# mit-acl/clipper

Measured on AMD Instinct MI355X. Metric: affinity+solve ms and GEMV HBM GB/s, n=10k assoc, 95% outliers, 1/8 GPU, lower is better.
Workload: dtype f64 (M stored f32)

## Files before the change

clipper_amd/csrc/clipper_hip.hip:

```cpp
#include <hip/hip_runtime.h>
#include <rccl/rccl.h>

#include <dlfcn.h>

#include <algorithm>
#include <atomic>
#include <chrono>
#include <cmath>
#include <cstdarg>
#include <cstdio>
#include <cstdlib>
#include <cstring>
#include <functional>
#include <limits>
#include <queue>
#include <string>
#include <type_traits>
#include <utility>
#include <map>
#include <mutex>
#include <new>
#include <exception>
#include <vector>

#include "../../include/clipper_hip.h"
#include "kernels.hip.h"
#include "dsd_host.h"
#include "host_batch.hpp"
#include "host_plan.hpp"

using namespace clipper_hip;

#include "host_state.hpp"
#include "host_solver.hpp"
#include "host_matrix.hpp"
#include "host_rowview.hpp"
#include "host_resident.hpp"
#include "host_rv_resident.hpp"
#include "host_subproblem.hpp"
#include "host_registration.hpp"

namespace {

template <int K, int D>
int knn_run(const double* dP0, int64_t n0, const double* dP1, int64_t n1, int S, int64_t chunk,
            double* pd, int32_t* pi, double* od, int32_t* oi, hipStream_t st) {
  dim3 g(static_cast<unsigned>(ceil_div(n0, 256)), static_cast<unsigned>(S));
  hipLaunchKernelGGL((k_knn_partial<K, D>), g, dim3(256), 0, st, dP0, n0, dP1, n1, chunk, pd, pi);
  hipLaunchKernelGGL((k_knn_merge<K>), dim3(static_cast<unsigned>(ceil_div(n0, 256))), dim3(256), 0,
                     st, pd, pi, n0, S, od, oi);
  return 0;
}

}

extern "C" {

const char* clipper_hip_last_error(void) try {
  return g_err.c_str();
} CLIPPER_HIP_GUARD_STR

int clipper_hip_device_count(void) try {
  int n = 0;
  if (hipGetDeviceCount(&n) != hipSuccess) {
    (void)hipGetLastError();
    return 0;
  }
  return n;
} CLIPPER_HIP_GUARD_INT

clipper_hip_t* clipper_hip_create(int device, int storage) try {
  return make_ctx(&device, 1, storage, 1, 0, false);
} CLIPPER_HIP_GUARD_PTR

clipper_hip_t* clipper_hip_create_group(const int* devices, int nshards, int storage) try {
  if (!devices || nshards < 1) {
    fail(CLIPPER_HIP_E_INVALID, "invalid shard list");
    return nullptr;
  }
  return make_ctx(devices, nshards, storage, nshards, 0, false);
} CLIPPER_HIP_GUARD_PTR

clipper_hip_t* clipper_hip_create_rank(int device, int storage, int rank, int world) try {
  if (world < 1 || rank < 0 || rank >= world) {
    fail(CLIPPER_HIP_E_INVALID, "rank %d / world %d invalid", rank, world);
    return nullptr;
  }
  const char* force = std::getenv("CLIPPER_HIP_FORCE_RCCL");
  const bool multiproc = world > 1 || (force && force[0] == '1');
  return make_ctx(&device, 1, storage, world, rank, multiproc);
} CLIPPER_HIP_GUARD_PTR

int clipper_hip_comm_unique_id(void* id128) try {
  if (!id128) return fail(CLIPPER_HIP_E_INVALID, "null id buffer");
  int rc = load_rccl();
  if (rc) return rc;
  static_assert(sizeof(ncclUniqueId) == 128, "ncclUniqueId is 128 bytes");
  ncclUniqueId id;
  ncclResult_t r = g_rccl.GetUniqueId(&id);
  if (r != ncclSuccess) return fail(CLIPPER_HIP_E_COMM, "ncclGetUniqueId failed (%d)", (int)r);
  std::memcpy(id128, &id, sizeof(id));
  return 0;
} CLIPPER_HIP_GUARD_INT

int clipper_hip_comm_init(clipper_hip_t* h, const void* id128) try {
  if (!h || !id128) return fail(CLIPPER_HIP_E_INVALID, "invalid argument");
  if (!h->multiproc) return 0;
  int rc = load_rccl();
  if (rc) return rc;
  ncclUniqueId id;
  std::memcpy(&id, id128, sizeof(id));
  HIPCHK(hipSetDevice(h->sh[0].device));
  ncclResult_t r = g_rccl.CommInitRank(&h->comm, h->world, id, h->sh[0].slot);
  if (r != ncclSuccess)
    return fail(CLIPPER_HIP_E_COMM, "ncclCommInitRank: %s",
                g_rccl.GetErrorString ? g_rccl.GetErrorString(r) : "error");
  return 0;
} CLIPPER_HIP_GUARD_INT

int clipper_hip_comm_init_callback(clipper_hip_t* h, clipper_hip_allgather_fn fn, void* user) try {
  if (!h || !fn) return fail(CLIPPER_HIP_E_INVALID, "invalid argument");
  if (!h->multiproc) return 0;
  h->xchg_fn = fn;
  h->xchg_user = user;
  return 0;
} CLIPPER_HIP_GUARD_INT

void clipper_hip_destroy(clipper_hip_t* h) try {
  if (!h) return;
  for (auto& s : h->sh) {
    hipSetDevice(s.device);
    if (s.stream) hipStreamSynchronize(s.stream);
  }
  if (h->comm && g_rccl.CommDestroy) g_rccl.CommDestroy(h->comm);
  sub_free(h);
  for (auto& s : h->sh) {
    free_shard_buffers(s);
    if (s.ev_reduced) hipEventDestroy(s.ev_reduced);
    if (s.ev_copied) hipEventDestroy(s.ev_copied);
    if (s.stream) hipStreamDestroy(s.stream);
  }
  if (!h->sh.empty()) hipSetDevice(h->sh[0].device);
  for (hipEvent_t e : h->ev_pairs) hipEventDestroy(e);
  for (hipEvent_t e : h->ev_xchg) hipEventDestroy(e);
  if (h->ev_poll[0]) hipEventDestroy(h->ev_poll[0]);
  if (h->ev_poll[1]) hipEventDestroy(h->ev_poll[1]);
  if (h->host_state) hipHostFree(h->host_state);
  if (h->mirror) hipHostFree(h->mirror);
  if (h->kind) hipHostFree(h->kind);
  if (h->u_pinned) hipHostFree(h->u_pinned);
  if (h->stamps_dev) hipFree(h->stamps_dev);
  if (h->xchg_send) hipHostFree(h->xchg_send);
  if (h->xchg_recv) hipHostFree(h->xchg_recv);
  if (h->ev_aff[0]) hipEventDestroy(h->ev_aff[0]);
  if (h->ev_aff[1]) hipEventDestroy(h->ev_aff[1]);
  if (h->csc_hLq) hipHostFree(h->csc_hLq);
  if (h->csc_hctl) hipHostFree(h->csc_hctl);
  if (h->csc_htotal) hipHostFree(h->csc_htotal);
  resident_free(h);
  rvr_free(h);
  if (h->csc_hwork) hipHostFree(h->csc_hwork);
  if (h->rv_count) hipHostFree(h->rv_count);
  if (h->rv_desc_host) hipHostFree(h->rv_desc_host);
  delete h;
} CLIPPER_HIP_GUARD_VOID


int clipper_hip_stage_inputs(clipper_hip_t* h, const double* D1, int d, int64_t n1,
                             const double* D2, int64_t n2, const int32_t* A, int64_t m) try {
  return stage_inputs(h, D1, d, n1, D2, n2, A, m);
} CLIPPER_HIP_GUARD_INT

int clipper_hip_affinity_euclidean_staged(clipper_hip_t* h, double sigma, double epsilon,
                                          double mindist, double affinityeps) try {
  if (!h) return fail(CLIPPER_HIP_E_INVALID, "invalid argument");
  if (h->staged_d < 1) return fail(CLIPPER_HIP_E_STATE, "clipper_hip_stage_inputs not called");
  const EuclidParams prm{sigma, epsilon, mindist, affinityeps};
  const int64_t mm = h->m, W = h->W, pstride = h->staged_pstride;
  const int d = h->staged_d;
  h->fill_kind = 1;
  h->fill_e = prm;
  h->fill_n = PointNormalParams{};
  h->fill_E2 = guarded_threshold_sq(guarded_threshold(epsilon, h->staged_maxabs, d));
  return run_affinity(h, use_sym_fill(h) && (d == 2 || d == 3), [&](Shard& s) {
    dim3 grid(static_cast<unsigned>(ceil_div(W, 1024)),
              static_cast<unsigned>(ceil_div(mm, AFF_ROWS_PER_BLK))),
        block(256);
    const int64_t c0 = static_cast<int64_t>(s.slot) * W;
    const int32_t* A0 = s.Adev;
    const int32_t* A1 = s.Adev + mm;
#define LAUNCH_EUCLID(T, D)                                                                 \
  hipLaunchKernelGGL((k_affinity_euclid<T, D>), grid, block, 0, s.stream,                   \
                     static_cast<T*>(s.S), W, mm, c0, AFF_ROWS_PER_BLK, d, s.P1, s.P2, pstride, \
                     A0, A1, prm)
#define LAUNCH_EUCLID_COMPACT(T, D)                                                         \
  hipLaunchKernelGGL((k_affinity_euclid_compact<T, D>), grid, block, 0, s.stream,           \
                     static_cast<T*>(s.S), W, mm, c0, AFF_ROWS_PER_BLK, s.P1, s.P2, s.P1f,  \
                     s.P2f, pstride, A0, A1, prm, thr)
    const float thr = guarded_threshold(epsilon, h->staged_maxabs, d);
    if (use_sym_fill(h) && (d == 2 || d == 3)) {
      const int nT = static_cast<int>(ceil_div(mm, AT));
      dim3 g(static_cast<unsigned>(static_cast<int64_t>(nT) * (nT + 1) / 2));
      const PointNormalParams none{};
      const float E2 = guarded_threshold_sq(thr);
      if (h->storage == CLIPPER_HIP_STORE_F64) {
        if (d == 3)
          launch_sym<double>(k_affinity_sym<3, false, double>, g, s.stream, static_cast<double*>(nullptr), W, mm, nT, s,
                             pstride, A0, A1, prm, none, E2, h->csc_out);
        else
          launch_sym<double>(k_affinity_sym<2, false, double>, g, s.stream, static_cast<double*>(nullptr), W, mm, nT, s,
                             pstride, A0, A1, prm, none, E2, h->csc_out);
      } else if (d == 3)
        launch_sym<float>(k_affinity_sym<3, false>, g, s.stream, static_cast<float*>(s.S), W, mm, nT, s,
                          pstride, A0, A1, prm, none, E2, h->csc_out);
      else
        launch_sym<float>(k_affinity_sym<2, false>, g, s.stream, static_cast<float*>(s.S), W, mm, nT, s,
                          pstride, A0, A1, prm, none, E2, h->csc_out);
      h->csc_emitted = (h->csc_out.Pre != nullptr);
      return;
    }
    const bool compact = !h->plain_affinity && (d == 2 || d == 3);
    if (h->storage == CLIPPER_HIP_STORE_F64) {
      if (compact && d == 3) LAUNCH_EUCLID_COMPACT(double, 3);
      else if (compact && d == 2) LAUNCH_EUCLID_COMPACT(double, 2);
      else if (d == 3) LAUNCH_EUCLID(double, 3);
      else if (d == 2) LAUNCH_EUCLID(double, 2);
      else LAUNCH_EUCLID(double, 0);
    } else {
      if (compact && d == 3) LAUNCH_EUCLID_COMPACT(float, 3);
      else if (compact && d == 2) LAUNCH_EUCLID_COMPACT(float, 2);
      else if (d == 3) LAUNCH_EUCLID(float, 3);
      else if (d == 2) LAUNCH_EUCLID(float, 2);
      else LAUNCH_EUCLID(float, 0);
    }
#undef LAUNCH_EUCLID_COMPACT
#undef LAUNCH_EUCLID
  });
} CLIPPER_HIP_GUARD_INT

int clipper_hip_affinity_pointnormal_staged(clipper_hip_t* h, double sigp, double epsp,
                                            double sign, double epsn, double affinityeps) try {
  if (!h) return fail(CLIPPER_HIP_E_INVALID, "invalid argument");
  if (h->staged_d != 6)
    return fail(CLIPPER_HIP_E_STATE, "PointNormalDistance needs staged inputs with d == 6");
  const PointNormalParams prm{sigp, epsp, sign, epsn, affinityeps};
  const int64_t mm = h->m, W = h->W, pstride = h->staged_pstride;
  h->fill_kind = 2;
  h->fill_e = EuclidParams{};
  h->fill_n = prm;
  h->fill_E2 = guarded_threshold_sq(guarded_threshold(epsp, h->staged_maxabs, 3));
  return run_affinity(h, use_sym_fill(h), [&](Shard& s) {
    dim3 grid(static_cast<unsigned>(ceil_div(W, 1024)),
              static_cast<unsigned>(ceil_div(mm, AFF_ROWS_PER_BLK))),
        block(256);
    const int64_t c0 = static_cast<int64_t>(s.slot) * W;
    const float thr = guarded_threshold(epsp, h->staged_maxabs, 3);
    if (use_sym_fill(h)) {
      const int nT = static_cast<int>(ceil_div(mm, AT));
      dim3 g(static_cast<unsigned>(static_cast<int64_t>(nT) * (nT + 1) / 2));
      const EuclidParams none{};
      if (h->storage == CLIPPER_HIP_STORE_F64)
        launch_sym<double>(k_affinity_sym<3, true, double>, g, s.stream, static_cast<double*>(nullptr), W, mm, nT, s,
                           pstride, s.Adev, s.Adev + mm, none, prm, guarded_threshold_sq(thr), h->csc_out);
      else
        launch_sym<float>(k_affinity_sym<3, true>, g, s.stream, static_cast<float*>(s.S), W, mm, nT, s,
                          pstride, s.Adev, s.Adev + mm, none, prm, guarded_threshold_sq(thr), h->csc_out);
      h->csc_emitted = (h->csc_out.Pre != nullptr);
      return;
    }
    if (h->plain_affinity) {
      if (h->storage == CLIPPER_HIP_STORE_F64)
        hipLaunchKernelGGL((k_affinity_pointnormal<double>), grid, block, 0, s.stream,
                           static_cast<double*>(s.S), W, mm, c0, AFF_ROWS_PER_BLK, s.P1, s.P2,
                           pstride, s.Adev, s.Adev + mm, prm);
      else
        hipLaunchKernelGGL((k_affinity_pointnormal<float>), grid, block, 0, s.stream,
                           static_cast<float*>(s.S), W, mm, c0, AFF_ROWS_PER_BLK, s.P1, s.P2,
                           pstride, s.Adev, s.Adev + mm, prm);
    } else {
      if (h->storage == CLIPPER_HIP_STORE_F64)
        hipLaunchKernelGGL((k_affinity_pointnormal_compact<double>), grid, block, 0, s.stream,
                           static_cast<double*>(s.S), W, mm, c0, AFF_ROWS_PER_BLK, s.P1, s.P2,
                           s.P1f, s.P2f, pstride, s.Adev, s.Adev + mm, prm, thr);
      else
        hipLaunchKernelGGL((k_affinity_pointnormal_compact<float>), grid, block, 0, s.stream,
                           static_cast<float*>(s.S), W, mm, c0, AFF_ROWS_PER_BLK, s.P1, s.P2,
                           s.P1f, s.P2f, pstride, s.Adev, s.Adev + mm, prm, thr);
    }
  });
} CLIPPER_HIP_GUARD_INT

int clipper_hip_affinity_euclidean(clipper_hip_t* h, const double* D1, int d, int64_t n1,
                                   const double* D2, int64_t n2, const int32_t* A, int64_t m,
                                   double sigma, double epsilon, double mindist,
                                   double affinityeps) try {
  const auto t0 = std::chrono::high_resolution_clock::now();
  int rc = stage_inputs(h, D1, d, n1, D2, n2, A, m);
  if (rc) return rc;
  rc = clipper_hip_affinity_euclidean_staged(h, sigma, epsilon, mindist, affinityeps);
  if (rc) return rc;
  h->tm.affinity_total_ms =
      std::chrono::duration<double, std::milli>(std::chrono::high_resolution_clock::now() - t0)
          .count();
  return 0;
} CLIPPER_HIP_GUARD_INT

int clipper_hip_affinity_pointnormal(clipper_hip_t* h, const double* D1, int d, int64_t n1,
                                     const double* D2, int64_t n2, const int32_t* A, int64_t m,
                                     double sigp, double epsp, double sign, double epsn,
                                     double affinityeps) try {
  if (d != 6) return fail(CLIPPER_HIP_E_INVALID, "PointNormalDistance needs d == 6");
  const auto t0 = std::chrono::high_resolution_clock::now();
  int rc = stage_inputs(h, D1, d, n1, D2, n2, A, m);
  if (rc) return rc;
  rc = clipper_hip_affinity_pointnormal_staged(h, sigp, epsp, sign, epsn, affinityeps);
  if (rc) return rc;
  h->tm.affinity_total_ms =
      std::chrono::duration<double, std::milli>(std::chrono::high_resolution_clock::now() - t0)
          .count();
  return 0;
} CLIPPER_HIP_GUARD_INT

int64_t clipper_hip_num_associations(const clipper_hip_t* h) try {
  return h ? h->m : 0;
} CLIPPER_HIP_GUARD_INT

int clipper_hip_get_associations(const clipper_hip_t* h, int32_t* A_out) try {
  if (!h || !A_out) return fail(CLIPPER_HIP_E_INVALID, "invalid argument");
  if (h->A.size() != static_cast<size_t>(2 * h->m))
    return fail(CLIPPER_HIP_E_STATE, "no association list is held");
  std::memcpy(A_out, h->A.data(), h->A.size() * sizeof(int32_t));
  return 0;
} CLIPPER_HIP_GUARD_INT


int clipper_hip_set_matrix(clipper_hip_t* h, const double* M, const double* C, int64_t m) try {
  if (!h || !M || !C || m < 1) return fail(CLIPPER_HIP_E_INVALID, "invalid argument");
  if (h->A.size() != static_cast<size_t>(2 * m)) h->A.clear();
  h->nodes.clear();
  h->has_matrix = false;
  h->csc_valid = false;
  h->fill_kind = 0;
  rowview_drop(h);
  int rc = ensure_problem(h, m);
  if (rc) return rc;
  h->has_matrix = false;
  h->csc_valid = false;
  if ((rc = ensure_dense(h, false))) return rc;
  const size_t bytes = static_cast<size_t>(m) * m * sizeof(double);
  const int64_t W = h->W;
  struct Temps {
    std::vector<std::pair<int, void*>> v;
    ~Temps() {
      for (auto& p : v) {
        hipSetDevice(p.first);
        hipFree(p.second);
      }
    }
    int alloc(int dev, void** p, size_t n) {
      HIPCHK(hipMalloc(p, n));
      v.emplace_back(dev, *p);
      return 0;
    }
  } tmp;
  std::vector<double*> dM(h->sh.size(), nullptr), dC(h->sh.size(), nullptr);
  std::vector<int*> dflag(h->sh.size(), nullptr);
  int mismatch = 0;
  const unsigned gy = static_cast<unsigned>(std::min<int64_t>(m, 65535));
  for (size_t k = 0; k < h->sh.size(); ++k) {
    Shard& s = h->sh[k];
    HIPCHK(hipSetDevice(s.device));
    if ((rc = tmp.alloc(s.device, reinterpret_cast<void**>(&dM[k]), bytes))) return rc;
    if ((rc = tmp.alloc(s.device, reinterpret_cast<void**>(&dC[k]), bytes))) return rc;
    if ((rc = tmp.alloc(s.device, reinterpret_cast<void**>(&dflag[k]), sizeof(int)))) return rc;
    HIPCHK(hipMemsetAsync(dflag[k], 0, sizeof(int), s.stream));
    HIPCHK(hipMemcpyAsync(dM[k], M, bytes, hipMemcpyHostToDevice, s.stream));
    HIPCHK(hipMemcpyAsync(dC[k], C, bytes, hipMemcpyHostToDevice, s.stream));
    if (s.Cs) {
      hipFree(s.Cs);
      s.Cs = nullptr;
    }
    dim3 grid(static_cast<unsigned>(ceil_div(W, 256)), gy), block(256);
    const int64_t c0 = static_cast<int64_t>(s.slot) * W;
    if (h->storage == CLIPPER_HIP_STORE_F64)
      hipLaunchKernelGGL((k_from_dense_upper<double>), grid, block, 0, s.stream,
                         static_cast<double*>(s.S), W, m, c0, dM[k], dC[k],
                         static_cast<double*>(nullptr), dflag[k]);
    else
      hipLaunchKernelGGL((k_from_dense_upper<float>), grid, block, 0, s.stream,
                         static_cast<float*>(s.S), W, m, c0, dM[k], dC[k],
                         static_cast<float*>(nullptr), dflag[k]);
    int f = 0;
    HIPCHK(hipMemcpyAsync(&f, dflag[k], sizeof(int), hipMemcpyDeviceToHost, s.stream));
    HIPCHK(hipStreamSynchronize(s.stream));
    HIPCHK(hipGetLastError());
    mismatch |= f;
  }
  if (h->world > 1 && !mismatch) {
    for (int64_t hi = 1; hi < m && !mismatch; ++hi)
      for (int64_t lo = 0; lo < hi; ++lo) {
        const double mv = M[lo + hi * m], cv = C[lo + hi * m];
        if (cv != ((mv != 0.0) ? 1.0 : 0.0)) {
          mismatch = 1;
          break;
        }
      }
  }
  h->explicitC = (mismatch != 0);
  plan_tiles(h);
  if (h->explicitC) {
    for (size_t k = 0; k < h->sh.size(); ++k) {
      Shard& s = h->sh[k];
      HIPCHK(hipSetDevice(s.device));
      HIPCHK(hipMalloc(&s.Cs, s.bytes_S));
      dim3 grid(static_cast<unsigned>(ceil_div(W, 256)), gy), block(256);
      const int64_t c0 = static_cast<int64_t>(s.slot) * W;
      if (h->storage == CLIPPER_HIP_STORE_F64)
        hipLaunchKernelGGL((k_from_dense_upper<double>), grid, block, 0, s.stream,
                           static_cast<double*>(s.S), W, m, c0, dM[k], dC[k],
                           static_cast<double*>(s.Cs), static_cast<int*>(nullptr));
      else
        hipLaunchKernelGGL((k_from_dense_upper<float>), grid, block, 0, s.stream,
                           static_cast<float*>(s.S), W, m, c0, dM[k], dC[k],
                           static_cast<float*>(s.Cs), static_cast<int*>(nullptr));
    }
  }
  if ((rc = sync_all(h))) return rc;
  if ((rc = csc_rebuild(h))) return rc;
  h->has_matrix = true;
  return 0;
} CLIPPER_HIP_GUARD_INT

int clipper_hip_set_sparse(clipper_hip_t* h, int64_t m, const int64_t* Mcolptr,
                           const int32_t* Mrow, const double* Mval, const int64_t* Ccolptr,
                           const int32_t* Crow, const double* Cval) try {
  if (!h || !Mcolptr || !Ccolptr || m < 1) return fail(CLIPPER_HIP_E_INVALID, "invalid argument");
  auto check_csc = [&](const char* what, const int64_t* cp, const int32_t* ri, const double* va) -> int {
    if (cp[0] != 0) return fail(CLIPPER_HIP_E_INVALID, "%s: colptr[0] must be 0", what);
    for (int64_t c = 0; c < m; ++c)
      if (cp[c + 1] < cp[c]) return fail(CLIPPER_HIP_E_INVALID, "%s: colptr decreases at column %lld", what, static_cast<long long>(c));
    const int64_t nnz = cp[m];
    if (nnz > 0 && (!ri || !va)) return fail(CLIPPER_HIP_E_INVALID, "%s: null CSC arrays", what);
    for (int64_t p = 0; p < nnz; ++p)
      if (ri[p] < 0 || ri[p] >= m)
        return fail(CLIPPER_HIP_E_INVALID, "%s: row index %d out of range at entry %lld", what, ri[p], static_cast<long long>(p));
    return 0;
  };
  int rc;
  if ((rc = check_csc("M", Mcolptr, Mrow, Mval))) return rc;
  if ((rc = check_csc("C", Ccolptr, Crow, Cval))) return rc;
  struct Csc {
    std::vector<int64_t> cp;
    std::vector<int32_t> ri;
    std::vector<double> va;
  } Mn, Cn;
  int64_t dropped_below = 0;
  auto upper_only = [&](const char* what, const int64_t*& cp, const int32_t*& ri, const double*& va, Csc& out) -> int {
    bool strict = true;
    for (int64_t j = 0; j < m && strict; ++j)
      for (int64_t p = cp[j]; p < cp[j + 1]; ++p)
        if (ri[p] >= j) {
          strict = false;
          break;
        }
    if (strict) return 0;
    out.cp.assign(static_cast<size_t>(m) + 1, 0);
    for (int64_t j = 0; j < m; ++j) {
      for (int64_t p = cp[j]; p < cp[j + 1]; ++p) {
        const int64_t i = ri[p];
        if (i > j) {
          ++dropped_below;
          continue;
        }
        if (i == j) {
          if (va[p] != 0.0)
            return fail(CLIPPER_HIP_E_INVALID, "%s: a stored diagonal entry (%lld,%lld) — the matrices must not have diagonal values set",
                        what, static_cast<long long>(i), static_cast<long long>(j));
          continue;
        }
        out.ri.push_back(static_cast<int32_t>(i));
        out.va.push_back(va[p]);
      }
      out.cp[static_cast<size_t>(j) + 1] = static_cast<int64_t>(out.ri.size());
    }
    cp = out.cp.data();
    ri = out.ri.data();
    va = out.va.data();
    return 0;
  };
  if ((rc = upper_only("M", Mcolptr, Mrow, Mval, Mn))) return rc;
  if ((rc = upper_only("C", Ccolptr, Crow, Cval, Cn))) return rc;
  if (dropped_below > 0)
    (void)fail(0, "warning: %lld stored entries below the diagonal were ignored (the matrices are read through their upper "
                  "triangle, as the reference's selfadjointView<Upper> does: clipper.cpp:194-271)", static_cast<long long>(dropped_below));
  const int64_t nnzM = Mcolptr[m], nnzC = Ccolptr[m];
  if (h->A.size() != static_cast<size_t>(2 * m)) h->A.clear();
  h->nodes.clear();
  h->has_matrix = false;
  h->csc_valid = false;
  h->total_slice_bytes = 0.0;
  h->fill_kind = 0;
  rowview_drop(h);
  if ((rc = ensure_problem(h, m))) return rc;
  h->has_matrix = false;
  h->csc_valid = false;
  bool pattern = (nnzM == nnzC) && std::equal(Mcolptr, Mcolptr + m + 1, Ccolptr) &&
                 (nnzM == 0 || std::equal(Mrow, Mrow + nnzM, Crow));
  for (int64_t p = 0; pattern && p < nnzM; ++p) pattern = (Cval[p] == 1.0) && (Mval[p] != 0.0);
  h->explicitC = !pattern;
  plan_tiles(h);
  const int64_t W = h->W;
  for (auto& s : h->sh) {
    HIPCHK(hipSetDevice(s.device));
    if (s.Cs) {
      hipFree(s.Cs);
      s.Cs = nullptr;
    }
  }
  struct Temps {
    std::vector<std::pair<int, void*>> v;
    ~Temps() {
      for (auto& p : v) {
        hipSetDevice(p.first);
        hipFree(p.second);
      }
    }
    int alloc(int dev, void** p, size_t n) {
      HIPCHK(hipMalloc(p, std::max<size_t>(n, 16)));
      v.emplace_back(dev, *p);
      return 0;
    }
  } tmp;

  if (csc_applies(h)) {
    drop_dense(h);
    std::vector<int64_t> cp(static_cast<size_t>(m) + 1, 0);
    for (int64_t j = 0; j < m; ++j)
      for (int64_t p = Mcolptr[j]; p < Mcolptr[j + 1]; ++p) {
        const int64_t i = Mrow[p];
        if (i == j) continue;
        ++cp[static_cast<size_t>(i) + 1];
        ++cp[static_cast<size_t>(j) + 1];
      }
    for (int64_t c = 0; c < m; ++c) cp[static_cast<size_t>(c) + 1] += cp[static_cast<size_t>(c)];
    const int64_t nnz2 = cp[static_cast<size_t>(m)];
    std::vector<int32_t> ri(static_cast<size_t>(nnz2));
    std::vector<double> va(static_cast<size_t>(nnz2));
    {
      std::vector<int64_t> cur(cp.begin(), cp.end() - 1);
      for (int64_t j = 0; j < m; ++j)
        for (int64_t p = Mcolptr[j]; p < Mcolptr[j + 1]; ++p) {
          const int64_t i = Mrow[p];
          if (i == j) continue;
          int64_t& a = cur[static_cast<size_t>(j)];
          ri[static_cast<size_t>(a)] = static_cast<int32_t>(i);
          va[static_cast<size_t>(a)] = Mval[p];
          ++a;
          int64_t& b = cur[static_cast<size_t>(i)];
          ri[static_cast<size_t>(b)] = static_cast<int32_t>(j);
          va[static_cast<size_t>(b)] = Mval[p];
          ++b;
        }
    }
    std::vector<std::pair<int32_t, double>> buf;
    for (int64_t c = 0; c < m; ++c) {
      const int64_t a = cp[static_cast<size_t>(c)], b = cp[static_cast<size_t>(c) + 1];
      bool sorted = true;
      for (int64_t p = a + 1; p < b && sorted; ++p) sorted = ri[static_cast<size_t>(p - 1)] < ri[static_cast<size_t>(p)];
      if (sorted) continue;
      buf.clear();
      for (int64_t p = a; p < b; ++p) buf.emplace_back(ri[static_cast<size_t>(p)], va[static_cast<size_t>(p)]);
      std::sort(buf.begin(), buf.end(), [](const auto& x, const auto& y) { return x.first < y.first; });
      for (size_t q = 1; q < buf.size(); ++q)
        if (buf[q - 1].first == buf[q].first)
          return fail(CLIPPER_HIP_E_INVALID, "entry (%d,%lld) is stored more than once", buf[q].first,
                      static_cast<long long>(c));
      for (int64_t p = a; p < b; ++p) {
        ri[static_cast<size_t>(p)] = buf[static_cast<size_t>(p - a)].first;
        va[static_cast<size_t>(p)] = buf[static_cast<size_t>(p - a)].second;
      }
    }
    for (auto& s : h->sh) {
      HIPCHK(hipSetDevice(s.device));
      int64_t* dcp = nullptr;
      int32_t* dri = nullptr;
      double* dva = nullptr;
      if ((rc = tmp.alloc(s.device, reinterpret_cast<void**>(&dcp), cp.size() * sizeof(int64_t)))) return rc;
      if ((rc = tmp.alloc(s.device, reinterpret_cast<void**>(&dri), ri.size() * sizeof(int32_t)))) return rc;
      if ((rc = tmp.alloc(s.device, reinterpret_cast<void**>(&dva), va.size() * sizeof(double)))) return rc;
      HIPCHK(hipMemcpyAsync(dcp, cp.data(), cp.size() * sizeof(int64_t), hipMemcpyHostToDevice, s.stream));
      if (nnz2 > 0) {
        HIPCHK(hipMemcpyAsync(dri, ri.data(), ri.size() * sizeof(int32_t), hipMemcpyHostToDevice, s.stream));
        HIPCHK(hipMemcpyAsync(dva, va.data(), va.size() * sizeof(double), hipMemcpyHostToDevice, s.stream));
      }
      const int64_t c0 = static_cast<int64_t>(s.slot) * W;
      dispatch_vt(h, [&](auto t) {
        using VT = decltype(t);
        bool again = true;
        for (int attempt = 0; again && !rc; ++attempt) {
          if (attempt >= 3) {
            rc = fail(CLIPPER_HIP_E_HIP, "compressed storage: the build keeps overflowing");
            break;
          }
          GroupOut<VT> unused;
          if ((rc = groups_prepare<VT>(h, s, unused))) break;
          CscSource<VT> src{};
          src.colptr = dcp + std::min<int64_t>(c0, m);
          src.rowidx = dri;
          src.values = dva;
          src.ncols = std::max<int64_t>(0, std::min<int64_t>(W, m - c0));
          if ((rc = slices_enqueue<VT>(h, s, src, nullptr))) break;
          if (hipStreamSynchronize(s.stream) != hipSuccess) {
            rc = fail(CLIPPER_HIP_E_HIP, "set_sparse: %s", hipGetErrorString(hipGetLastError()));
            break;
          }
          rc = slices_check<VT>(h, s, false, again);
        }
      });
      if (rc) return rc;
    }
    if ((rc = sync_all(h))) return rc;
    h->csc_valid = true;
    if ((rc = gather_slice_bytes(h))) return rc;
    h->has_matrix = true;
    return 0;
  }

  if ((rc = ensure_dense(h, false))) return rc;
  auto scatter = [&](Shard& s, void* dst, const int64_t* cp, const int32_t* ri, const double* va,
                     int64_t nnz) -> int {
    int64_t* dcp = nullptr;
    int32_t* dri = nullptr;
    double* dva = nullptr;
    int r;
    if ((r = tmp.alloc(s.device, reinterpret_cast<void**>(&dcp), static_cast<size_t>(m + 1) * sizeof(int64_t)))) return r;
    if ((r = tmp.alloc(s.device, reinterpret_cast<void**>(&dri), static_cast<size_t>(nnz) * sizeof(int32_t)))) return r;
    if ((r = tmp.alloc(s.device, reinterpret_cast<void**>(&dva), static_cast<size_t>(nnz) * sizeof(double)))) return r;
    HIPCHK(hipMemcpyAsync(dcp, cp, static_cast<size_t>(m + 1) * sizeof(int64_t),
                          hipMemcpyHostToDevice, s.stream));
    if (nnz > 0) {
      HIPCHK(hipMemcpyAsync(dri, ri, static_cast<size_t>(nnz) * sizeof(int32_t),
                            hipMemcpyHostToDevice, s.stream));
      HIPCHK(hipMemcpyAsync(dva, va, static_cast<size_t>(nnz) * sizeof(double),
                            hipMemcpyHostToDevice, s.stream));
    }
    HIPCHK(hipMemsetAsync(dst, 0, s.bytes_S, s.stream));
    const int64_t c0 = static_cast<int64_t>(s.slot) * W;
    dim3 grid(static_cast<unsigned>(std::min<int64_t>(m, 1 << 20))), block(256);
    if (h->storage == CLIPPER_HIP_STORE_F64)
      hipLaunchKernelGGL((k_from_csc<double>), grid, block, 0, s.stream,
                         static_cast<double*>(dst), W, m, c0, W, dcp, dri, dva);
    else
      hipLaunchKernelGGL((k_from_csc<float>), grid, block, 0, s.stream, static_cast<float*>(dst),
                         W, m, c0, W, dcp, dri, dva);
    HIPCHK(hipGetLastError());
    HIPCHK(hipStreamSynchronize(s.stream));
    return 0;
  };
  for (auto& s : h->sh) {
    HIPCHK(hipSetDevice(s.device));
    rc = scatter(s, s.S, Mcolptr, Mrow, Mval, nnzM);
    if (rc) return rc;
    if (h->explicitC) {
      HIPCHK(hipMalloc(&s.Cs, s.bytes_S));
      rc = scatter(s, s.Cs, Ccolptr, Crow, Cval, nnzC);
      if (rc) return rc;
    }
  }
  rc = csc_rebuild(h);
  if (rc) return rc;
  h->has_matrix = true;
  return 0;
} CLIPPER_HIP_GUARD_INT

int clipper_hip_get_matrix(clipper_hip_t* h, double* M_out, double* C_out) try {
  if (!h) return fail(CLIPPER_HIP_E_INVALID, "invalid argument");
  if (!h->has_matrix) return fail(CLIPPER_HIP_E_STATE, "no matrix has been built or set");
  if (h->multiproc)
    return fail(CLIPPER_HIP_E_STATE, "get_matrix is not available on a multi-process shard");
  const int64_t m = h->m, W = h->W;
  const bool f64 = (h->storage == CLIPPER_HIP_STORE_F64);
  if (int rc = ensure_dense(h, true)) return rc;
  std::vector<unsigned char> buf;
  auto fetch = [&](Shard& s, const void* src, double* out, bool as_pattern) -> int {
    buf.resize(s.bytes_S);
    HIPCHK(hipSetDevice(s.device));
    HIPCHK(hipMemcpy(buf.data(), src, s.bytes_S, hipMemcpyDeviceToHost));
    const int64_t c0 = static_cast<int64_t>(s.slot) * W;
    for (int64_t c = 0; c < W; ++c) {
      const int64_t g = c0 + c;
      if (g >= m) break;
      for (int64_t j = 0; j < m; ++j) {
        const double v = f64 ? reinterpret_cast<const double*>(buf.data())[j * W + c]
                             : static_cast<double>(
                                   reinterpret_cast<const float*>(buf.data())[j * W + c]);
        double o = as_pattern ? ((v != 0.0) ? 1.0 : 0.0) : v;
        if (j == g) o += 1.0;
        out[j + g * m] = o;
      }
    }
    return 0;
  };
  for (auto& s : h->sh) {
    int rc;
    if (M_out && (rc = fetch(s, s.S, M_out, false))) return rc;
    if (C_out) {
      rc = h->explicitC ? fetch(s, s.Cs, C_out, false) : fetch(s, s.S, C_out, true);
      if (rc) return rc;
    }
  }
  if (h->csc_valid) drop_dense(h);
  return 0;
} CLIPPER_HIP_GUARD_INT


int clipper_hip_stage_u0(clipper_hip_t* h, const double* u0) try {
  if (!h || !u0) return fail(CLIPPER_HIP_E_INVALID, "u0 is required");
  if (!h->has_matrix) return fail(CLIPPER_HIP_E_STATE, "no matrix has been built or set");
  const size_t vbytes = static_cast<size_t>(h->m) * sizeof(double);
  for (auto& s : h->sh) {
    HIPCHK(hipSetDevice(s.device));
    HIPCHK(hipMemcpyAsync(s.u0, u0, vbytes, hipMemcpyHostToDevice, s.stream));
  }
  int rc = sync_all(h);
  if (rc) return rc;
  h->u0_staged = true;
  return 0;
} CLIPPER_HIP_GUARD_INT

int clipper_hip_solve(clipper_hip_t* h, const double* u0, const clipper_params_t* P,
                      double* u_out, clipper_solve_info_t* info) try {
  if (!h || !u0 || !P) return fail(CLIPPER_HIP_E_INVALID, "u0 and params are required");
  const auto t0 = std::chrono::high_resolution_clock::now();
  int rc = clipper_hip_stage_u0(h, u0);
  if (rc) return rc;
  rc = clipper_hip_solve_staged(h, P, u_out, info);
  if (rc) return rc;
  const double secs =
      std::chrono::duration<double>(std::chrono::high_resolution_clock::now() - t0).count();
  h->tm.solve_total_ms = secs * 1e3;
  if (info) info->seconds = secs;
  return 0;
} CLIPPER_HIP_GUARD_INT

int clipper_hip_solve_staged(clipper_hip_t* h, const clipper_params_t* P, double* u_out,
                             clipper_solve_info_t* info) try {
  if (!h || !P) return fail(CLIPPER_HIP_E_INVALID, "params are required");
  if (!h->has_matrix) return fail(CLIPPER_HIP_E_STATE, "no matrix has been built or set");
  if (!h->u0_staged) return fail(CLIPPER_HIP_E_STATE, "clipper_hip_stage_u0 not called");
  if (P->rounding == CLIPPER_ROUNDING_DSD && h->multiproc)
    return fail(CLIPPER_HIP_E_SCOPE,
                "Rounding::DSD needs the induced sub-matrix on one host: not available on a "
                "multi-process shard");
  if (P->rounding != CLIPPER_ROUNDING_NONZERO && P->rounding != CLIPPER_ROUNDING_DSD_HEU &&
      P->rounding != CLIPPER_ROUNDING_DSD)
    return fail(CLIPPER_HIP_E_INVALID, "unknown rounding mode %d", P->rounding);
  if (P->maxlsiters < 1) return fail(CLIPPER_HIP_E_INVALID, "maxlsiters must be >= 1");

  const auto t0 = std::chrono::high_resolution_clock::now();
  const int64_t m = h->m;
  const size_t vbytes = static_cast<size_t>(m) * sizeof(double);
  static const bool host_timing = std::getenv("CLIPPER_HIP_HOST_TIMING") != nullptr;
  std::vector<std::pair<const char*, double>> marks_t;
  auto mark_t = [&](const char* what) {
    if (host_timing)
      marks_t.emplace_back(what, std::chrono::duration<double, std::micro>(std::chrono::high_resolution_clock::now() - t0).count());
  };

  h->rv_stats = clipper_hip_view_stats_t{};
  h->ev_used = 0;
  std::fill(h->ev_xchg_used.begin(), h->ev_xchg_used.end(), 0);
  if (h->profiling)
  {
    const size_t n = static_cast<size_t>(std::min<int64_t>(h->launch_counter + 1, KIND_CAP));
    std::memset(h->kind, 0, n);
    HIPCHK(hipSetDevice(h->sh[0].device));
    HIPCHK(hipMemsetAsync(h->sh[0].marks, 0, n, h->sh[0].stream));
  }
  h->launch_counter = 0;

  SolverParams prm;
  prm.tol_u = P->tol_u;
  prm.tol_F = P->tol_F;
  prm.beta = P->beta;
  prm.eps = P->eps;
  prm.maxiniters = P->maxiniters;
  prm.maxoliters = P->maxoliters;
  prm.maxlsiters = P->maxlsiters;

  SolverState init;
  std::memset(&init, 0, sizeof(init));
  init.alpha = 1.0;
  for (int l = 0; l < VS; ++l) init.nrm[l] = 1.0;
  init.nlive = init.nout = static_cast<int32_t>(std::min<int64_t>(m, 0x7fffffff));
  init.rv_last = -100;
  init.weff = 0;
  init.zero_run = 2;
  rowview_drop(h);
  rvr_begin_solve(h);
  sub_begin_solve(h);
  h->rvp = rowview_policy(h);
  init.phase = P->rescale_u0 ? PH_RESCALE : PH_NORMALIZE;
  init.stage = P->rescale_u0 ? ST_PASS : ST_RESULTS;
  if (h->u_pinned_cap < vbytes) {
    if (h->u_pinned) hipHostFree(h->u_pinned);
    h->u_pinned = nullptr;
    h->u_pinned_dev = nullptr;
    h->u_pinned_cap = 0;
    HIPCHK(hipSetDevice(h->sh[0].device));
    HIPCHK(hipHostMalloc(reinterpret_cast<void**>(&h->u_pinned), vbytes,
                         hipHostMallocMapped | hipHostMallocCoherent));
    HIPCHK(hipHostGetDevicePointer(reinterpret_cast<void**>(&h->u_pinned_dev), h->u_pinned, 0));
    h->u_pinned_cap = vbytes;
  }
  Shard& s0 = h->sh[0];
  SolveShared fin;
  std::memset(&fin, 0, sizeof(fin));
  int rc = 0;
  bool resident = false;
  if ((rc = resident_solve(h, prm, P->rescale_u0 != 0, fin, resident))) return rc;
  h->last_solver = resident ? 1 : 0;
  if (!resident) {
  h->par = 0;
  std::memset(h->mirror, 0, sizeof(HostMirror));
  std::atomic_thread_fence(std::memory_order_seq_cst);
  for (auto& s : h->sh) {
    HIPCHK(hipSetDevice(s.device));
    const SolveArgs a = solve_args(h, s, prm, 0);
    hipLaunchKernelGGL(k_init, dim3(static_cast<unsigned>(ceil_div(m, 256))), dim3(256), 0,
                       s.stream, a, init, s.st, s.X[0]);
  }
  mark_t("init queued");
  if (!h->multiproc) {
    volatile HostMirror* hm = h->mirror;
    int64_t queued = 0;
    uint64_t spins = 0;
    h->rv_fresh = false;
    constexpr int run_ahead = RUN_AHEAD;
    h->enqueue_one = [h, &prm]() { return enqueue_iteration(h, prm); };
    auto enqueue_next = [&]() { return enqueue_iteration(h->sub.active ? h->sub.use : h, prm); };
    auto sub_account = [&]() {
      h->sub.sub_passes += std::max<int64_t>(0, hm->n_passes - h->sub.passes_at_entry);
    };
    struct ClearEnqueue {
      Ctx* c;
      ~ClearEnqueue() { c->enqueue_one = nullptr; }
    } clear_enqueue{h};
    while (!hm->done) {
      if (hm->hold) {
        mark_t("hold seen");
        if (host_timing)
          std::fprintf(stderr, "[solve] hold: iters %lld passes %lld trials %lld view passes %lld live %d of which outside the view %d\n",
                       static_cast<long long>(hm->iters), static_cast<long long>(hm->n_passes), static_cast<long long>(hm->n_trials),
                       static_cast<long long>(hm->n_view_passes), static_cast<int>(hm->hold_nlive), static_cast<int>(hm->nout));
        if (h->sh.size() > 1 && (rc = sync_all(h))) return rc;
        std::atomic_thread_fence(std::memory_order_acquire);
        const int hold_reason = hm->hold;
        hm->hold = 0;
        queued = hm->iters;
        h->launch_counter = hm->iters;
        while (h->ev_used > 0 && h->ev_launch_index[static_cast<size_t>(h->ev_used - 1)] >= hm->iters)
          --h->ev_used;
        if (hold_reason == 2) {
          if ((rc = sub_enter(h, prm))) return rc;
          ++queued;
          mark_t("sub-problem entered");
          continue;
        }
        if (hold_reason == 3) {
          sub_account();
          if ((rc = sub_leave(h))) return rc;
          mark_t("sub-problem left");
          continue;
        }
        bool built = false;
        if ((rc = rowview_build(h, built))) return rc;
        mark_t("view built");
        const bool early = h->early_decide_done;
        h->early_decide_done = false;
        if (early) ++queued;
        else h->rv_fresh = built;
        if (built && h->vres.ready) {
          if (!early) {
            h->decide_only = true;
            rc = enqueue_iteration(h, prm);
            h->decide_only = false;
            if (rc) return rc;
            ++queued;
          }
          bool launched = false;
          if ((rc = rvr_enqueue(h, prm, launched))) return rc;
          mark_t("resident queued");
        }
        if ((rc = rowview_finish_plan(h))) return rc;
        if (built && !h->vres.ready && !early) {
          if (int r2 = sub_prepare(h)) {
            if (r2 != CLIPPER_HIP_E_NOMEM) return r2;
            (void)hipGetLastError();
            h->sub.ready = false;
          }
          mark_t("sub-problem prepared");
        }
        continue;
      }
      if (hm->iters > queued) queued = hm->iters;
      if (queued - hm->iters < run_ahead) {
        if ((rc = enqueue_next())) return rc;
        ++queued;
        spins = 0;
      } else if ((++spins & 0xfffff) == 0) {
        hipError_t q = hipStreamQuery(s0.stream);
        if (q != hipSuccess && q != hipErrorNotReady)
          return fail(CLIPPER_HIP_E_HIP, "solver stream failed: %s", hipGetErrorString(q));
        if (q == hipSuccess && !hm->done && queued - hm->iters >= run_ahead)
          return fail(CLIPPER_HIP_E_HIP, "solver made no progress (iters %lld of %lld queued)",
                      static_cast<long long>(hm->iters), static_cast<long long>(queued));
      }
    }
    mark_t("done seen");
    std::atomic_thread_fence(std::memory_order_acquire);
    if (h->sub.active) {
      sub_account();
      h->sub.active = false;
    }
    fin.F = hm->F;
    fin.d = hm->d;
    fin.n_passes = hm->n_passes;
    fin.n_trials = hm->n_trials;
    fin.ifinal = hm->ifinal;
    fin.ubp = hm->ubp;
    fin.ubv = hm->ubv;
    h->rv_stats.view_passes = hm->n_view_passes;
  } else {
    int batch = SOLVE_BATCH;
    if (const char* e = std::getenv("CLIPPER_HIP_SOLVE_BATCH")) batch = std::max(1, std::atoi(e));
    HIPCHK(hipSetDevice(s0.device));
    h->rv_fresh = false;
    rc = run_batched_with_holds(
        batch, [&]() { return enqueue_iteration(h, prm); },
        [&](int slot) -> int {
          HIPCHK(hipSetDevice(s0.device));
          HIPCHK(hipMemcpyAsync(&h->host_state[slot], s0.shared, sizeof(SolveShared),
                                hipMemcpyDeviceToHost, s0.stream));
          HIPCHK(hipEventRecord(h->ev_poll[slot], s0.stream));
          return 0;
        },
        [&](int slot, int& st) -> int {
          HIPCHK(hipEventSynchronize(h->ev_poll[slot]));
          st = h->host_state[slot].done != 0 ? 1 : (h->host_state[slot].hold != 0 ? 2 : 0);
          return 0;
        },
        [&]() -> int {
          if (int r2 = sync_all(h)) return r2;
          h->mirror->hold = 0;
          h->launch_counter = h->mirror->iters;
          while (h->ev_used > 0 && h->ev_launch_index[static_cast<size_t>(h->ev_used - 1)] >= h->mirror->iters)
            --h->ev_used;
          bool built = false;
          if (int r2 = rowview_build(h, built)) return r2;
          h->rv_fresh = built;
          if (built)
            if (int r2 = rvr_replica_handover(h, prm)) return r2;
          return 0;
        },
        nullptr);
    if (rc) return rc;
    if ((rc = sync_all(h))) return rc;
    HIPCHK(hipSetDevice(s0.device));
    HIPCHK(hipMemcpy(&fin, s0.shared, sizeof(fin), hipMemcpyDeviceToHost));
    h->rv_stats.view_passes = h->mirror->n_view_passes;
  }

  rvr_end_solve(h);
  }

  HIPCHK(hipSetDevice(s0.device));
  if (h->multiproc) {
    const double* u_dev =
        s0.pt + ((static_cast<int64_t>(fin.ubp & 1) * h->V + fin.ubv) * 2 + 0) * h->mp;
    HIPCHK(hipMemcpyAsync(h->u_pinned, u_dev, vbytes, hipMemcpyDeviceToHost, s0.stream));
    if (h->profiling)
      HIPCHK(hipMemcpyAsync(h->kind, s0.marks,
                            static_cast<size_t>(std::min<int64_t>(h->launch_counter, KIND_CAP)),
                            hipMemcpyDeviceToHost, s0.stream));
    if ((rc = sync_all(h))) return rc;
  } else {
    HIPCHK(hipGetLastError());
  }
  std::vector<double>& u = h->u_host;
  u.assign(h->u_pinned, h->u_pinned + m);

  std::vector<int32_t> nodes;
  if (P->rounding == CLIPPER_ROUNDING_NONZERO) {
    for (int64_t i = 0; i < m; ++i)
      if (u[static_cast<size_t>(i)] > 0.0) nodes.push_back(static_cast<int32_t>(i));
  } else if (P->rounding == CLIPPER_ROUNDING_DSD) {
    std::vector<int32_t> S;
    for (int64_t i = 0; i < m; ++i)
      if (u[static_cast<size_t>(i)] > 0.0) S.push_back(static_cast<int32_t>(i));
    if ((rc = densest_subgraph_of(h, S, nodes))) return rc;
  } else {
    const int omega = static_cast<int>(std::round(fin.F));
    nodes = indices_of_k_largest(u, omega);
  }
  h->nodes = nodes;
  if (u_out) std::memcpy(u_out, u.data(), vbytes);
  mark_t("rounded");
  if (host_timing) {
    std::fprintf(stderr, "[solve]");
    for (const auto& mk : marks_t) std::fprintf(stderr, " %s %.1f |", mk.first, mk.second);
    std::fprintf(stderr, "\n");
  }

  const double secs =
      std::chrono::duration<double>(std::chrono::high_resolution_clock::now() - t0).count();
  h->tm.solve_total_ms = secs * 1e3;
  if (info) {
    info->score = fin.F;
    info->seconds = secs;
    info->d = fin.d;
    info->ifinal = fin.ifinal;
    info->num_nodes = static_cast<int32_t>(nodes.size());
    info->n_passes = fin.n_passes;
    info->n_trials = fin.n_trials;
  }
  h->rv_stats.passes = fin.n_passes;
  h->rv_stats.sub_leaves = h->sub.leaves;
  h->rv_stats.sub_passes = h->sub.sub_passes;
  h->rv_stats.sub_build_ms = h->sub.build_ms;
  if (h->rv_stats.sub_entries > 0 && h->sub.use) {
    h->rv_stats.sub_rows = h->sub.nS;
    h->rv_stats.sub_bytes = h->sub.use->csc_valid ? static_cast<int64_t>(h->sub.use->sh[0].s_bytes)
                                                   : static_cast<int64_t>(algorithmic_gemv_bytes(h->sub.use));
    h->rv_stats.sub_dense = h->sub.use->csc_valid ? 0 : 1;
  }

  h->tm.gemv_avg_us = h->tm.gemv_min_us = 0.0;
  h->tm.gemv_launches = 0;
  h->tm.gemv_bytes = algorithmic_gemv_bytes(h);
  h->tm.gemv_useful_bytes = h->csc_valid ? static_cast<double>(h->sh[0].s_entries) * (h->esize() + 1.0) : h->tm.gemv_bytes;
  if (h->profiling && h->ev_used > 0) {
    const uint8_t* kind = h->kind;
    const int64_t iters_run = std::min<int64_t>(h->launch_counter, KIND_CAP);
    double sum = 0.0, mn = 1e30, vsum = 0.0, ssum = 0.0;
    int64_t nreal = 0, nview = 0, nsub = 0;
    for (int k = 0; k < h->ev_used; ++k) {
      const int64_t li = h->ev_launch_index[static_cast<size_t>(k)];
      if (li >= iters_run || !kind[static_cast<size_t>(li)]) continue;
      float ms = 0.f;
      HIPCHK(hipEventElapsedTime(&ms, h->ev_pairs[2 * k], h->ev_pairs[2 * k + 1]));
      if (kind[static_cast<size_t>(li)] == 2) {
        vsum += ms;
        ++nview;
        continue;
      }
      if (kind[static_cast<size_t>(li)] == 4) {
        ssum += ms;
        ++nsub;
        continue;
      }
      if (kind[static_cast<size_t>(li)] == 3 || kind[static_cast<size_t>(li)] == 5) continue;
      sum += ms;
      mn = std::min<double>(mn, ms);
      ++nreal;
    }
    h->tm.exchange_avg_us = 0.0;
    h->tm.exchange_samples = 0;
    h->tm.exchange_bytes = static_cast<double>(nslot(h->V)) * static_cast<double>(h->W) * sizeof(double);
    {
      double xs = 0.0;
      int64_t nx = 0;
      for (int k = 0; k < h->ev_used; ++k) {
        const int64_t li = h->ev_launch_index[static_cast<size_t>(k)];
        if (!h->ev_xchg_used[static_cast<size_t>(k)] || li >= iters_run || !kind[static_cast<size_t>(li)]) continue;
        float ms = 0.f;
        HIPCHK(hipEventElapsedTime(&ms, h->ev_xchg[2 * k], h->ev_xchg[2 * k + 1]));
        xs += ms;
        ++nx;
      }
      if (nx > 0) {
        h->tm.exchange_avg_us = xs / static_cast<double>(nx) * 1e3;
        h->tm.exchange_samples = nx;
      }
    }
    if (nview > 0) {
      h->rv_stats.view_pass_avg_us = vsum / static_cast<double>(nview) * 1e3;
      h->rv_stats.view_pass_samples = nview;
    }
    if (nsub > 0) {
      h->rv_stats.sub_pass_avg_us = ssum / static_cast<double>(nsub) * 1e3;
      h->rv_stats.sub_pass_samples = nsub;
    }
    if (nreal > 0) {
      h->tm.gemv_avg_us = sum / static_cast<double>(nreal) * 1e3;
      h->tm.gemv_min_us = mn * 1e3;
      h->tm.gemv_launches = nreal;
    }
  }
  return 0;
} CLIPPER_HIP_GUARD_INT

int clipper_hip_get_nodes(const clipper_hip_t* h, int32_t* out, int32_t capacity) try {
  if (!h || !out) return fail(CLIPPER_HIP_E_INVALID, "invalid argument");
  const int32_t k = static_cast<int32_t>(h->nodes.size());
  if (capacity < k) return fail(CLIPPER_HIP_E_INVALID, "capacity %d < %d nodes", capacity, k);
  if (k) std::memcpy(out, h->nodes.data(), static_cast<size_t>(k) * sizeof(int32_t));
  return k;
} CLIPPER_HIP_GUARD_INT

int clipper_hip_get_selected_associations(const clipper_hip_t* h, int32_t* A_out,
                                          int32_t capacity) try {
  if (!h || !A_out) return fail(CLIPPER_HIP_E_INVALID, "invalid argument");
  const int32_t k = static_cast<int32_t>(h->nodes.size());
  if (capacity < k) return fail(CLIPPER_HIP_E_INVALID, "capacity %d < %d nodes", capacity, k);
  if (k == 0) return 0;
  if (h->A.size() != static_cast<size_t>(2 * h->m))
    return fail(CLIPPER_HIP_E_STATE, "no association list is held");
  for (int32_t r = 0; r < k; ++r) {
    const size_t n = static_cast<size_t>(h->nodes[static_cast<size_t>(r)]);
    A_out[r] = h->A[n];
    A_out[k + r] = h->A[static_cast<size_t>(h->m) + n];
  }
  return k;
} CLIPPER_HIP_GUARD_INT

int clipper_hip_densest_subgraph(clipper_hip_t* h, const int32_t* S, int32_t k, int32_t* nodes_out,
                                 int32_t capacity) try {
  if (!h || !nodes_out) return fail(CLIPPER_HIP_E_INVALID, "invalid argument");
  if (!h->has_matrix) return fail(CLIPPER_HIP_E_STATE, "no matrix has been built or set");
  if (h->multiproc)
    return fail(CLIPPER_HIP_E_SCOPE, "not available on a multi-process shard");
  std::vector<int32_t> sub;
  if (S == nullptr || k <= 0) {
    sub.resize(static_cast<size_t>(h->m));
    for (int64_t i = 0; i < h->m; ++i) sub[static_cast<size_t>(i)] = static_cast<int32_t>(i);
  } else {
    sub.assign(S, S + k);
    for (int32_t v : sub)
      if (v < 0 || v >= h->m) return fail(CLIPPER_HIP_E_INVALID, "node %d out of range", v);
  }
  std::vector<int32_t> nodes;
  int rc = densest_subgraph_of(h, sub, nodes);
  if (rc) return rc;
  const int32_t n = static_cast<int32_t>(nodes.size());
  if (capacity < n) return fail(CLIPPER_HIP_E_INVALID, "capacity %d < %d nodes", capacity, n);
  if (n) std::memcpy(nodes_out, nodes.data(), static_cast<size_t>(n) * sizeof(int32_t));
  return n;
} CLIPPER_HIP_GUARD_INT


int clipper_hip_knn(int device, const double* P0, int64_t n0, const double* P1, int64_t n1, int d,
                    int knn, int32_t* idx_out, double* sqd_out) try {
  if (!P0 || !P1 || !idx_out || n0 < 1 || n1 < 1) return fail(CLIPPER_HIP_E_INVALID, "invalid argument");
  if (d != 2 && d != 3) return fail(CLIPPER_HIP_E_INVALID, "points must have 2 or 3 coordinates");
  if (knn < 1 || knn > 16) return fail(CLIPPER_HIP_E_INVALID, "knn must be in 1..16");
  int ndev = 0;
  if (hipGetDeviceCount(&ndev) != hipSuccess || ndev <= 0)
    return fail(CLIPPER_HIP_E_NODEVICE, "no HIP device visible (this library has no CPU fallback)");
  if (device < 0 || device >= ndev) return fail(CLIPPER_HIP_E_INVALID, "device %d out of range", device);
  HIPCHK(hipSetDevice(device));
  const int K = knn <= 1 ? 1 : (knn <= 2 ? 2 : (knn <= 4 ? 4 : (knn <= 8 ? 8 : 16)));
  const int64_t qblocks = ceil_div(n0, 256);
  const int64_t tiles = ceil_div(n1, KNN_TILE);
  const int S = static_cast<int>(std::max<int64_t>(1, std::min<int64_t>(tiles, ceil_div(512, qblocks))));
  const int64_t chunk = ceil_div(tiles, S) * KNN_TILE;
  double *dP0 = nullptr, *dP1 = nullptr, *pd = nullptr, *od = nullptr;
  int32_t *pi = nullptr, *oi = nullptr;
  auto cleanup = [&]() {
    hipFree(dP0); hipFree(dP1); hipFree(pd); hipFree(od); hipFree(pi); hipFree(oi);
  };
  const size_t b0 = static_cast<size_t>(n0) * d * sizeof(double), b1 = static_cast<size_t>(n1) * d * sizeof(double);
  const size_t np = static_cast<size_t>(S) * n0 * K, no = static_cast<size_t>(n0) * K;
  if (hipMalloc(&dP0, b0) != hipSuccess || hipMalloc(&dP1, b1) != hipSuccess ||
      hipMalloc(&pd, np * sizeof(double)) != hipSuccess || hipMalloc(&pi, np * sizeof(int32_t)) != hipSuccess ||
      hipMalloc(&od, no * sizeof(double)) != hipSuccess || hipMalloc(&oi, no * sizeof(int32_t)) != hipSuccess) {
    cleanup();
    return fail(CLIPPER_HIP_E_NOMEM, "device allocation failed");
  }
  hipStream_t st = nullptr;
  bool ok = hipMemcpyAsync(dP0, P0, b0, hipMemcpyHostToDevice, st) == hipSuccess &&
            hipMemcpyAsync(dP1, P1, b1, hipMemcpyHostToDevice, st) == hipSuccess;
  if (ok) {
#define KNN_CASE(KK)                                                                        \
  case KK:                                                                                  \
    if (d == 3) knn_run<KK, 3>(dP0, n0, dP1, n1, S, chunk, pd, pi, od, oi, st);             \
    else knn_run<KK, 2>(dP0, n0, dP1, n1, S, chunk, pd, pi, od, oi, st);                    \
    break
    switch (K) {
      KNN_CASE(1);
      KNN_CASE(2);
      KNN_CASE(4);
      KNN_CASE(8);
      default:
        if (d == 3) knn_run<16, 3>(dP0, n0, dP1, n1, S, chunk, pd, pi, od, oi, st);
        else knn_run<16, 2>(dP0, n0, dP1, n1, S, chunk, pd, pi, od, oi, st);
        break;
    }
#undef KNN_CASE
    std::vector<double> hd(no);
    std::vector<int32_t> hi(no);
    ok = hipMemcpy(hd.data(), od, no * sizeof(double), hipMemcpyDeviceToHost) == hipSuccess &&
         hipMemcpy(hi.data(), oi, no * sizeof(int32_t), hipMemcpyDeviceToHost) == hipSuccess &&
         hipGetLastError() == hipSuccess;
    if (ok) {
      for (int64_t i = 0; i < n0; ++i)
        for (int k = 0; k < knn; ++k) {
          idx_out[i * knn + k] = hi[static_cast<size_t>(i) * K + k];
          if (sqd_out) sqd_out[i * knn + k] = hd[static_cast<size_t>(i) * K + k];
        }
    }
  }
  cleanup();
  if (!ok) return fail(CLIPPER_HIP_E_HIP, "nearest-neighbour search failed: %s", hipGetErrorString(hipGetLastError()));
  return 0;
} CLIPPER_HIP_GUARD_INT

int64_t clipper_hip_distance_based_correspondences(int device, const double* P0, int64_t n0,
                                                   const double* P1, int64_t n1, int d, int knn,
                                                   double radius, int enforce_1to1, int32_t* A_out,
                                                   int64_t capacity) try {
  if (!A_out && capacity > 0) return fail(CLIPPER_HIP_E_INVALID, "invalid argument");
  std::vector<int32_t> idx(static_cast<size_t>(std::max<int64_t>(n0, 0)) * std::max(knn, 0));
  std::vector<double> sqd(idx.size());
  int rc = clipper_hip_knn(device, P0, n0, P1, n1, d, knn, idx.data(), sqd.data());
  if (rc) return rc;
  const double r2 = radius * radius;
  std::vector<std::pair<int32_t, int32_t>> rows;
  std::map<int32_t, std::vector<std::pair<int32_t, double>>> claim;
  for (int64_t i = 0; i < n0; ++i)
    for (int k = 0; k < knn; ++k) {
      const int32_t c1 = idx[static_cast<size_t>(i) * knn + k];
      const double sd = sqd[static_cast<size_t>(i) * knn + k];
      if (c1 < 0) continue;
      if (sd <= r2) {
        rows.emplace_back(static_cast<int32_t>(i), c1);
        if (enforce_1to1) claim[c1].emplace_back(static_cast<int32_t>(i), sd);
      }
    }
  if (enforce_1to1) {
    rows.clear();
    for (const auto& it : claim) {
      size_t best = 0;
      for (size_t q = 1; q < it.second.size(); ++q)
        if (it.second[q].second < it.second[best].second) best = q;
      rows.emplace_back(it.second[best].first, it.first);
    }
  }
  const int64_t n = static_cast<int64_t>(rows.size());
  if (n > capacity) return fail(CLIPPER_HIP_E_INVALID, "capacity %lld < %lld associations",
                                static_cast<long long>(capacity), static_cast<long long>(n));
  for (int64_t r = 0; r < n; ++r) {
    A_out[r] = rows[static_cast<size_t>(r)].first;
    A_out[n + r] = rows[static_cast<size_t>(r)].second;
  }
  return n;
} CLIPPER_HIP_GUARD_INT

int clipper_hip_set_window(clipper_hip_t* h, int window) try {
  if (!h) return fail(CLIPPER_HIP_E_INVALID, "invalid argument");
  if (window != 0 && window != 1 && window != 4 && window != 6 && window != 8)
    return fail(CLIPPER_HIP_E_INVALID, "window must be 0 (automatic), 1, 4, 6 or 8");
  h->V_forced = window;
  return 0;
} CLIPPER_HIP_GUARD_INT

int clipper_hip_window(const clipper_hip_t* h) try {
  return h ? h->V : 0;
} CLIPPER_HIP_GUARD_INT

int clipper_hip_set_resident(clipper_hip_t* h, int mode) try {
  if (!h) return fail(CLIPPER_HIP_E_INVALID, "invalid argument");
  if (mode != 0 && mode != 1 && mode != 2)
    return fail(CLIPPER_HIP_E_INVALID, "mode must be 0 (automatic), 1 (never) or 2 (the sub-problem always as slices)");
  h->resident_mode = mode;
  return 0;
} CLIPPER_HIP_GUARD_INT

int clipper_hip_last_solver(const clipper_hip_t* h) try {
  return h ? h->last_solver : -1;
} CLIPPER_HIP_GUARD_INT

int clipper_hip_set_row_view(clipper_hip_t* h, int mode) try {
  if (!h) return fail(CLIPPER_HIP_E_INVALID, "invalid argument");
  if (mode != 0 && mode != 1 && mode != 2)
    return fail(CLIPPER_HIP_E_INVALID, "mode must be 0 (automatic), 1 (never) or 2 (views, but streamed: never the resident solver on one)");
  h->rv_mode = mode;
  if (mode == 1) rowview_drop(h);
  if (mode != 0) h->vres.ready = false;
  return 0;
} CLIPPER_HIP_GUARD_INT

int clipper_hip_set_subproblem(clipper_hip_t* h, int mode) try {
  if (!h) return fail(CLIPPER_HIP_E_INVALID, "invalid argument");
  if (mode != 0 && mode != 1 && mode != 2)
    return fail(CLIPPER_HIP_E_INVALID, "mode must be 0 (automatic), 1 (never) or 2 (the sub-problem always as slices)");
  h->sub_mode = mode;
  if (mode == 1) h->sub.ready = false;
  return 0;
} CLIPPER_HIP_GUARD_INT

int clipper_hip_get_view_stats(const clipper_hip_t* h, clipper_hip_view_stats_t* out) try {
  if (!h || !out) return fail(CLIPPER_HIP_E_INVALID, "invalid argument");
  *out = h->rv_stats;
  return 0;
} CLIPPER_HIP_GUARD_INT

int clipper_hip_storage_in_use(const clipper_hip_t* h) try {
  if (!h) return -1;
  if (!h->csc_valid) return h->storage;
  return h->storage == CLIPPER_HIP_STORE_F64 ? CLIPPER_HIP_STORE_F64_CSC : CLIPPER_HIP_STORE_F32_CSC;
} CLIPPER_HIP_GUARD_INT

int clipper_hip_matvec(clipper_hip_t* h, const double* x, double* yM, double* yC) try {
  if (!h || !x) return fail(CLIPPER_HIP_E_INVALID, "invalid argument");
  if (!h->has_matrix) return fail(CLIPPER_HIP_E_STATE, "no matrix has been built or set");
  const int64_t m = h->m, W = h->W;
  for (auto& s : h->sh) {
    HIPCHK(hipSetDevice(s.device));
    HIPCHK(hipMemcpyAsync(s.u0, x, static_cast<size_t>(m) * sizeof(double),
                          hipMemcpyHostToDevice, s.stream));
    hipLaunchKernelGGL(k_spread, dim3(static_cast<unsigned>(ceil_div(m, 256))), dim3(256), 0,
                       s.stream, s.u0, m, s.X[0]);
  }
  h->u0_staged = false;
  int rc = h->csc_valid ? 0 : ensure_dense(h, true);
  if (rc) return rc;
  if ((rc = enqueue_gemv_plain(h))) return rc;
  if ((rc = enqueue_reduce_exchange(h))) return rc;
  if ((rc = sync_all(h))) return rc;
  std::vector<double> ab(static_cast<size_t>(h->world) * 2 * W);
  Shard& s0 = h->sh[0];
  HIPCHK(hipSetDevice(s0.device));
  HIPCHK(hipMemcpy(ab.data(), s0.ab, ab.size() * sizeof(double), hipMemcpyDeviceToHost));
  for (int64_t i = 0; i < m; ++i) {
    const int64_t p = i / W, off = i - p * W;
    if (yM) yM[i] = ab[static_cast<size_t>(p * 2 * W + off)];
    if (yC) yC[i] = ab[static_cast<size_t>(p * 2 * W + W + off)];
  }
  return 0;
} CLIPPER_HIP_GUARD_INT

int clipper_hip_view_matvec(clipper_hip_t* h, const int32_t* rows, int64_t nrows, const double* x,
                            double* yM, double* yC) try {
  if (!h || !rows || !x || nrows < 1) return fail(CLIPPER_HIP_E_INVALID, "invalid argument");
  if (!h->has_matrix || !h->csc_valid || !csc_single(h) || !rect_fill_possible(h))
    return fail(CLIPPER_HIP_E_STATE, "a row view needs slices of a matrix scored from staged points on one device");
  const int64_t m = h->m, W = h->W;
  for (int64_t r = 0; r < nrows; ++r)
    if (rows[r] < 0 || rows[r] >= m || (r > 0 && rows[r] <= rows[r - 1]))
      return fail(CLIPPER_HIP_E_INVALID, "rows must be ascending association indices");
  Shard& s = h->sh[0];
  RowView& v = s.rv;
  HIPCHK(hipSetDevice(s.device));
  HIPCHK(hipStreamSynchronize(s.stream));
  v.valid = false;
  int rc;
  {
    size_t r0 = v.cap_rows, r1 = v.cap_rows;
    if ((rc = rv_grow(v.rowmap[0], r0, static_cast<size_t>(h->mp)))) return rc;
    if ((rc = rv_grow(v.rowmap[1], r1, static_cast<size_t>(h->mp)))) return rc;
    v.cap_rows = static_cast<size_t>(h->mp);
  }
  HIPCHK(hipMemcpyAsync(v.rowmap[0], rows, static_cast<size_t>(nrows) * sizeof(int32_t), hipMemcpyHostToDevice, s.stream));
  for (int attempt = 0;; ++attempt) {
    SliceOut O{};
    if ((rc = emit_prepare(h, s, v.st, nrows, O))) return rc;
    if ((rc = launch_rect(h, s, v.rowmap[0], nrows, O))) return rc;
    if ((rc = emit_enqueue(h, s, v.st))) return rc;
    HIPCHK(hipStreamSynchronize(s.stream));
    HIPCHK(hipGetLastError());
    bool again = false;
    if ((rc = emit_check(h, s, v.st, false, again))) return rc;
    if (!again) break;
    if (attempt >= 2) return fail(CLIPPER_HIP_E_HIP, "row view: the build keeps overflowing");
  }
  HIPCHK(hipMemcpyAsync(s.u0, x, static_cast<size_t>(m) * sizeof(double), hipMemcpyHostToDevice, s.stream));
  hipLaunchKernelGGL(k_spread, dim3(static_cast<unsigned>(ceil_div(m, 256))), dim3(256), 0, s.stream, s.u0, m, s.X[0]);
  h->u0_staged = false;
  SliceView R{};
  R.data = v.st.sdata;
  R.Pre = v.st.sPre;
  R.work = v.st.swork;
  R.nchunks = v.st.s_nchunks;
  R.ncg = v.st.s_ncg;
  R.nwork = v.st.s_nwork;
  R.rowmap = v.rowmap[0];
  R.nrows = nrows;
  R.pad = 0;
  dim3 grid(static_cast<unsigned>(R.nwork)), block(SL_NW * 64);
  if (h->storage == CLIPPER_HIP_STORE_F64)
    hipLaunchKernelGGL((k_gemv_slices_plain<double, 1>), grid, block, 0, s.stream, R, W, m, s.X[0], s.part);
  else
    hipLaunchKernelGGL((k_gemv_slices_plain<float, 1>), grid, block, 0, s.stream, R, W, m, s.X[0], s.part);
  hipLaunchKernelGGL(k_reduce, dim3(static_cast<unsigned>(ceil_div(2 * W, 256))), dim3(256), 0, s.stream, s.part,
                     v.st.s_nslots, 2, W, s.ab);
  std::vector<double> ab(static_cast<size_t>(2 * W));
  HIPCHK(hipMemcpyAsync(ab.data(), s.ab, ab.size() * sizeof(double), hipMemcpyDeviceToHost, s.stream));
  HIPCHK(hipStreamSynchronize(s.stream));
  HIPCHK(hipGetLastError());
  for (int64_t i = 0; i < m; ++i) {
    if (yM) yM[i] = ab[static_cast<size_t>(i)];
    if (yC) yC[i] = ab[static_cast<size_t>(W + i)];
  }
  return 0;
} CLIPPER_HIP_GUARD_INT


int clipper_hip_set_profiling(clipper_hip_t* h, int on) try {
  if (!h) return fail(CLIPPER_HIP_E_INVALID, "invalid argument");
  h->profiling = (on != 0);
  h->profiling_level = on;
  if (h->profiling && h->ev_pairs.empty()) {
    HIPCHK(hipSetDevice(h->sh[0].device));
    h->ev_pairs.resize(2 * MAX_EVENT_PAIRS);
    h->ev_launch_index.assign(MAX_EVENT_PAIRS, 0);
    for (auto& e : h->ev_pairs) HIPCHK(hipEventCreate(&e));
    h->ev_xchg.resize(2 * MAX_EVENT_PAIRS);
    h->ev_xchg_used.assign(MAX_EVENT_PAIRS, 0);
    for (auto& e : h->ev_xchg) HIPCHK(hipEventCreate(&e));
  }
  return 0;
} CLIPPER_HIP_GUARD_INT

int clipper_hip_get_timings(const clipper_hip_t* h, clipper_hip_timings_t* out) try {
  if (!h || !out) return fail(CLIPPER_HIP_E_INVALID, "invalid argument");
  *out = h->tm;
  return 0;
} CLIPPER_HIP_GUARD_INT

int clipper_hip_bench_matvec(clipper_hip_t* h, int reps, double* avg_us) try {
  if (!h || reps < 1 || !avg_us) return fail(CLIPPER_HIP_E_INVALID, "invalid argument");
  if (!h->has_matrix) return fail(CLIPPER_HIP_E_STATE, "no matrix has been built or set");
  if (!h->csc_valid)
    if (int rc = ensure_dense(h, true)) return rc;
  Shard& s = h->sh[0];
  HIPCHK(hipSetDevice(s.device));
  hipEvent_t e0, e1;
  HIPCHK(hipEventCreate(&e0));
  HIPCHK(hipEventCreate(&e1));
  for (int w = 0; w < 3; ++w) launch_plain(h, s, s.X[0]);
  HIPCHK(hipEventRecord(e0, s.stream));
  for (int r = 0; r < reps; ++r) launch_plain(h, s, s.X[0]);
  HIPCHK(hipEventRecord(e1, s.stream));
  HIPCHK(hipStreamSynchronize(s.stream));
  float ms = 0.f;
  HIPCHK(hipEventElapsedTime(&ms, e0, e1));
  hipEventDestroy(e0);
  hipEventDestroy(e1);
  *avg_us = static_cast<double>(ms) * 1e3 / reps;
  h->tm.gemv_bytes = algorithmic_gemv_bytes(h, !h->csc_valid);
  return 0;
} CLIPPER_HIP_GUARD_INT

int clipper_hip_debug_stamps(clipper_hip_t* h, int64_t* out, int capacity) try {
  if (!h || !out || capacity < 0) return fail(CLIPPER_HIP_E_INVALID, "invalid argument");
  if (!h->stamps_dev) return fail(CLIPPER_HIP_E_STATE, "CLIPPER_HIP_STAMPS was not set when the context was created");
  const int n = std::min(capacity, h->stamps_rows * 4);
  HIPCHK(hipSetDevice(h->sh[0].device));
  HIPCHK(hipStreamSynchronize(h->sh[0].stream));
  HIPCHK(hipMemcpy(out, h->stamps_dev, static_cast<size_t>(n) * sizeof(long long), hipMemcpyDeviceToHost));
  return n;
} CLIPPER_HIP_GUARD_INT

int clipper_hip_debug_occupy(int device, int workgroups, int lds_bytes, double milliseconds) try {
  if (workgroups < 1 || lds_bytes < 0 || lds_bytes > static_cast<int>(RS_LDS_MAX) || !(milliseconds >= 0.0) || milliseconds > 2000.0)
    return fail(CLIPPER_HIP_E_INVALID, "invalid argument");
  HIPCHK(hipSetDevice(device));
  if (!raise_dynamic_lds(reinterpret_cast<const void*>(k_debug_occupy), device, static_cast<int>(RS_LDS_MAX)))
    return fail(CLIPPER_HIP_E_HIP, "the device refuses %u bytes of dynamic LDS", RS_LDS_MAX);
  hipStream_t st = nullptr;
  HIPCHK(hipStreamCreateWithFlags(&st, hipStreamNonBlocking));
  hipLaunchKernelGGL(k_debug_occupy, dim3(static_cast<unsigned>(workgroups)), dim3(64), static_cast<size_t>(lds_bytes), st,
                     static_cast<long long>(milliseconds * 1e5));
  const hipError_t e = hipStreamSynchronize(st);
  hipStreamDestroy(st);
  HIPCHK(e);
  return 0;
} CLIPPER_HIP_GUARD_INT

int clipper_hip_device_info(const clipper_hip_t* h, char* name64, int* cus, int64_t* hbm_bytes) try {
  if (!h) return fail(CLIPPER_HIP_E_INVALID, "invalid argument");
  hipDeviceProp_t prop;
  HIPCHK(hipGetDeviceProperties(&prop, h->sh[0].device));
  if (name64) {
    std::snprintf(name64, 64, "%s (%s)", prop.name, prop.gcnArchName);
  }
  if (cus) *cus = prop.multiProcessorCount;
  if (hbm_bytes) *hbm_bytes = static_cast<int64_t>(prop.totalGlobalMem);
  return 0;
} CLIPPER_HIP_GUARD_INT

}
```

clipper_amd/csrc/host_matrix.hpp:

```cpp
#pragma once

namespace {

bool csc_applies(const Ctx* h) { return csc_possible(h) && !h->explicitC; }
constexpr int SL_H = 1;

SliceView slice_view(const Ctx* h, const Shard& s) {
  SliceView M;
  M.data = s.sdata;
  M.Pre = s.sPre;
  M.work = s.swork;
  M.nchunks = s.s_nchunks;
  M.ncg = s.s_ncg;
  M.nwork = s.s_nwork;
  M.rowmap = nullptr;
  M.nrows = h->m;
  M.pad = 0;
  return M;
}

SliceView row_view(const Ctx* h, const Shard& s) {
  SliceView R{};
  if (!s.rv.valid || !h->csc_valid) return R;
  R.data = s.rv.st.sdata;
  R.Pre = s.rv.st.sPre;
  R.work = s.rv.st.swork;
  R.nchunks = s.rv.st.s_nchunks;
  R.ncg = s.rv.st.s_ncg;
  R.nwork = s.rv.st.s_nwork;
  R.rowmap = s.rv.rowmap[s.rv.cur];
  R.nrows = s.rv.nrows;
  return R;
}

SliceView row_view_full(const Ctx* h, const Shard& s) {
  SliceView R{};
  if (!s.rv.valid || !s.rv.full_valid || !h->csc_valid) return R;
  R.data = s.rv.full.sdata;
  R.Pre = s.rv.full.sPre;
  R.work = nullptr;
  R.nchunks = s.rv.full.s_nchunks;
  R.ncg = s.rv.full.s_ncg;
  R.nwork = 0;
  R.rowmap = s.rv.rowmap[s.rv.cur];
  R.nrows = s.rv.nrows;
  return R;
}

template <typename F>
void dispatch_vt(const Ctx* h, F&& f) {
  if (h->storage == CLIPPER_HIP_STORE_F64) f(double{});
  else f(float{});
}

int ensure_dense(Ctx* h, bool from_csc) {
  for (auto& s : h->sh) {
    if (s.S) continue;
    HIPCHK(hipSetDevice(s.device));
    if (hipMalloc(&s.S, s.bytes_S) != hipSuccess) {
      s.S = nullptr;
      (void)hipGetLastError();
      return fail(CLIPPER_HIP_E_NOMEM, "dense store of %zu bytes (this call needs one) does not fit",
                  s.bytes_S);
    }
    if (from_csc && h->csc_valid) {
      const int64_t nsl = static_cast<int64_t>(s.s_ncg) * s.s_nchunks;
      dim3 grid(static_cast<unsigned>(ceil_div(nsl, 4))), block(256);
      dispatch_vt(h, [&](auto t) {
        using T = decltype(t);
        hipLaunchKernelGGL((k_slice_expand<T, SL_H, T>), grid, block, 0, s.stream, slice_view(h, s),
                           static_cast<T*>(s.S), h->W, h->m);
      });
      HIPCHK(hipStreamSynchronize(s.stream));
    }
  }
  return 0;
}

void drop_dense(Ctx* h) {
  for (auto& s : h->sh) {
    if (!s.S) continue;
    hipSetDevice(s.device);
    hipFree(s.S);
    s.S = nullptr;
  }
}

template <typename T>
int grow_dev(T*& p, size_t& cap, size_t need, size_t elem = sizeof(T)) {
  if (need <= cap && p) return 0;
  if (p) hipFree(p);
  p = nullptr;
  cap = 0;
  HIPCHK(hipMalloc(reinterpret_cast<void**>(&p), std::max<size_t>(need, 1) * elem));
  cap = need;
  return 0;
}

int slices_arrays(Ctx* h, Shard& sh, SliceStore& s, int64_t nrows, int64_t wcols = -1) {
  HIPCHK(hipSetDevice(sh.device));
  if (!sh.cctl) HIPCHK(hipMalloc(&sh.cctl, CSC_ARENAS * sizeof(CscBuildCtl)));
  s.s_ncg = static_cast<int>((wcols > 0 ? wcols : h->W) / SL_W);
  s.s_nchunks = static_cast<int>(ceil_div(nrows, SL_SUB * SL_H));
  const size_t nsl = static_cast<size_t>(s.s_ncg) * s.s_nchunks;
  if (nsl > s.scap_slices) {
    for (void** p : {reinterpret_cast<void**>(&s.sSizes), reinterpret_cast<void**>(&s.sLq),
                     reinterpret_cast<void**>(&s.sPre), reinterpret_cast<void**>(&s.sBlk)}) {
      if (*p) hipFree(*p);
      *p = nullptr;
    }
    s.scap_slices = 0;
    HIPCHK(hipMalloc(&s.sSizes, nsl * sizeof(uint32_t)));
    HIPCHK(hipMalloc(&s.sLq, round_up(nsl, 32) * sizeof(uint32_t) + CSC_ARENAS * sizeof(CscBuildCtl)));
    HIPCHK(hipMalloc(&s.sPre, nsl * sizeof(uint64_t)));
    HIPCHK(hipMalloc(&s.sBlk, (ceil_div(nsl, SCAN_BLK) + 4) * sizeof(uint64_t)));
    s.scap_slices = nsl;
  }
  if (nsl > h->csc_hcap_slices) {
    if (h->csc_hLq) hipHostFree(h->csc_hLq);
    h->csc_hLq = nullptr;
    h->csc_hcap_slices = 0;
    HIPCHK(hipHostMalloc(&h->csc_hLq, round_up(nsl, 32) * sizeof(uint32_t) + CSC_ARENAS * sizeof(CscBuildCtl),
                         hipHostMallocDefault));
    h->csc_hcap_slices = nsl;
  }
  if (!h->csc_hctl)
    HIPCHK(hipHostMalloc(&h->csc_hctl, 2 * CSC_ARENAS * sizeof(CscBuildCtl), hipHostMallocDefault));
  if (!h->csc_htotal) HIPCHK(hipHostMalloc(&h->csc_htotal, 2 * sizeof(uint64_t), hipHostMallocDefault));
  return 0;
}
int slices_arrays(Ctx* h, Shard& s) { return slices_arrays(h, s, s, h->m); }

int emit_prepare(Ctx* h, Shard& sh, SliceStore& s, int64_t nrows, SliceOut& out, int64_t wcols = -1) {
  out = SliceOut{};
  if (!csc_applies(h)) return 0;
  if (int rc = slices_arrays(h, sh, s, nrows, wcols)) return rc;
  const size_t units = s.scap_bytes >= SL_TAILPAD ? (s.scap_bytes - SL_TAILPAD) / 16 : 0;
  CscBuildCtl* init = h->csc_hctl + CSC_ARENAS;
  for (int k = 0; k < CSC_ARENAS; ++k) {
    init[k].cursor = 0;
    init[k].capacity = units / CSC_ARENAS;
    init[k].origin = static_cast<unsigned long long>(k) * (units / CSC_ARENAS);
    init[k].overflow = 0;
  }
  CscBuildCtl* ectl = reinterpret_cast<CscBuildCtl*>(
      s.sLq + round_up(static_cast<int64_t>(s.s_ncg) * s.s_nchunks, 32));
  void* idev = nullptr;
  if (hipHostGetDevicePointer(&idev, init, 0) == hipSuccess && idev) {
    hipLaunchKernelGGL(k_copy_words, dim3(1), dim3(256), 0, sh.stream, reinterpret_cast<const uint4*>(idev),
                       reinterpret_cast<uint4*>(ectl), static_cast<int64_t>(CSC_ARENAS * sizeof(CscBuildCtl) / 16));
  } else {
    (void)hipGetLastError();
    HIPCHK(hipMemcpyAsync(ectl, init, CSC_ARENAS * sizeof(CscBuildCtl), hipMemcpyHostToDevice, sh.stream));
  }
  out.Pre = s.sPre;
  out.Lq = s.sLq;
  out.data = s.sdata;
  out.ctl = ectl;
  out.nchunks = s.s_nchunks;
  out.ncg = s.s_ncg;
  out.stamps = h->stamps_dev ? h->stamps_dev + 8192 : nullptr;
  return 0;
}
int emit_prepare(Ctx* h, Shard& s, SliceOut& out) {
  h->csc_valid = false;
  h->csc_emitted = false;
  return emit_prepare(h, s, s, h->m, out);
}

int emit_enqueue(Ctx* h, Shard& sh, SliceStore& s) {
  HIPCHK(hipSetDevice(sh.device));
  const size_t nsl8 = static_cast<size_t>(round_up(static_cast<int64_t>(s.s_ncg) * s.s_nchunks, 32));
  const size_t bytes = nsl8 * sizeof(uint32_t) + CSC_ARENAS * sizeof(CscBuildCtl);
  void* hdev = nullptr;
  if (bytes <= (1u << 20) && hipHostGetDevicePointer(&hdev, h->csc_hLq, 0) == hipSuccess && hdev) {
    const int64_t n16 = static_cast<int64_t>(bytes / 16);
    hipLaunchKernelGGL(k_copy_words, dim3(static_cast<unsigned>(std::min<int64_t>(ceil_div(n16, 256), 64))),
                       dim3(256), 0, sh.stream, reinterpret_cast<const uint4*>(s.sLq),
                       reinterpret_cast<uint4*>(hdev), n16);
  } else {
    (void)hipGetLastError();
    HIPCHK(hipMemcpyAsync(h->csc_hLq, s.sLq, bytes, hipMemcpyDeviceToHost, sh.stream));
  }
  return 0;
}
int emit_enqueue(Ctx* h, Shard& s) { return emit_enqueue(h, s, s); }

int slices_plan(Ctx* h, Shard& sh, SliceStore& s, bool whole);
int slices_plan(Ctx* h, Shard& s) { return slices_plan(h, s, s, true); }
int resident_plan(Ctx* h, Shard& s);

int emit_check(Ctx* h, Shard& sh, SliceStore& s, bool whole, bool& again, bool plan = true) {
  again = false;
  HIPCHK(hipSetDevice(sh.device));
  bool over = false;
  size_t worst = 0;
  uint64_t sum = 0;
  const CscBuildCtl* rb = reinterpret_cast<const CscBuildCtl*>(
      h->csc_hLq + round_up(static_cast<int64_t>(s.s_ncg) * s.s_nchunks, 32));
  for (int k = 0; k < CSC_ARENAS; ++k) {
    over = over || rb[k].overflow != 0;
    worst = std::max(worst, static_cast<size_t>(rb[k].cursor));
    sum += rb[k].cursor;
  }
  if (over) {
    const size_t need = worst * CSC_ARENAS;
    if (s.sdata) hipFree(s.sdata);
    s.sdata = nullptr;
    s.scap_bytes = 0;
    const size_t units = (need + need / 8 + 256 * CSC_ARENAS) / CSC_ARENAS * CSC_ARENAS;
    const size_t cap = units * 16 + SL_TAILPAD;
    HIPCHK(hipMalloc(&s.sdata, cap));
    HIPCHK(hipMemsetAsync(s.sdata + units * 16, 0, SL_TAILPAD, sh.stream));
    s.scap_bytes = cap;
    again = true;
    return 0;
  }
  s.s_bytes = sum * 16;
  if (!plan) {
    s.s_nwork = 0;
    return 0;
  }
  return slices_plan(h, sh, s, whole);
}
int emit_check(Ctx* h, Shard& s, bool& again) { return emit_check(h, s, s, true, again); }

template <typename VT>
int groups_prepare(Ctx* h, Shard& s, GroupOut<VT>& out) {
  out = GroupOut<VT>{};
  h->csc_valid = false;
  h->csc_emitted = false;
  if (!csc_applies(h)) return 0;
  HIPCHK(hipSetDevice(s.device));
  h->csc_nblocks = static_cast<int>(ceil_div(h->m, GR_RB));
  h->csc_nstrips = static_cast<int>(ceil_div(h->W, GR_CW));
  const size_t G = static_cast<size_t>(h->csc_nstrips) * static_cast<size_t>(h->csc_nblocks);
  if (G > s.gcap_groups) {
    if (s.gOff) hipFree(s.gOff);
    if (s.gPre) hipFree(s.gPre);
    s.gOff = nullptr;
    s.gPre = nullptr;
    s.gcap_groups = 0;
    HIPCHK(hipMalloc(&s.gOff, G * GR_OFFS * sizeof(uint16_t)));
    HIPCHK(hipMalloc(&s.gPre, G * sizeof(uint64_t)));
    s.gcap_groups = G;
  }
  if (int rc = slices_arrays(h, s)) return rc;
  CscBuildCtl* init = h->csc_hctl + CSC_ARENAS;
  for (int k = 0; k < CSC_ARENAS; ++k) {
    init[k].cursor = 0;
    init[k].capacity = s.gcap_units / CSC_ARENAS;
    init[k].origin = static_cast<unsigned long long>(k) * (s.gcap_units / CSC_ARENAS);
    init[k].overflow = 0;
  }
  HIPCHK(hipMemcpyAsync(s.cctl, init, CSC_ARENAS * sizeof(CscBuildCtl), hipMemcpyHostToDevice,
                        s.stream));
  out.Goff = s.gOff;
  out.Gpre = s.gPre;
  out.vals = static_cast<VT*>(s.gvals);
  out.rows = s.grows;
  out.ctl = s.cctl;
  out.nblocks = h->csc_nblocks;
  return 0;
}

template <typename VT, typename Source>
int slices_enqueue(Ctx* h, Shard& s, const Source& src, const CscBuildCtl* ctl) {
  HIPCHK(hipSetDevice(s.device));
  const int64_t nsl = static_cast<int64_t>(s.s_ncg) * s.s_nchunks;
  const int64_t nblk = ceil_div(nsl, SCAN_BLK);
  dim3 g4(static_cast<unsigned>(ceil_div(nsl, 4))), b256(256);
  hipLaunchKernelGGL((k_slice_count<VT, SL_H, Source>), g4, b256, 0, s.stream, src, s.s_ncg,
                     s.s_nchunks, s.sSizes, s.sLq, ctl, s.sBlk + nblk + 1);
  if (nsl <= 32768) {
    hipLaunchKernelGGL(k_slice_scan_small, dim3(1), dim3(1024), 0, s.stream, s.sSizes, nsl, s.sPre,
                       s.sBlk + nblk);
  } else {
    hipLaunchKernelGGL(k_slice_scan_local, dim3(static_cast<unsigned>(nblk)), b256, 0, s.stream,
                       s.sSizes, nsl, s.sPre, s.sBlk);
    hipLaunchKernelGGL(k_slice_scan_blocks, dim3(1), b256, 0, s.stream, s.sBlk, nblk);
    hipLaunchKernelGGL(k_slice_scan_add, dim3(static_cast<unsigned>(nblk)), b256, 0, s.stream, s.sPre,
                       nsl, s.sBlk);
  }
  const uint64_t cap_units = s.scap_bytes >= SL_TAILPAD ? (s.scap_bytes - SL_TAILPAD) / 16 : 0;
  int heavy_only = 0;
  if constexpr (std::is_same<Source, GroupSource<VT>>::value && SL_H == 1) {
    hipLaunchKernelGGL((k_slice_pack_staged<VT>), g4, b256, 0, s.stream, src, s.s_ncg, s.s_nchunks,
                       s.sPre, s.sdata, s.sBlk + nblk, cap_units);
    heavy_only = 1;
  }
  hipLaunchKernelGGL((k_slice_pack<VT, SL_H, Source>),
                     dim3(static_cast<unsigned>(std::min<int64_t>(nsl, 1 << 20))),
                     dim3(SL_PACKW * 64), 0, s.stream, src, s.s_ncg, s.s_nchunks, s.sPre, s.sdata,
                     s.sBlk + nblk, cap_units, s.sLq, heavy_only);
  if (ctl)
    HIPCHK(hipMemcpyAsync(h->csc_hctl, s.cctl, CSC_ARENAS * sizeof(CscBuildCtl),
                          hipMemcpyDeviceToHost, s.stream));
  HIPCHK(hipMemcpyAsync(h->csc_htotal, s.sBlk + nblk, sizeof(uint64_t), hipMemcpyDeviceToHost,
                        s.stream));
  HIPCHK(hipMemcpyAsync(h->csc_hLq, s.sLq, static_cast<size_t>(nsl) * sizeof(uint32_t),
                        hipMemcpyDeviceToHost, s.stream));
  return 0;
}

template <typename VT>
GroupSource<VT> group_source(const Ctx* h, const Shard& s) {
  GroupSource<VT> g{};
  g.Goff = s.gOff;
  g.Gpre = s.gPre;
  g.vals = static_cast<const VT*>(s.gvals);
  g.rows = s.grows;
  g.nblocks = h->csc_nblocks;
  g.ncols = static_cast<int64_t>(h->csc_nstrips) * GR_CW;
  return g;
}

int slices_plan(Ctx* h, Shard& sh, SliceStore& s, bool whole) {
  static const double target_env = std::getenv("CLIPPER_HIP_CSC_WGS") ? std::max(1.0, std::atof(std::getenv("CLIPPER_HIP_CSC_WGS"))) : 0.0;
  static_assert(sizeof(clipper_plan::Work) == sizeof(SliceWork), "the planner's work item is the kernel's");
  static thread_local clipper_plan::PassPlan plan;
  clipper_plan::plan_pass(h->csc_hLq, s.s_ncg, s.s_nchunks, clipper_plan::PassConsts{SL_NW, SL_SO, SL_OCC, whole ? 12 : 8},
                          h->cus, target_env, 2.0, plan);
  s.s_entries = plan.entries;
  const int nslots = plan.nslots;
  const size_t nw = plan.work.size();
  if (nw > h->csc_hcap_work) {
    if (h->csc_hwork) hipHostFree(h->csc_hwork);
    h->csc_hwork = nullptr;
    h->csc_hcap_work = 0;
    HIPCHK(hipHostMalloc(&h->csc_hwork, (nw + 1024) * sizeof(SliceWork), hipHostMallocDefault));
    h->csc_hcap_work = nw + 1024;
  }
  std::memcpy(h->csc_hwork, plan.work.data(), nw * sizeof(SliceWork));
  HIPCHK(hipSetDevice(sh.device));
  int rc = grow_dev(s.swork, s.scap_work, nw);
  if (rc) return rc;
  {
    void* wdev = nullptr;
    const size_t bytes = nw * sizeof(SliceWork);
    if (bytes <= (1u << 20) && hipHostGetDevicePointer(&wdev, h->csc_hwork, 0) == hipSuccess && wdev) {
      hipLaunchKernelGGL(k_copy_words, dim3(static_cast<unsigned>(std::min<size_t>(ceil_div(bytes / 16, 256), 64))),
                         dim3(256), 0, sh.stream, reinterpret_cast<const uint4*>(wdev),
                         reinterpret_cast<uint4*>(s.swork), static_cast<int64_t>(bytes / 16));
    } else {
      (void)hipGetLastError();
      HIPCHK(hipMemcpyAsync(s.swork, h->csc_hwork, bytes, hipMemcpyHostToDevice, sh.stream));
    }
    if (h->sh.size() > 1) HIPCHK(hipStreamSynchronize(sh.stream));
  }
  const size_t NSLOT = static_cast<size_t>(nslot(h->V));
  if (static_cast<size_t>(nslots) > sh.part_tiles) {
    HIPCHK(hipStreamSynchronize(sh.stream));
    HIPCHK(hipFree(sh.part));
    sh.part = nullptr;
    sh.part_tiles = static_cast<size_t>(nslots) + 8;
    HIPCHK(hipMalloc(&sh.part, sh.part_tiles * NSLOT * static_cast<size_t>(h->W) * sizeof(double)));
  }
  s.s_nwork = static_cast<int>(nw);
  s.s_nslots = nslots;
  return whole ? resident_plan(h, sh) : 0;
}

template <typename VT>
int slices_check(Ctx* h, Shard& s, bool with_groups, bool& again) {
  again = false;
  if (!csc_applies(h)) return 0;
  HIPCHK(hipSetDevice(s.device));
  if (with_groups) {
    bool over = false;
    size_t worst = 0;
    for (int k = 0; k < CSC_ARENAS; ++k) {
      over = over || h->csc_hctl[k].overflow != 0;
      worst = std::max(worst, static_cast<size_t>(h->csc_hctl[k].cursor));
    }
    if (over) {
      const size_t need = worst * CSC_ARENAS;
      if (s.gvals) hipFree(s.gvals);
      if (s.grows) hipFree(s.grows);
      s.gvals = nullptr;
      s.grows = nullptr;
      s.gcap_units = 0;
      const size_t units = (need + need / 8 + 64 * CSC_ARENAS) / CSC_ARENAS * CSC_ARENAS;
      HIPCHK(hipMalloc(&s.gvals, units * 4 * sizeof(VT)));
      HIPCHK(hipMalloc(&s.grows, units * 4));
      s.gcap_units = units;
      again = true;
    }
  }
  const uint64_t bytes = h->csc_htotal[0] * 16;
  if (bytes + SL_TAILPAD > s.scap_bytes) {
    if (s.sdata) hipFree(s.sdata);
    s.sdata = nullptr;
    s.scap_bytes = 0;
    const size_t cap = static_cast<size_t>(bytes) + static_cast<size_t>(bytes) / 16 + SL_TAILPAD + 4096;
    HIPCHK(hipMalloc(&s.sdata, cap));
    HIPCHK(hipMemsetAsync(s.sdata + bytes, 0, cap - bytes, s.stream));
    s.scap_bytes = cap;
    again = true;
  }
  if (again) return 0;
  s.s_bytes = bytes;
  return slices_plan(h, s);
}

int gather_slice_bytes(Ctx* h);

int csc_rebuild(Ctx* h) {
  h->csc_valid = false;
  h->total_slice_bytes = 0.0;
  if (!csc_applies(h)) return 0;
  int rc = 0;
  dispatch_vt(h, [&](auto t) {
    using VT = decltype(t);
    for (auto& s : h->sh) {
      bool again = true;
      for (int attempt = 0; again; ++attempt) {
        if (attempt >= 3) {
          rc = fail(CLIPPER_HIP_E_HIP, "compressed storage: the build keeps overflowing");
          return;
        }
        GroupOut<VT> O;
        if ((rc = groups_prepare<VT>(h, s, O))) return;
        dim3 grid(h->csc_nstrips, static_cast<unsigned>(ceil_div(h->csc_nblocks, 2))), block(256);
        hipLaunchKernelGGL((k_groups_from_dense<VT>), grid, block, 0, s.stream,
                           static_cast<const VT*>(s.S), h->W, h->m, O);
        if ((rc = slices_enqueue<VT>(h, s, group_source<VT>(h, s), s.cctl))) return;
        if (hipStreamSynchronize(s.stream) != hipSuccess) {
          rc = fail(CLIPPER_HIP_E_HIP, "compressed storage: build failed: %s",
                    hipGetErrorString(hipGetLastError()));
          return;
        }
        if ((rc = slices_check<VT>(h, s, true, again))) return;
      }
    }
  });
  if (rc) return rc;
  h->csc_valid = true;
  drop_dense(h);
  if ((rc = sync_all(h))) return rc;
  return gather_slice_bytes(h);
}

bool rect_fill_possible(const Ctx* h);
int gather_slice_bytes(Ctx* h);
int launch_rect(Ctx* h, Shard& s, const int32_t* rowmap, int64_t nrows, const SliceOut& O, int64_t col0 = -1, int64_t wcols = -1);

int run_affinity_rect(Ctx* h, double& kernel_ms) {
  drop_dense(h);
  Shard& s0 = h->sh[0];
  HIPCHK(hipSetDevice(s0.device));
  if (!h->ev_aff[0]) {
    HIPCHK(hipEventCreate(&h->ev_aff[0]));
    HIPCHK(hipEventCreate(&h->ev_aff[1]));
  }
  std::vector<char> pending(h->sh.size(), 1);
  kernel_ms = 0.0;
  for (int attempt = 0;; ++attempt) {
    if (attempt >= 3) return fail(CLIPPER_HIP_E_HIP, "compressed storage: the build keeps overflowing");
    HIPCHK(hipSetDevice(s0.device));
    HIPCHK(hipEventRecord(h->ev_aff[0], s0.stream));
    std::vector<SliceOut> outs(h->sh.size());
    for (size_t k = 0; k < h->sh.size(); ++k) {
      if (!pending[k]) continue;
      Shard& s = h->sh[k];
      HIPCHK(hipSetDevice(s.device));
      int rc = emit_prepare(h, s, s, h->m, outs[k]);
      if (rc) return rc;
      if (h->sh.size() > 1) HIPCHK(hipStreamSynchronize(s.stream));
      if ((rc = launch_rect(h, s, nullptr, h->m, outs[k]))) return rc;
    }
    HIPCHK(hipSetDevice(s0.device));
    HIPCHK(hipEventRecord(h->ev_aff[1], s0.stream));
    bool any = false;
    for (size_t k = 0; k < h->sh.size(); ++k) {
      if (!pending[k]) continue;
      Shard& s = h->sh[k];
      int rc = emit_enqueue(h, s, s);
      if (rc) return rc;
      HIPCHK(hipStreamSynchronize(s.stream));
      HIPCHK(hipGetLastError());
      bool again = false;
      if ((rc = emit_check(h, s, s, csc_single(h), again))) return rc;
      pending[k] = again ? 1 : 0;
      any = any || again;
    }
    float ms = 0.f;
    HIPCHK(hipSetDevice(s0.device));
    HIPCHK(hipEventElapsedTime(&ms, h->ev_aff[0], h->ev_aff[1]));
    kernel_ms = ms;
    if (!any) break;
  }
  return sync_all(h);
}

template <typename Launch>
int run_affinity(Ctx* h, bool emits, Launch launch) {
  h->has_matrix = false;
  h->csc_valid = false;
  h->total_slice_bytes = 0.0;
  for (auto& s : h->sh) s.rv.valid = false;
  h->nodes.clear();
  for (auto& s : h->sh) {
    if (s.Cs) {
      hipSetDevice(s.device);
      hipFree(s.Cs);
      s.Cs = nullptr;
    }
  }
  h->explicitC = false;
  plan_tiles(h);
  int rc = 0;
  const bool emit = csc_applies(h) && csc_single(h) && emits;
  if (!emit && csc_applies(h) && rect_fill_possible(h) && !h->plain_affinity && !h->strip_affinity) {
    double kms = 0.0;
    if ((rc = run_affinity_rect(h, kms))) return rc;
    h->csc_valid = true;
    h->csc_emitted = true;
    if ((rc = gather_slice_bytes(h))) return rc;
    h->tm.affinity_kernel_ms = kms;
    h->tm.affinity_bytes = static_cast<double>(h->sh[0].s_bytes);
    h->has_matrix = true;
    return 0;
  }
  if (emit) drop_dense(h);
  else if ((rc = ensure_dense(h, false))) return rc;
  Shard& s0 = h->sh[0];
  HIPCHK(hipSetDevice(s0.device));
  if (!h->ev_aff[0]) {
    HIPCHK(hipEventCreate(&h->ev_aff[0]));
    HIPCHK(hipEventCreate(&h->ev_aff[1]));
  }
  hipEvent_t e0 = h->ev_aff[0], e1 = h->ev_aff[1];
  double build_ms = 0.0;
  for (int attempt = 0;; ++attempt) {
    CscOut O{};
    if (emit) {
      rc = emit_prepare(h, s0, O);
      if (rc) return rc;
    } else {
      h->csc_valid = false;
      h->csc_emitted = false;
    }
    h->csc_out = O;
    HIPCHK(hipSetDevice(s0.device));
    HIPCHK(hipEventRecord(e0, s0.stream));
    for (auto& s : h->sh) {
      HIPCHK(hipSetDevice(s.device));
      launch(s);
    }
    if (emit) {
      rc = emit_enqueue(h, s0);
      if (rc) return rc;
    }
    HIPCHK(hipSetDevice(s0.device));
    HIPCHK(hipEventRecord(e1, s0.stream));
    const auto th0 = std::chrono::high_resolution_clock::now();
    rc = sync_all(h);
    if (rc) return rc;
    const auto th1 = std::chrono::high_resolution_clock::now();
    if (!emit) {
      const auto t0 = std::chrono::high_resolution_clock::now();
      rc = csc_rebuild(h);
      if (rc) return rc;
      build_ms = std::chrono::duration<double, std::milli>(
                     std::chrono::high_resolution_clock::now() - t0).count();
      break;
    }
    bool again = false;
    rc = emit_check(h, s0, again);
    if (rc) return rc;
    if (std::getenv("CLIPPER_HIP_HOST_TIMING")) {
      const auto th2 = std::chrono::high_resolution_clock::now();
      float kms = 0.f;
      (void)hipEventElapsedTime(&kms, e0, e1);
      std::fprintf(stderr, "[affinity] enqueue->synced %.1f us (events %.1f us), check+plan %.1f us\n",
                   std::chrono::duration<double, std::micro>(th1 - th0).count(), kms * 1e3,
                   std::chrono::duration<double, std::micro>(th2 - th1).count());
    }
    if (!again) {
      h->csc_valid = true;
      break;
    }
    if (attempt >= 2) return fail(CLIPPER_HIP_E_HIP, "compressed storage: the build keeps overflowing");
  }
  float ms = 0.f;
  HIPCHK(hipSetDevice(s0.device));
  HIPCHK(hipEventElapsedTime(&ms, e0, e1));
  h->tm.affinity_kernel_ms = ms + (h->csc_valid ? build_ms : 0.0);
  h->tm.affinity_bytes = h->csc_valid ? static_cast<double>(h->sh[0].s_bytes)
                                      : static_cast<double>(h->sh[0].bytes_S);
  h->has_matrix = true;
  return 0;
}

constexpr int AFF_ROWS_PER_BLK = 32;

double algorithmic_gemv_bytes(const Ctx* h, bool dense = false) {
  if (h->csc_valid && !dense)
    return static_cast<double>(h->sh[0].s_bytes) +
           static_cast<double>(h->sh[0].s_ncg) * h->sh[0].s_nchunks * 8.0;
  const int64_t c0 = static_cast<int64_t>(h->sh[0].slot) * h->W;
  const int64_t valid = std::max<int64_t>(0, std::min<int64_t>(h->W, h->m - c0));
  return static_cast<double>(h->esize()) * static_cast<double>(h->m) *
         static_cast<double>(valid) * (h->explicitC ? 2.0 : 1.0);
}

int densest_subgraph_of(Ctx* h, const std::vector<int32_t>& S, std::vector<int32_t>& nodes) {
  nodes.clear();
  const int k = static_cast<int>(S.size());
  if (k < 2) return 0;
  std::vector<double> Wsub, tmp;
  std::vector<int32_t> pos;
  try {
    Wsub.assign(static_cast<size_t>(k) * k, 0.0);
    tmp.resize(static_cast<size_t>(k) * k);
    pos.assign(static_cast<size_t>(h->m), -1);
  } catch (const std::bad_alloc&) {
    return fail(CLIPPER_HIP_E_NOMEM, "densest subgraph of %d nodes: %.1f GB of host memory per copy of the sub-matrix", k,
                static_cast<double>(k) * k * 8e-9);
  }
  bool listed_once = true;
  for (int a = 0; a < k; ++a) {
    int32_t& p = pos[static_cast<size_t>(S[static_cast<size_t>(a)])];
    listed_once = listed_once && p < 0;
    p = a;
  }
  const bool from_slices = h->csc_valid && listed_once;
  const auto t0 = std::chrono::high_resolution_clock::now();
  if (!from_slices)
    if (int rc = ensure_dense(h, true)) return rc;
  for (auto& s : h->sh) {
    HIPCHK(hipSetDevice(s.device));
    int32_t* didx = nullptr;
    double* dout = nullptr;
    const size_t nidx = from_slices ? pos.size() : static_cast<size_t>(k);
    HIPCHK(hipMalloc(&didx, nidx * sizeof(int32_t)));
    HIPCHK(hipMalloc(&dout, tmp.size() * sizeof(double)));
    HIPCHK(hipMemcpyAsync(didx, from_slices ? pos.data() : S.data(), nidx * sizeof(int32_t),
                          hipMemcpyHostToDevice, s.stream));
    HIPCHK(hipMemsetAsync(dout, 0, tmp.size() * sizeof(double), s.stream));
    const int64_t c0 = static_cast<int64_t>(s.slot) * h->W;
    if (from_slices) {
      const int64_t nsl = static_cast<int64_t>(s.s_ncg) * s.s_nchunks;
      dim3 grid(static_cast<unsigned>(ceil_div(nsl, 4))), block(256);
      dispatch_vt(h, [&](auto t) {
        using T = decltype(t);
        hipLaunchKernelGGL((k_slice_gather_sub<T, SL_H>), grid, block, 0, s.stream, slice_view(h, s), didx,
                           c0, h->m, k, dout);
      });
    } else {
      dim3 grid(static_cast<unsigned>(ceil_div(static_cast<int64_t>(k) * k, 256))), block(256);
      if (h->storage == CLIPPER_HIP_STORE_F64)
        hipLaunchKernelGGL((k_gather_sub<double>), grid, block, 0, s.stream,
                           static_cast<const double*>(s.S), h->W, c0, h->W, didx, k, dout);
      else
        hipLaunchKernelGGL((k_gather_sub<float>), grid, block, 0, s.stream,
                           static_cast<const float*>(s.S), h->W, c0, h->W, didx, k, dout);
    }
    HIPCHK(hipGetLastError());
    HIPCHK(hipMemcpyAsync(tmp.data(), dout, tmp.size() * sizeof(double), hipMemcpyDeviceToHost,
                          s.stream));
    HIPCHK(hipStreamSynchronize(s.stream));
    hipFree(didx);
    hipFree(dout);
    for (size_t e = 0; e < tmp.size(); ++e) Wsub[e] += tmp[e];
  }
  if (h->csc_valid) drop_dense(h);
  const auto t1 = std::chrono::high_resolution_clock::now();
  int flows = 0;
  tmp = std::vector<double>();
  try {
    for (int32_t a : dsd::densest_subgraph(Wsub, k, h->m, &flows)) nodes.push_back(S[static_cast<size_t>(a)]);
  } catch (const std::bad_alloc&) {
    return fail(CLIPPER_HIP_E_NOMEM, "densest subgraph of %d nodes: the flow network does not fit the host's memory", k);
  }
  if (std::getenv("CLIPPER_HIP_HOST_TIMING"))
    std::fprintf(stderr, "[dsd] k = %d: gather (%s) %.2f ms, host %.2f ms, %d maximum flows%s, %zu nodes\n", k,
                 from_slices ? "slices" : "dense store", std::chrono::duration<double, std::milli>(t1 - t0).count(),
                 std::chrono::duration<double, std::milli>(std::chrono::high_resolution_clock::now() - t1).count(),
                 flows < 0 ? -flows : flows, flows < 0 ? " (plain bisection)" : "", nodes.size());
  return 0;
}

}
```

clipper_amd/csrc/host_rowview.hpp:

```cpp
#pragma once

namespace {

template <typename K>
void launch_rect_kernel(K kernel, int lds_bytes, dim3 grid, hipStream_t stream, const RectGeom& G,
                        const Shard& s, int64_t pstride, const int32_t* A0, const int32_t* A1,
                        const EuclidParams& e, const PointNormalParams& n, float E2, const SliceOut& O) {
  raise_dynamic_lds(reinterpret_cast<const void*>(kernel), s.device, lds_bytes);
  hipLaunchKernelGGL(kernel, grid, dim3(AT_WAVES * 64), lds_bytes, stream, G, s.P1, s.P2, s.P1f, s.P2f,
                     pstride, A0, A1, e, n, E2, O);
}

bool rect_fill_possible(const Ctx* h) {
  return (h->fill_kind == 1 && (h->staged_d == 2 || h->staged_d == 3)) ||
         (h->fill_kind == 2 && h->staged_d == 6);
}

int launch_rect(Ctx* h, Shard& s, const int32_t* rowmap, int64_t nrows, const SliceOut& O, int64_t col0, int64_t wcols) {
  if (!rect_fill_possible(h)) return fail(CLIPPER_HIP_E_STATE, "no built-in invariant is staged");
  const int64_t W = wcols > 0 ? wcols : h->W;
  RectGeom G;
  G.m = h->m;
  G.nrows = nrows;
  G.rowmap = rowmap;
  G.col0 = col0 >= 0 ? col0 : static_cast<int64_t>(s.slot) * h->W;
  G.ncols = std::max<int64_t>(0, std::min<int64_t>(W, h->m - G.col0));
  const int64_t nTr = ceil_div(nrows, AT);
  const int32_t* A0 = s.Adev;
  const int32_t* A1 = s.Adev + h->m;
  const int64_t ps = h->staged_pstride;
  const bool thin = nTr * ceil_div(W, 128) <= 2 * static_cast<int64_t>(h->cus);
  dispatch_vt(h, [&](auto t) {
    using VT = decltype(t);
    auto run = [&](auto twc) {
      constexpr int TW = decltype(twc)::value;
      G.nTc = static_cast<int>(ceil_div(W, TW));
      const int64_t ntiles = nTr * G.nTc;
      constexpr int64_t PER_LAUNCH = int64_t(1) << 22;
      constexpr int L = rect_lds_bytes<VT, TW>();
      for (int64_t t0 = 0; t0 < ntiles; t0 += PER_LAUNCH) {
        G.tile0 = t0;
        const dim3 grid(static_cast<unsigned>(std::min<int64_t>(PER_LAUNCH, ntiles - t0)));
        if (h->fill_kind == 2)
          launch_rect_kernel(k_affinity_rect<3, true, VT, TW>, L, grid, s.stream, G, s, ps, A0, A1, h->fill_e, h->fill_n, h->fill_E2, O);
        else if (h->staged_d == 3)
          launch_rect_kernel(k_affinity_rect<3, false, VT, TW>, L, grid, s.stream, G, s, ps, A0, A1, h->fill_e, h->fill_n, h->fill_E2, O);
        else
          launch_rect_kernel(k_affinity_rect<2, false, VT, TW>, L, grid, s.stream, G, s, ps, A0, A1, h->fill_e, h->fill_n, h->fill_E2, O);
      }
    };
    if constexpr (rect_tw<VT>() == 64) {
      run(std::integral_constant<int, 64>{});
    } else {
      if (thin) run(std::integral_constant<int, 64>{});
      else run(std::integral_constant<int, 128>{});
    }
  });
  HIPCHK(hipGetLastError());
  return 0;
}

int launch_filter(Ctx* h, Shard& s, const int32_t* rowmap, const int32_t* viewpos, int64_t nrows, const SliceOut& O) {
  FilterGeom G;
  G.nrows = nrows;
  G.rowmap = rowmap;
  G.viewpos = viewpos;
  const int64_t nTr = ceil_div(nrows, AT);
  const SliceView M = slice_view(h, s);
  dispatch_vt(h, [&](auto t) {
    using VT = decltype(t);
    G.nTc = static_cast<int>(ceil_div(h->W, FILT_TW));
    const int64_t ntiles = nTr * G.nTc;
    constexpr int64_t PER_LAUNCH = int64_t(1) << 22;
    constexpr int L = filt_lds_bytes<VT>();
    raise_dynamic_lds(reinterpret_cast<const void*>(k_slice_filter_rows<VT>), s.device, L);
    for (int64_t t0 = 0; t0 < ntiles; t0 += PER_LAUNCH) {
      G.tile0 = t0;
      const dim3 grid(static_cast<unsigned>(std::min<int64_t>(PER_LAUNCH, ntiles - t0)));
      hipLaunchKernelGGL((k_slice_filter_rows<VT>), grid, dim3(AT_WAVES * 64), L, s.stream, M, G, O);
    }
  });
  HIPCHK(hipGetLastError());
  return 0;
}

int rowview_build_env() {
  static const int mode = [] {
    const char* e = std::getenv("CLIPPER_HIP_RV_BUILD");
    if (!e) return 0;
    const std::string v(e);
    return v == "filter" ? 1 : (v == "rectfill" ? 2 : 0);
  }();
  return mode;
}
bool rowview_fill_by_filter(const Ctx* h) { return rowview_build_env() == 1 || !rect_fill_possible(h); }
bool rowview_cost_of_filter(const Ctx* h) { return rowview_build_env() != 0 || !rect_fill_possible(h); }


int rvr_plan(Ctx* h, Shard& s, bool replica);
uint32_t* rvr_ctl_block(Ctx* h) {
  ViewResident& r = h->vres;
  return (r.ctl != nullptr && r.launches_this_solve < RVR_GIVEUP_SLOTS) ? r.ctl + 16 * r.launches_this_solve : nullptr;
}
bool rvr_candidate(const Ctx* h, int64_t nrows);
int rowview_put_descriptor(Ctx* h, Shard& s);

void rowview_drop(Ctx* h) {
  for (auto& s : h->sh) s.rv.valid = s.rv.full_valid = false;
  h->vres.ready = false;
}

void rowview_free(Shard& s) {
  auto fr = [](auto*& p) {
    if (p) hipFree(p);
    p = nullptr;
  };
  RowView& v = s.rv;
  fr(v.st.sSizes);
  fr(v.st.sLq);
  fr(v.st.sPre);
  fr(v.st.sBlk);
  fr(v.st.sdata);
  fr(v.st.swork);
  v.st = SliceStore{};
  fr(v.full.sSizes);
  fr(v.full.sLq);
  fr(v.full.sPre);
  fr(v.full.sBlk);
  fr(v.full.sdata);
  fr(v.full.swork);
  v.full = SliceStore{};
  v.full_valid = false;
  fr(v.rowmap[0]);
  fr(v.rowmap[1]);
  fr(v.in_view[0]);
  fr(v.in_view[1]);
  fr(v.blk);
  fr(v.viewpos);
  fr(v.desc);
  v.cap_rows = v.cap_flags = v.cap_blk = v.cap_pos = 0;
  v.valid = false;
  v.nrows = 0;
}

bool rowview_possible(const Ctx* h) {
  static const bool env_off = [] {
    const char* e = std::getenv("CLIPPER_HIP_ROW_VIEW");
    return e && std::atoi(e) == 0;
  }();
  return !env_off && h->rv_mode != 1 && h->csc_valid && !h->explicitC &&
         h->m >= RV_MIN_M &&
         (csc_single(h) || h->total_slice_bytes > 0.0);
}

int gather_slice_bytes(Ctx* h) {
  h->total_slice_bytes = 0.0;
  if (csc_single(h) || !h->csc_valid) return 0;
  if (h->multiproc && !h->comm && !h->xchg_fn) return 0;
  for (auto& s : h->sh) {
    HIPCHK(hipSetDevice(s.device));
    const double v = static_cast<double>(s.s_bytes);
    HIPCHK(hipMemcpy(s.ab + static_cast<int64_t>(s.slot) * h->W, &v, sizeof(double), hipMemcpyHostToDevice));
  }
  if (int rc = exchange(h, 1)) return rc;
  if (int rc = sync_all(h)) return rc;
  Shard& s0 = h->sh[0];
  HIPCHK(hipSetDevice(s0.device));
  double total = 0.0;
  for (int p = 0; p < h->world; ++p) {
    double v = 0.0;
    HIPCHK(hipMemcpy(&v, s0.ab + static_cast<int64_t>(p) * h->W, sizeof(double), hipMemcpyDeviceToHost));
    total += v;
  }
  h->total_slice_bytes = total;
  return 0;
}

ViewPolicy rowview_policy(const Ctx* h) {
  static const double scale_env = std::getenv("CLIPPER_HIP_RV_BUILD_SCALE") ? std::atof(std::getenv("CLIPPER_HIP_RV_BUILD_SCALE")) : 1.0;
  ViewPolicy p{};
  p.on = rowview_possible(h) ? 1 : 0;
  p.max_builds = RV_MAX_BUILDS;
  p.pass_fixed = 8e-6;
  const double bytes = csc_single(h) ? static_cast<double>(h->sh[0].s_bytes)
                                     : h->total_slice_bytes / static_cast<double>(std::max(1, h->world));
  p.pass_per_row = bytes / static_cast<double>(h->m) / 3.3e12;
  if (rowview_cost_of_filter(h)) {
    p.build_fixed = (100e-6 + bytes / 1.1e12) * scale_env;
    p.build_per_row = bytes / static_cast<double>(h->m) / 1.1e12 * scale_env;
  } else {
    p.build_fixed = 60e-6 * scale_env;
    p.build_per_row = static_cast<double>(h->W) * (h->esize() == 8 ? 9.0e-12 : 4.5e-12) * scale_env;
  }
  return p;
}

template <typename T>
int rv_grow(T*& p, size_t& cap, size_t need) {
  if (need <= cap && p) return 0;
  if (p) hipFree(p);
  p = nullptr;
  cap = 0;
  HIPCHK(hipMalloc(reinterpret_cast<void**>(&p), std::max<size_t>(need, 1) * sizeof(T)));
  cap = need;
  return 0;
}

template <int V>
int rowview_build_shard(Ctx* h, Shard& s, bool& built);

template <int V>
int rowview_build_v(Ctx* h, bool& built) {
  built = false;
  bool first = true;
  for (auto& s : h->sh) {
    bool b = false;
    if (int rc = rowview_build_shard<V>(h, s, b)) return rc;
    if (first) built = b;
    else if (b != built) return fail(CLIPPER_HIP_E_HIP, "row view: the shards disagree");
    first = false;
  }
  if (built) {
    h->rv_stats.builds += 1;
    h->rv_stats.rows = h->sh[0].rv.nrows;
    h->rv_stats.bytes = static_cast<int64_t>(h->sh[0].rv.st.s_bytes);
  }
  return 0;
}

template <int V>
int rowview_build_shard(Ctx* h, Shard& s, bool& built) {
  built = false;
  RowView& v = s.rv;
  const auto t0 = std::chrono::high_resolution_clock::now();
  HIPCHK(hipSetDevice(s.device));
  const int64_t m = h->m, mp = h->mp;
  const int nblk = static_cast<int>(ceil_div(m, RV_BLK));
  int rc;
  {
    size_t c0 = v.cap_flags, c1 = v.cap_flags;
    if ((rc = rv_grow(v.in_view[0], c0, static_cast<size_t>(mp)))) return rc;
    if ((rc = rv_grow(v.in_view[1], c1, static_cast<size_t>(mp)))) return rc;
    v.cap_flags = static_cast<size_t>(mp);
    size_t r0 = v.cap_rows, r1 = v.cap_rows;
    if ((rc = rv_grow(v.rowmap[0], r0, static_cast<size_t>(mp)))) return rc;
    if ((rc = rv_grow(v.rowmap[1], r1, static_cast<size_t>(mp)))) return rc;
    v.cap_rows = static_cast<size_t>(mp);
    if ((rc = rv_grow(v.blk, v.cap_blk, static_cast<size_t>(nblk) + 2))) return rc;
    if ((rc = rv_grow(v.viewpos, v.cap_pos, static_cast<size_t>(mp)))) return rc;
  }
  if (!h->rv_count) {
    HIPCHK(hipHostMalloc(reinterpret_cast<void**>(&h->rv_count), 64, hipHostMallocMapped | hipHostMallocCoherent));
    HIPCHK(hipHostGetDevicePointer(reinterpret_cast<void**>(&h->rv_count_dev), h->rv_count, 0));
  }
  const int next = v.cur ^ 1;
  *h->rv_count = -1;
  std::atomic_thread_fence(std::memory_order_seq_cst);
  if (mp <= RV_ONE_MAX) {
    hipLaunchKernelGGL((k_rv_list_one<V>), dim3(1), dim3(1024), 0, s.stream, s.st + h->par, s.pt, mp, m, v.in_view[next],
                       v.rowmap[next], static_cast<int64_t>(v.cap_rows), v.viewpos, h->rv_count_dev);
  } else {
    hipLaunchKernelGGL((k_rv_flags<V>), dim3(static_cast<unsigned>(nblk)), dim3(256), 0, s.stream,
                       s.st + h->par, s.pt, mp, m, v.in_view[next], v.blk);
    hipLaunchKernelGGL(k_rv_scan, dim3(1), dim3(1024), 0, s.stream, v.blk, nblk, h->rv_count_dev);
    hipLaunchKernelGGL(k_rv_scatter, dim3(static_cast<unsigned>(nblk)), dim3(256), 0, s.stream,
                       v.in_view[next], m, v.blk, v.rowmap[next], static_cast<int64_t>(v.cap_rows), v.viewpos, mp);
  }
  static const bool host_timing = std::getenv("CLIPPER_HIP_HOST_TIMING") != nullptr;
  auto lap = [&](const char* what) {
    if (host_timing)
      std::fprintf(stderr, "[view] %s %.1f us\n", what,
                   std::chrono::duration<double, std::micro>(std::chrono::high_resolution_clock::now() - t0).count());
  };
  const int64_t asked = h->mirror->hold_nlive;
  int64_t nrows = asked;
  static const bool test_miscount = std::getenv("CLIPPER_HIP_RV_TEST_MISCOUNT") != nullptr;
  if (test_miscount && asked > 1) nrows = asked - 1;
  bool counted = false;
  bool store_gone = false;
  bool early_done = false;
  const bool early_ok = h->enqueue_one != nullptr && h->sh.size() == 1 && !h->multiproc;
  h->early_decide_done = false;
  if (asked <= 0 || asked > m) {
    HIPCHK(hipStreamSynchronize(s.stream));
    nrows = *h->rv_count;
    counted = true;
    lap("row list");
  }
  const double rows_now = v.valid ? static_cast<double>(v.nrows) : static_cast<double>(m);
  const ViewPolicy pol = h->rvp;
  const double horizon = std::max<double>(12.0, static_cast<double>(h->mirror->iters + 1));
  for (int attempt = 0;; ++attempt) {
    if (counted) {
      if (nrows < 0) return fail(CLIPPER_HIP_E_HIP, "row view: the row count did not arrive");
      const bool as_asked = nrows > 0 && nrows == asked;
      if (!as_asked &&
          (nrows == 0 ||
           (!store_gone && (static_cast<double>(nrows) > RV_ROWS_RATIO * rows_now ||
                            RV_GAIN_MARGIN * (pol.build_fixed + pol.build_per_row * static_cast<double>(nrows)) >=
                                horizon * (rows_now - static_cast<double>(nrows)) * pol.pass_per_row)))) {
        if (!early_done)
          hipLaunchKernelGGL(k_rv_resume, dim3(1), dim3(64), 0, s.stream, s.st + h->par, s.shared, static_cast<int>(nrows),
                             static_cast<uint32_t*>(nullptr));
        h->early_decide_done = early_done;
        h->rv_stats.build_ms +=
            std::chrono::duration<double, std::milli>(std::chrono::high_resolution_clock::now() - t0).count();
        return 0;
      }
    }
    v.valid = false;
    v.full_valid = false;
    store_gone = true;
    SliceOut O{};
    if ((rc = emit_prepare(h, s, v.st, nrows, O))) return rc;
    if (rowview_fill_by_filter(h)) rc = launch_filter(h, s, v.rowmap[next], v.viewpos, nrows, O);
    else rc = launch_rect(h, s, v.rowmap[next], nrows, O);
    if (rc) return rc;
    if ((rc = emit_enqueue(h, s, v.st))) return rc;
    if (early_ok && attempt == 0 && !counted && rvr_candidate(h, nrows)) {
      const int cur0 = v.cur;
      const int64_t nrows0 = v.nrows;
      v.cur = next;
      v.nrows = nrows;
      v.valid = true;
      v.st.s_nwork = 0;
      if ((rc = rowview_put_descriptor(h, s))) return rc;
      hipLaunchKernelGGL(k_rv_resume, dim3(1), dim3(64), 0, s.stream, s.st + h->par, s.shared, 0, rvr_ctl_block(h));
      h->rv_fresh = true;
      h->decide_only = true;
      rc = h->enqueue_one ? h->enqueue_one() : CLIPPER_HIP_E_INTERNAL;
      h->decide_only = false;
      if (rc) return rc;
      early_done = true;
      v.valid = false;
      v.cur = cur0;
      v.nrows = nrows0;
    }
    HIPCHK(hipStreamSynchronize(s.stream));
    HIPCHK(hipGetLastError());
    lap("filled");
    if (!counted) {
      counted = true;
      if (*h->rv_count != nrows) {
        nrows = *h->rv_count;
        continue;
      }
    }
    bool again = false;
    const bool defer = rvr_candidate(h, nrows);
    if ((rc = emit_check(h, s, v.st, false, again, !defer))) return rc;
    lap("planned");
    if (!again) {
      v.plan_pending = defer;
      break;
    }
    if (attempt >= 3) return fail(CLIPPER_HIP_E_HIP, "row view: the build keeps overflowing");
  }
  v.cur = next;
  v.nrows = nrows;
  v.valid = true;
  built = true;
  if ((rc = rvr_plan(h, s, false))) return rc;
  lap("resident plan");
  if (v.plan_pending && !h->vres.ready) {
    if ((rc = slices_plan(h, s, v.st, false))) return rc;
    v.plan_pending = false;
  }
  if ((rc = rowview_put_descriptor(h, s))) return rc;
  if (!early_done) hipLaunchKernelGGL(k_rv_resume, dim3(1), dim3(64), 0, s.stream, s.st + h->par, s.shared, 0, rvr_ctl_block(h));
  h->early_decide_done = early_done;
  h->rv_stats.build_ms +=
      std::chrono::duration<double, std::milli>(std::chrono::high_resolution_clock::now() - t0).count();
  return 0;
}

int rowview_put_descriptor(Ctx* h, Shard& s) {
  RowView& v = s.rv;
  if (!v.desc) HIPCHK(hipMalloc(reinterpret_cast<void**>(&v.desc), sizeof(SliceView)));
  if (!h->rv_desc_host) {
    HIPCHK(hipHostMalloc(reinterpret_cast<void**>(&h->rv_desc_host), 2 * sizeof(SliceView), hipHostMallocMapped | hipHostMallocCoherent));
    HIPCHK(hipHostGetDevicePointer(reinterpret_cast<void**>(&h->rv_desc_host_dev), h->rv_desc_host, 0));
  }
  const int slot = (h->rv_desc_slot ^= 1);
  h->rv_desc_host[slot] = row_view(h, s);
  std::atomic_thread_fence(std::memory_order_seq_cst);
  hipLaunchKernelGGL(k_copy_words, dim3(1), dim3(64), 0, s.stream, reinterpret_cast<const uint4*>(h->rv_desc_host_dev + slot),
                     reinterpret_cast<uint4*>(v.desc), static_cast<int64_t>(sizeof(SliceView) / 16));
  if (h->sh.size() > 1) HIPCHK(hipStreamSynchronize(s.stream));
  return 0;
}

int rowview_finish_plan(Ctx* h) {
  for (auto& s : h->sh) {
    RowView& v = s.rv;
    if (!v.valid || !v.plan_pending) continue;
    HIPCHK(hipSetDevice(s.device));
    if (int rc = slices_plan(h, s, v.st, false)) return rc;
    v.plan_pending = false;
    if (int rc = rowview_put_descriptor(h, s)) return rc;
  }
  return 0;
}

int rowview_build(Ctx* h, bool& built) {
  int rc = 0;
  dispatch_window(h, [&](auto v) { rc = rowview_build_v<decltype(v)::value>(h, built); });
  return rc;
}

}
```

clipper_amd/csrc/host_solver.hpp:

```cpp
#pragma once

namespace {

using Ctx = clipper_hip_ctx;

void rowview_free(Shard& s);
void rowview_drop(Ctx* h);
void sub_free(Ctx* h);

int free_shard_buffers(Shard& s) {
  hipSetDevice(s.device);
  auto fr = [](auto*& p) {
    if (p) hipFree(p);
    p = nullptr;
  };
  fr(s.S);
  fr(s.Cs);
  fr(s.part);
  fr(s.u0);
  fr(s.pt);
  fr(s.cab);
  fr(s.X[0]);
  fr(s.X[1]);
  fr(s.ab);
  fr(s.scal);
  fr(s.st);
  fr(s.shared);
  fr(s.marks);
  fr(s.gOff);
  fr(s.gPre);
  fr(s.gvals);
  fr(s.grows);
  fr(s.cctl);
  s.gcap_units = s.gcap_groups = 0;
  fr(s.sSizes);
  fr(s.sLq);
  fr(s.sPre);
  fr(s.sBlk);
  fr(s.sdata);
  fr(s.swork);
  s.scap_slices = s.scap_bytes = s.scap_work = 0;
  rowview_free(s);
  s.part_tiles = 0;
  fr(s.P1);
  fr(s.P2);
  fr(s.P1f);
  fr(s.P2f);
  s.capPf = 0;
  fr(s.Adev);
  fr(s.dD1);
  fr(s.dD2);
  s.capP = s.capA = s.capD1 = s.capD2 = 0;
  s.bytes_S = 0;
  return 0;
}

bool csc_possible(const Ctx* h) { return h->compressed; }
bool csc_single(const Ctx* h) { return csc_possible(h) && h->world == 1 && !h->multiproc; }

int plan_unr(const Ctx* h) {
  return gemv_unr(h->V, static_cast<int>(h->esize()), h->explicitC);
}

int64_t max_tiles(const Ctx* h) {
  const int64_t slots = static_cast<int64_t>(h->cus) * GEMV_WG_PER_CU;
  int64_t nt = std::max<int64_t>(16, ceil_div(slots, std::max(1, h->nstrips)) + 1);
  return nt;
}

void plan_tiles(Ctx* h) {
  const int unr = plan_unr(h);
  const int64_t chunk = static_cast<int64_t>(GEMV_NW) * unr;
  h->nstrips = static_cast<int>(ceil_div(h->W, 256));
  const double slots = static_cast<double>(h->cus) * GEMV_WG_PER_CU;
  int64_t nt_max = std::min<int64_t>(max_tiles(h), std::max<int64_t>(1, ceil_div(h->m, chunk)));
  if (h->world > 1) nt_max = std::min<int64_t>(nt_max, 32);
  int64_t best = 1;
  double best_cost = 1e300;
  for (int64_t nt = 1; nt <= nt_max; ++nt) {
    const double w = static_cast<double>(h->nstrips) * static_cast<double>(nt) / slots;
    const double whole = std::floor(w), frac = w - whole;
    const double waves = whole + ((frac <= 0.03 && whole >= 1.0) ? frac : (frac > 0.0 ? 1.0 : 0.0));
    const double cost = waves / w + 0.003 * static_cast<double>(nt);
    if (cost < best_cost) {
      best_cost = cost;
      best = nt;
    }
  }
  int64_t rpt = round_up(ceil_div(h->m, best), chunk);
  h->rows_per_tile = static_cast<int>(rpt);
  h->ntiles = static_cast<int>(ceil_div(h->m, rpt));
}

int ensure_problem(Ctx* h, int64_t m) {
  if (m <= 0) return fail(CLIPPER_HIP_E_INVALID, "m must be positive");
  const int64_t P = h->world;
  const int64_t W = round_up(ceil_div(m, P), 64);
  h->m = m;
  h->W = W;
  h->mp = P * W;
  const int64_t six_from = h->compressed ? WINDOW_MIN_M_CSC : WINDOW_MIN_M;
  const int V = h->V_forced ? h->V_forced : (m >= six_from ? 6 : (m >= WINDOW4_MIN_M ? 4 : 1));
  const bool same = (h->alloc_m == m && h->alloc_W == W && h->V == V);
  h->V = V;
  plan_tiles(h);
  if (same) return 0;
  sub_free(h);
  for (auto& s : h->sh) {
    free_shard_buffers(s);
    HIPCHK(hipSetDevice(s.device));
    const size_t bytesS = static_cast<size_t>(m) * static_cast<size_t>(W) * h->esize();
    s.bytes_S = bytesS;
    if (!h->compressed) HIPCHK(hipMalloc(&s.S, bytesS));
    const size_t nvec = static_cast<size_t>(P * W) * sizeof(double);
    const size_t V = static_cast<size_t>(h->V);
    HIPCHK(hipMalloc(&s.u0, nvec));
    const size_t NSLOT = static_cast<size_t>(nslot(h->V));
    HIPCHK(hipMalloc(&s.pt, 2 * V * 2 * nvec));
    HIPCHK(hipMalloc(&s.cab, 2 * nvec));
    for (int k = 0; k < 2; ++k) {
      HIPCHK(hipMalloc(&s.X[k], (V + 1) * VS * nvec));
      HIPCHK(hipMemsetAsync(s.X[k], 0, (V + 1) * VS * nvec, s.stream));
    }
    const size_t Q = static_cast<size_t>(tail_q(h->V));
    const size_t nwg = static_cast<size_t>(ceil_div(m, TAIL_THREADS));
    HIPCHK(hipMalloc(&s.scal, (nwg + ceil_div(nwg, SCAL_FOLD) + 1) * Q * sizeof(double)));
    HIPCHK(hipMalloc(&s.ab, NSLOT * nvec));
    HIPCHK(hipMemsetAsync(s.ab, 0, NSLOT * nvec, s.stream));
    s.part_tiles = static_cast<size_t>(max_tiles(h));
    HIPCHK(hipMalloc(&s.part, s.part_tiles * NSLOT * W * sizeof(double)));
    HIPCHK(hipMalloc(&s.st, 2 * sizeof(SolverState)));
    HIPCHK(hipMemsetAsync(s.st, 0, 2 * sizeof(SolverState), s.stream));
    HIPCHK(hipMalloc(&s.shared, sizeof(SolveShared)));
    HIPCHK(hipMalloc(&s.marks, KIND_CAP));
    HIPCHK(hipMemsetAsync(s.marks, 0, KIND_CAP, s.stream));
    HIPCHK(hipMemsetAsync(s.shared, 0, sizeof(SolveShared), s.stream));
  }
  h->alloc_m = m;
  h->alloc_W = W;
  h->has_matrix = false;
  h->csc_valid = false;
  h->explicitC = false;
  plan_tiles(h);
  h->u0_staged = false;
  h->staged_d = 0;
  return 0;
}

template <typename T, bool HASC, int V>
void launch_pass_tv(Ctx* h, Shard& s, const SolveArgs& a) {
  constexpr int UNR = gemv_unr(V, sizeof(T), HASC);
  dim3 grid(h->nstrips, h->ntiles), block(GEMV_NW * 64);
  hipLaunchKernelGGL((k_gemv<T, HASC, V, GEMV_NW, UNR>), grid, block, 0, s.stream,
                     static_cast<const T*>(s.S), static_cast<const T*>(s.Cs), h->rows_per_tile, a);
}

template <typename T, bool HASC>
void launch_plain_t(Ctx* h, Shard& s, const double* X) {
  constexpr int UNR = gemv_unr(1, sizeof(T), HASC);
  dim3 grid(h->nstrips, h->ntiles), block(GEMV_NW * 64);
  hipLaunchKernelGGL((k_gemv_plain<T, HASC, GEMV_NW, UNR>), grid, block, 0, s.stream,
                     static_cast<const T*>(s.S), static_cast<const T*>(s.Cs), h->W, h->m,
                     h->rows_per_tile, X, s.part);
}

template <typename F>
void dispatch_storage(Ctx* h, F&& f) {
  if (h->storage == CLIPPER_HIP_STORE_F64) {
    if (h->explicitC) f(double{}, std::true_type{});
    else f(double{}, std::false_type{});
  } else {
    if (h->explicitC) f(float{}, std::true_type{});
    else f(float{}, std::false_type{});
  }
}

template <int V>
void launch_pass(Ctx* h, Shard& s, const SolveArgs& a) {
  dispatch_storage(h, [&](auto t, auto c) {
    launch_pass_tv<decltype(t), decltype(c)::value, V>(h, s, a);
  });
}

SliceView slice_view(const Ctx* h, const Shard& s);
SliceView row_view(const Ctx* h, const Shard& s);

void launch_plain(Ctx* h, Shard& s, const double* X) {
  if (h->csc_valid) {
    const SliceView M = slice_view(h, s);
    dim3 grid(static_cast<unsigned>(s.s_nwork)), block(SL_NW * 64);
    if (h->storage == CLIPPER_HIP_STORE_F64)
      hipLaunchKernelGGL((k_gemv_slices_plain<double, 1>), grid, block, 0, s.stream, M, h->W, h->m, X, s.part);
    else
      hipLaunchKernelGGL((k_gemv_slices_plain<float, 1>), grid, block, 0, s.stream, M, h->W, h->m, X, s.part);
    return;
  }
  dispatch_storage(h, [&](auto t, auto c) {
    launch_plain_t<decltype(t), decltype(c)::value>(h, s, X);
  });
}

SliceView slice_view(const Ctx* h, const Shard& s);

template <int V>
void launch_pass_csc(Ctx* h, Shard& s, const SolveArgs& a) {
  const SliceView M = slice_view(h, s), R = row_view(h, s);
  dim3 grid(static_cast<unsigned>(std::max(M.nwork, R.nwork))), block(SL_NW * 64);
  const SliceView* rdev = s.rv.desc;
  if (h->storage == CLIPPER_HIP_STORE_F64)
    hipLaunchKernelGGL((k_gemv_slices<double, 1, V>), grid, block, 0, s.stream, M, rdev, a);
  else
    hipLaunchKernelGGL((k_gemv_slices<float, 1, V>), grid, block, 0, s.stream, M, rdev, a);
}

template <typename F>
void dispatch_window(const Ctx* h, F&& f) {
  switch (h->V) {
    case 1: f(std::integral_constant<int, 1>{}); break;
    case 4: f(std::integral_constant<int, 4>{}); break;
#ifndef CLIPPER_NO_V8
    case 8: f(std::integral_constant<int, 8>{}); break;
#endif
    default: f(std::integral_constant<int, 6>{}); break;
  }
}

void launch_reduce(Ctx* h, Shard& s, int nslots) {
  dim3 grid(static_cast<unsigned>(ceil_div(static_cast<int64_t>(nslots) * h->W, 256))), block(256);
  hipLaunchKernelGGL(k_reduce, grid, block, 0, s.stream, s.part,
                     h->csc_valid ? s.s_nslots : h->ntiles, nslots, h->W,
                     s.ab + static_cast<int64_t>(s.slot) * nslots * h->W);
}

int exchange(Ctx* h, int nslots) {
  if (h->world == 1 && !h->multiproc) return 0;
  const int64_t blk_elems = static_cast<int64_t>(nslots) * h->W;
  const size_t blk = static_cast<size_t>(blk_elems) * sizeof(double);
  if (h->multiproc && h->xchg_fn) {
    Shard& s = h->sh[0];
    HIPCHK(hipSetDevice(s.device));
    const size_t need = static_cast<size_t>(h->world) * blk;
    if (need > h->xchg_cap) {
      if (h->xchg_send) hipHostFree(h->xchg_send);
      if (h->xchg_recv) hipHostFree(h->xchg_recv);
      h->xchg_send = h->xchg_recv = nullptr;
      h->xchg_cap = 0;
      HIPCHK(hipHostMalloc(reinterpret_cast<void**>(&h->xchg_send), blk, hipHostMallocDefault));
      HIPCHK(hipHostMalloc(reinterpret_cast<void**>(&h->xchg_recv), need, hipHostMallocDefault));
      h->xchg_cap = need;
    }
    HIPCHK(hipMemcpyAsync(h->xchg_send, s.ab + static_cast<int64_t>(s.slot) * blk_elems, blk,
                          hipMemcpyDeviceToHost, s.stream));
    HIPCHK(hipStreamSynchronize(s.stream));
    if (int rc = h->xchg_fn(h->xchg_user, h->xchg_send, h->xchg_recv, blk))
      return fail(CLIPPER_HIP_E_COMM, "the exchange callback returned %d", rc);
    HIPCHK(hipMemcpyAsync(s.ab, h->xchg_recv, need, hipMemcpyHostToDevice, s.stream));
    return 0;
  }
  if (h->multiproc) {
    if (!h->comm) return fail(CLIPPER_HIP_E_COMM, "clipper_hip_comm_init was not called");
    Shard& s = h->sh[0];
    ncclResult_t r = g_rccl.AllGather(s.ab + static_cast<int64_t>(s.slot) * blk_elems, s.ab,
                                      static_cast<size_t>(blk_elems), ncclDouble, h->comm,
                                      s.stream);
    if (r != ncclSuccess)
      return fail(CLIPPER_HIP_E_COMM, "ncclAllGather: %s",
                  g_rccl.GetErrorString ? g_rccl.GetErrorString(r) : "error");
    return 0;
  }
  for (auto& p : h->sh) {
    HIPCHK(hipSetDevice(p.device));
    HIPCHK(hipEventRecord(p.ev_reduced, p.stream));
  }
  for (auto& q : h->sh) {
    HIPCHK(hipSetDevice(q.device));
    for (auto& p : h->sh) {
      if (p.slot == q.slot) continue;
      HIPCHK(hipStreamWaitEvent(q.stream, p.ev_reduced, 0));
      const int64_t off = static_cast<int64_t>(p.slot) * blk_elems;
      if (p.device == q.device) {
        HIPCHK(hipMemcpyAsync(q.ab + off, p.ab + off, blk, hipMemcpyDeviceToDevice, q.stream));
      } else {
        HIPCHK(hipMemcpyPeerAsync(q.ab + off, q.device, p.ab + off, p.device, blk, q.stream));
      }
    }
    HIPCHK(hipEventRecord(q.ev_copied, q.stream));
  }
  for (auto& p : h->sh) {
    HIPCHK(hipSetDevice(p.device));
    for (auto& q : h->sh) {
      if (p.slot == q.slot) continue;
      HIPCHK(hipStreamWaitEvent(p.stream, q.ev_copied, 0));
    }
  }
  return 0;
}

SolveArgs solve_args(Ctx* h, Shard& s, const SolverParams& prm, int par) {
  SolveArgs a;
  a.st_cur = s.st + par;
  a.st_next = s.st + (par ^ 1);
  a.shared = s.shared;
  a.host = (&s == &h->sh[0]) ? h->mirror_dev : nullptr;
  a.prm = prm;
  a.m = h->m;
  a.W = h->W;
  a.mp = h->mp;
  a.u0 = s.u0;
  a.pt = s.pt;
  a.cab = s.cab;
  a.Xin = s.X[par];
  a.Xout = s.X[par ^ 1];
  a.ab = s.ab;
  a.part = s.part;
  a.ntiles = h->csc_valid ? s.s_nslots : h->ntiles;
  a.slot = s.slot;
  a.scal = s.scal;
  a.nwg = static_cast<int>(ceil_div(h->m, TAIL_THREADS));
  a.scal_in = s.scal;
  a.nwg_in = a.nwg;
  if (a.nwg > SCAL_FOLD_MIN) {
    a.scal_in = s.scal + static_cast<int64_t>(a.nwg) * tail_q(h->V);
    a.nwg_in = static_cast<int>(ceil_div(a.nwg, SCAL_FOLD));
  }
  a.marks = (h->profiling && &s == &h->sh[0]) ? s.marks : nullptr;
  a.kind = (a.marks && !h->multiproc) ? h->kind_dev : nullptr;
  a.host_u = (!h->multiproc && &s == &h->sh[0]) ? h->u_pinned_dev : nullptr;
  a.stamps = (&s == &h->sh[0]) ? h->stamps_dev : nullptr;
  a.stamps_wide = h->stamps_rows > 4096 ? 1 : 0;
  const bool view = h->csc_valid && s.rv.valid;
  a.in_view = view ? s.rv.in_view[s.rv.cur] : nullptr;
  a.rv_nslots = view ? s.rv.st.s_nslots : 0;
  a.rv_nwork = view ? s.rv.st.s_nwork : 0;
  a.rv_fresh = (view && h->rv_fresh) ? 1 : 0;
  a.rv_rows = view ? static_cast<int>(s.rv.nrows) : 0;
  a.rvp = h->rvp;
  a.decide_only = h->decide_only ? 1 : 0;
  a.adaptive_window = (h->csc_valid && h->world == 1 && !h->multiproc && h->sh.size() == 1 && h->adaptive_window) ? 1 : 0;
  a.sub_state = 0;
  a.sub_ncol = 0.0;
  a.colmap = nullptr;
  if (h->parent != nullptr) {
    Ctx* p = h->parent;
    a.host = p->mirror_dev;
    a.host_u = p->u_pinned_dev;
    a.marks = p->profiling ? p->sh[0].marks : nullptr;
    a.kind = a.marks ? p->kind_dev : nullptr;
    a.stamps = p->stamps_dev;
    a.stamps_wide = p->stamps_rows > 4096 ? 1 : 0;
    a.sub_state = 2;
    a.sub_ncol = p->sub.ncol;
    a.colmap = p->sub.colmap;
    static const int test_leave = std::getenv("CLIPPER_HIP_SUB_TEST_LEAVE") ? std::atoi(std::getenv("CLIPPER_HIP_SUB_TEST_LEAVE")) : 0;
    if (test_leave > 0 && p->sub.launches_since_entry >= test_leave) a.sub_ncol = 1e300;
  } else if (h->sub.ready && !h->sub.active && !h->decide_only) {
    a.sub_state = 1;
    a.sub_ncol = h->sub.ncol;
  }
  return a;
}

template <int V>
int enqueue_iteration_v(Ctx* h, const SolverParams& prm) {
  const int par = h->par;
  h->par ^= 1;
  const bool sharded = !(h->world == 1 && !h->multiproc);
  Shard& s0 = h->sh[0];
  constexpr int every = PROFILE_EVERY;
  Ctx* hp = h->parent != nullptr ? h->parent : h;
  const bool prof = hp->profiling && (hp->launch_counter % every == 4 || hp->launch_counter == 11) &&
                    hp->ev_used < MAX_EVENT_PAIRS;
  for (auto& s : h->sh) {
    HIPCHK(hipSetDevice(s.device));
    const SolveArgs a = solve_args(h, s, prm, par);
    if (prof && &s == &s0) HIPCHK(hipEventRecord(hp->ev_pairs[2 * hp->ev_used], s.stream));
    if (h->csc_valid) launch_pass_csc<V>(h, s, a);
    else launch_pass<V>(h, s, a);
    if (prof && &s == &s0) {
      HIPCHK(hipEventRecord(hp->ev_pairs[2 * hp->ev_used + 1], s.stream));
      hp->ev_launch_index[hp->ev_used] = hp->launch_counter;
      ++hp->ev_used;
    }
  }
  ++hp->launch_counter;
  if (h->parent != nullptr) ++hp->sub.launches_since_entry;
  const bool fresh_used = h->rv_fresh;
  const int xk = (prof && sharded) ? h->ev_used - 1 : -1;
  if (xk >= 0) HIPCHK(hipEventRecord(h->ev_xchg[2 * xk], s0.stream));
  if (sharded) {
    for (auto& s : h->sh) {
      HIPCHK(hipSetDevice(s.device));
      const SolveArgs a = solve_args(h, s, prm, par);
      const int64_t n = static_cast<int64_t>(nslot(V)) * h->W;
      hipLaunchKernelGGL(k_reduce_pass, dim3(static_cast<unsigned>(ceil_div(n, 256))), dim3(256), 0,
                         s.stream, a, nslot(V));
    }
    int rc = exchange(h, nslot(V));
    if (rc) return rc;
    if (xk >= 0) {
      HIPCHK(hipSetDevice(s0.device));
      HIPCHK(hipEventRecord(h->ev_xchg[2 * xk + 1], s0.stream));
      h->ev_xchg_used[static_cast<size_t>(xk)] = 1;
    }
  }
  for (auto& s : h->sh) {
    HIPCHK(hipSetDevice(s.device));
    const SolveArgs a = solve_args(h, s, prm, par);
    dim3 grid(static_cast<unsigned>(a.nwg), V);
    const bool tables = !h->csc_valid;
    if (sharded) {
      if (tables) hipLaunchKernelGGL((k_tail<V, false, true>), grid, dim3(TAIL_THREADS), 0, s.stream, a);
      else hipLaunchKernelGGL((k_tail<V, false, false>), grid, dim3(TAIL_THREADS), 0, s.stream, a);
    } else {
      if (tables) hipLaunchKernelGGL((k_tail<V, true, true>), grid, dim3(TAIL_THREADS * TAIL_SPLIT), 0, s.stream, a);
      else hipLaunchKernelGGL((k_tail<V, true, false>), grid, dim3(TAIL_THREADS * TAIL_SPLIT), 0, s.stream, a);
    }
    if (a.nwg_in != a.nwg)
      hipLaunchKernelGGL(k_scal_fold, dim3(static_cast<unsigned>(a.nwg_in)), dim3(128), 0, s.stream,
                         a.scal, a.nwg, tail_q(V),
                         const_cast<double*>(a.scal_in), a.shared);
  }
  if (fresh_used) h->rv_fresh = false;
  return 0;
}

int enqueue_iteration(Ctx* h, const SolverParams& prm) {
  int rc = 0;
  dispatch_window(h, [&](auto v) { rc = enqueue_iteration_v<decltype(v)::value>(h, prm); });
  return rc;
}

int enqueue_gemv_plain(Ctx* h) {
  for (auto& s : h->sh) {
    HIPCHK(hipSetDevice(s.device));
    launch_plain(h, s, s.X[0]);
  }
  return 0;
}

int enqueue_reduce_exchange(Ctx* h) {
  for (auto& s : h->sh) {
    HIPCHK(hipSetDevice(s.device));
    launch_reduce(h, s, 2);
  }
  return exchange(h, 2);
}

int sync_all(Ctx* h) {
  for (auto& s : h->sh) {
    HIPCHK(hipSetDevice(s.device));
    HIPCHK(hipStreamSynchronize(s.stream));
  }
  HIPCHK(hipGetLastError());
  return 0;
}

std::vector<int32_t> indices_of_k_largest(const std::vector<double>& x, int k) {
  using T = std::pair<double, int>;
  if (k < 1) return {};
  if (static_cast<size_t>(k) > x.size()) k = static_cast<int>(x.size());
  std::vector<int> pos;
  bool nonneg = true;
  for (size_t i = 0; i < x.size(); ++i) {
    if (x[i] > 0.0) pos.push_back(static_cast<int>(i));
    else if (!(x[i] == 0.0)) nonneg = false;
  }
  const bool sparse_walk = nonneg && pos.size() >= static_cast<size_t>(k);
  const size_t n = sparse_walk ? pos.size() : x.size();
  std::priority_queue<T, std::vector<T>, std::greater<T>> q;
  for (size_t t = 0; t < n; ++t) {
    const size_t i = sparse_walk ? static_cast<size_t>(pos[t]) : t;
    if (q.size() < static_cast<size_t>(k)) {
      q.push({x[i], static_cast<int>(i)});
    } else if (q.top().first < x[i]) {
      q.pop();
      q.push({x[i], static_cast<int>(i)});
    }
  }
  std::vector<int32_t> out(static_cast<size_t>(k));
  for (int i = 0; i < k; ++i) {
    out[static_cast<size_t>(k - i - 1)] = q.top().second;
    q.pop();
  }
  return out;
}

Ctx* make_ctx(const int* devices, int nlocal, int storage, int world, int first_slot,
              bool multiproc) {
  int ndev = 0;
  if (hipGetDeviceCount(&ndev) != hipSuccess || ndev <= 0) {
    fail(CLIPPER_HIP_E_NODEVICE, "no HIP device visible (this library has no CPU fallback)");
    return nullptr;
  }
  if (storage != CLIPPER_HIP_STORE_F32 && storage != CLIPPER_HIP_STORE_F64 &&
      storage != CLIPPER_HIP_STORE_F32_CSC && storage != CLIPPER_HIP_STORE_F64_CSC) {
    fail(CLIPPER_HIP_E_INVALID, "storage must be CLIPPER_HIP_STORE_F32, _F64, _F32_CSC or _F64_CSC");
    return nullptr;
  }
  Ctx* h = new Ctx();
  h->compressed = (storage == CLIPPER_HIP_STORE_F32_CSC || storage == CLIPPER_HIP_STORE_F64_CSC);
  h->storage = (storage == CLIPPER_HIP_STORE_F32_CSC) ? CLIPPER_HIP_STORE_F32
               : (storage == CLIPPER_HIP_STORE_F64_CSC) ? CLIPPER_HIP_STORE_F64 : storage;
  h->world = world;
  h->multiproc = multiproc;
  h->sh.resize(static_cast<size_t>(nlocal));
  for (int p = 0; p < nlocal; ++p) {
    Shard& s = h->sh[static_cast<size_t>(p)];
    s.device = devices[p];
    s.slot = first_slot + p;
    if (s.device < 0 || s.device >= ndev) {
      fail(CLIPPER_HIP_E_INVALID, "device %d out of range (%d visible)", s.device, ndev);
      clipper_hip_destroy(h);
      return nullptr;
    }
    if (hipSetDevice(s.device) != hipSuccess ||
        hipStreamCreateWithFlags(&s.stream, hipStreamNonBlocking) != hipSuccess ||
        hipEventCreateWithFlags(&s.ev_reduced, hipEventDisableTiming) != hipSuccess ||
        hipEventCreateWithFlags(&s.ev_copied, hipEventDisableTiming) != hipSuccess) {
      fail(CLIPPER_HIP_E_HIP, "cannot create stream/events on device %d", s.device);
      clipper_hip_destroy(h);
      return nullptr;
    }
  }
  for (auto& a : h->sh)
    for (auto& b : h->sh)
      if (a.device != b.device) {
        hipSetDevice(a.device);
        int can = 0;
        hipDeviceCanAccessPeer(&can, a.device, b.device);
        if (can) {
          hipError_t e = hipDeviceEnablePeerAccess(b.device, 0);
          if (e != hipSuccess && e != hipErrorPeerAccessAlreadyEnabled) (void)hipGetLastError();
          (void)hipGetLastError();
        }
      }
  hipSetDevice(h->sh[0].device);
  hipDeviceProp_t prop;
  if (hipGetDeviceProperties(&prop, h->sh[0].device) == hipSuccess)
    h->cus = prop.multiProcessorCount > 0 ? prop.multiProcessorCount : 256;
  if (hipHostMalloc(reinterpret_cast<void**>(&h->host_state), 2 * sizeof(SolveShared),
                    hipHostMallocDefault) != hipSuccess ||
      hipEventCreateWithFlags(&h->ev_poll[0], hipEventDisableTiming) != hipSuccess ||
      hipEventCreateWithFlags(&h->ev_poll[1], hipEventDisableTiming) != hipSuccess) {
    fail(CLIPPER_HIP_E_HIP, "cannot allocate pinned solver state");
    clipper_hip_destroy(h);
    return nullptr;
  }
  if (hipHostMalloc(reinterpret_cast<void**>(&h->mirror), sizeof(HostMirror),
                    hipHostMallocMapped | hipHostMallocCoherent) != hipSuccess ||
      hipHostGetDevicePointer(reinterpret_cast<void**>(&h->mirror_dev), h->mirror, 0) !=
          hipSuccess) {
    fail(CLIPPER_HIP_E_HIP, "cannot allocate the pinned progress record");
    clipper_hip_destroy(h);
    return nullptr;
  }
  std::memset(h->mirror, 0, sizeof(HostMirror));
  if (hipHostMalloc(reinterpret_cast<void**>(&h->kind), KIND_CAP,
                    hipHostMallocMapped | hipHostMallocCoherent) != hipSuccess ||
      hipHostGetDevicePointer(reinterpret_cast<void**>(&h->kind_dev), h->kind, 0) != hipSuccess) {
    fail(CLIPPER_HIP_E_HIP, "cannot allocate the pinned iteration marks");
    clipper_hip_destroy(h);
    return nullptr;
  }
  std::memset(h->kind, 0, KIND_CAP);
  if (const char* e = std::getenv("CLIPPER_HIP_STAMPS")) {
    h->stamps_rows = std::atoi(e) == 2 ? 16384 : 4096;
    const size_t bytes = static_cast<size_t>(h->stamps_rows) * 4 * sizeof(long long);
    if (hipMalloc(&h->stamps_dev, bytes) == hipSuccess) (void)hipMemset(h->stamps_dev, 0, bytes);
    else h->stamps_dev = nullptr;
  }
  if (const char* w = std::getenv("CLIPPER_HIP_WINDOW")) {
    const int v = std::atoi(w);
    if (v == 1 || v == 4 || v == 6 || v == 8) h->V_forced = v;
  }
  if (const char* e = std::getenv("CLIPPER_HIP_ADAPTIVE_WINDOW"))
    if (std::atoi(e) == 0) h->adaptive_window = false;
  if (const char* e = std::getenv("CLIPPER_HIP_RESIDENT"))
    if (std::atoi(e) == 0) h->resident_mode = 1;
  return h;
}

template <typename T>
int ensure_cap(T*& p, size_t& cap, size_t bytes) {
  if (bytes <= cap && p) return 0;
  if (p) hipFree(p);
  p = nullptr;
  cap = 0;
  HIPCHK(hipMalloc(&p, bytes));
  cap = bytes;
  return 0;
}

int upload_points(Ctx* h, Shard& s, const double* D1, const double* D2, int d, int64_t n1,
                  int64_t n2, int64_t pstride) {
  const size_t b1 = static_cast<size_t>(d) * n1 * sizeof(double);
  const size_t b2 = static_cast<size_t>(d) * n2 * sizeof(double);
  const size_t bp = static_cast<size_t>(d) * pstride * sizeof(double);
  const size_t ba = static_cast<size_t>(2 * h->m) * sizeof(int32_t);
  int rc;
  if ((rc = ensure_cap(s.dD1, s.capD1, b1))) return rc;
  if ((rc = ensure_cap(s.dD2, s.capD2, b2))) return rc;
  size_t capP2 = s.capP;
  if ((rc = ensure_cap(s.P1, s.capP, bp))) return rc;
  if ((rc = ensure_cap(s.P2, capP2, bp))) return rc;
  if ((rc = ensure_cap(s.Adev, s.capA, ba))) return rc;
  size_t capPf2 = s.capPf;
  if ((rc = ensure_cap(s.P1f, s.capPf, bp / 2))) return rc;
  if ((rc = ensure_cap(s.P2f, capPf2, bp / 2))) return rc;
  HIPCHK(hipMemcpyAsync(s.dD1, D1, b1, hipMemcpyHostToDevice, s.stream));
  HIPCHK(hipMemcpyAsync(s.dD2, D2, b2, hipMemcpyHostToDevice, s.stream));
  HIPCHK(hipMemcpyAsync(s.Adev, h->A.data(), ba, hipMemcpyHostToDevice, s.stream));
  dim3 grid(static_cast<unsigned>(ceil_div(pstride, 256))), block(256);
  hipLaunchKernelGGL(k_gather_points, grid, block, 0, s.stream, s.dD1, d, s.Adev, h->m, pstride,
                     s.P1, s.P1f);
  hipLaunchKernelGGL(k_gather_points, grid, block, 0, s.stream, s.dD2, d, s.Adev + h->m, h->m,
                     pstride, s.P2, s.P2f);
  HIPCHK(hipStreamSynchronize(s.stream));
  return 0;
}

int stage_inputs(Ctx* h, const double* D1, int d, int64_t n1, const double* D2, int64_t n2,
                 const int32_t* A, int64_t m_in) {
  if (!h || !D1 || !D2 || d < 1 || n1 < 1 || n2 < 1)
    return fail(CLIPPER_HIP_E_INVALID, "invalid argument");
  int64_t m = m_in;
  if (A == nullptr || m_in == 0) {
    m = n1 * n2;
    h->A.assign(static_cast<size_t>(2 * m), 0);
    for (int64_t i = 0; i < n1; ++i)
      for (int64_t j = 0; j < n2; ++j) {
        h->A[static_cast<size_t>(j + i * n2)] = static_cast<int32_t>(i);
        h->A[static_cast<size_t>(m + j + i * n2)] = static_cast<int32_t>(j);
      }
  } else {
    h->A.assign(A, A + 2 * m);
  }
  for (int64_t r = 0; r < m; ++r) {
    const int32_t a0 = h->A[static_cast<size_t>(r)], a1 = h->A[static_cast<size_t>(m + r)];
    if (a0 < 0 || a0 >= n1 || a1 < 0 || a1 >= n2)
      return fail(CLIPPER_HIP_E_INVALID, "association %lld = (%d,%d) out of range",
                  static_cast<long long>(r), a0, a1);
  }
  h->nodes.clear();
  h->fill_kind = 0;
  rowview_drop(h);
  int rc = ensure_problem(h, m);
  if (rc) return rc;
  const int64_t pstride = round_up(m, 64);
  if (static_cast<int64_t>(d) * pstride * static_cast<int64_t>(sizeof(double)) >= (int64_t(1) << 32))
    return fail(CLIPPER_HIP_E_SCOPE, "point tables of %d x %lld doubles exceed 4 GiB", d, static_cast<long long>(pstride));
  for (auto& s : h->sh) {
    HIPCHK(hipSetDevice(s.device));
    rc = upload_points(h, s, D1, D2, d, n1, n2, pstride);
    if (rc) return rc;
  }
  h->staged_d = d;
  h->staged_pstride = pstride;
  double mx = 0.0;
  for (int64_t i = 0; i < static_cast<int64_t>(d) * n1; ++i) mx = std::max(mx, std::fabs(D1[i]));
  for (int64_t i = 0; i < static_cast<int64_t>(d) * n2; ++i) mx = std::max(mx, std::fabs(D2[i]));
  h->staged_maxabs = mx;
  const char* mode = std::getenv("CLIPPER_HIP_AFFINITY");
  h->plain_affinity = (mode && std::strcmp(mode, "plain") == 0);
  h->strip_affinity = (mode && std::strcmp(mode, "strip") == 0);
  return 0;
}

float guarded_threshold(double eps, double maxabs, int d) {
  const double guard = std::ldexp(128.0 * (d + 1), -24) * maxabs;
  const double t = eps + guard;
  if (!(t < 3.0e38)) return std::numeric_limits<float>::infinity();
  return std::nextafter(static_cast<float>(t), std::numeric_limits<float>::infinity());
}

float guarded_threshold_sq(float E) {
  if (!(E < 1.0e19f)) return std::numeric_limits<float>::infinity();
  const double e2 = static_cast<double>(E) * static_cast<double>(E);
  return std::nextafter(static_cast<float>(e2), std::numeric_limits<float>::infinity());
}

bool use_sym_fill(const Ctx* h) {
  return !h->plain_affinity && !h->strip_affinity && h->world == 1 && !h->multiproc &&
         (h->storage == CLIPPER_HIP_STORE_F32 || (h->storage == CLIPPER_HIP_STORE_F64 && h->compressed));
}

bool raise_dynamic_lds(const void* fn, int device, int bytes) {
  static std::mutex mu;
  static std::vector<std::pair<const void*, int>> raised;
  std::lock_guard<std::mutex> lock(mu);
  const std::pair<const void*, int> key{fn, device};
  if (std::find(raised.begin(), raised.end(), key) != raised.end()) return true;
  if (hipFuncSetAttribute(fn, hipFuncAttributeMaxDynamicSharedMemorySize, bytes) != hipSuccess) {
    (void)hipGetLastError();
    return false;
  }
  raised.push_back(key);
  return true;
}

template <typename VT, typename K>
void launch_sym(K kernel, dim3 grid, hipStream_t stream, VT* S, int64_t W, int64_t mm, int nT,
                const Shard& s, int64_t pstride, const int32_t* A0, const int32_t* A1,
                const EuclidParams& e, const PointNormalParams& n, float E2, const CscOut& O) {
  constexpr int L = at_sym_lds_bytes<VT>();
  raise_dynamic_lds(reinterpret_cast<const void*>(kernel), s.device, L);
  hipLaunchKernelGGL(kernel, grid, dim3(AT_WAVES * 64), L, stream, S, W, mm, nT, s.P1, s.P2,
                     s.P1f, s.P2f, pstride, A0, A1, e, n, E2, O);
}


}
```

clipper_amd/csrc/host_state.hpp:

```cpp
#pragma once

namespace {

thread_local std::string g_err;

int fail(int code, const char* fmt, ...) {
  char buf[512];
  va_list ap;
  va_start(ap, fmt);
  vsnprintf(buf, sizeof(buf), fmt, ap);
  va_end(ap);
  g_err = buf;
  return code;
}

int guard_fail(int code, const char* what) noexcept {
  try {
    g_err = what;
  } catch (...) {
  }
  return code;
}
#define CLIPPER_HIP_GUARD_CATCH(on_nomem, on_other)                                                     \
  catch (const std::bad_alloc&) { on_nomem; }                                                            \
  catch (const std::exception& e) { (void)e; on_other; }                                                 \
  catch (...) { on_other; }
#define CLIPPER_HIP_GUARD_INT                                                                            \
  CLIPPER_HIP_GUARD_CATCH(return guard_fail(CLIPPER_HIP_E_NOMEM, "out of host memory inside the library"), \
                          return guard_fail(CLIPPER_HIP_E_INTERNAL, "unexpected exception inside the library"))
#define CLIPPER_HIP_GUARD_PTR                                                                            \
  CLIPPER_HIP_GUARD_CATCH({ guard_fail(CLIPPER_HIP_E_NOMEM, "out of host memory inside the library"); return nullptr; }, \
                          { guard_fail(CLIPPER_HIP_E_INTERNAL, "unexpected exception inside the library"); return nullptr; })
#define CLIPPER_HIP_GUARD_STR CLIPPER_HIP_GUARD_CATCH(return "", return "")
#define CLIPPER_HIP_GUARD_VOID CLIPPER_HIP_GUARD_CATCH(return, return)


#define HIPCHK(expr)                                                                  \
  do {                                                                                \
    hipError_t e_ = (expr);                                                           \
    if (e_ != hipSuccess)                                                             \
      return fail(e_ == hipErrorOutOfMemory ? CLIPPER_HIP_E_NOMEM : CLIPPER_HIP_E_HIP, \
                  "%s failed: %s (%s:%d)", #expr, hipGetErrorString(e_), __FILE__,    \
                  __LINE__);                                                          \
  } while (0)

inline int64_t round_up(int64_t a, int64_t b) { return (a + b - 1) / b * b; }
inline int64_t ceil_div(int64_t a, int64_t b) { return (a + b - 1) / b; }

constexpr int GEMV_NW = 8;
constexpr int GEMV_WG_PER_CU = 2;
constexpr int gemv_unr(int V, int esize, bool hasc) {
  int u = (V <= 6) ? 8 : 4;
  if (esize == 8) u /= 2;
  if (hasc) u /= 2;
  return u < 1 ? 1 : u;
}
constexpr int64_t WINDOW_MIN_M = 6000;
constexpr int64_t WINDOW_MIN_M_CSC = 8500;
constexpr int64_t WINDOW4_MIN_M = 2000;
constexpr int64_t RV_MIN_M = 3000;
constexpr int RV_MAX_BUILDS = 6;
constexpr int SOLVE_BATCH = 4;
constexpr int RUN_AHEAD = 4;
constexpr int MAX_EVENT_PAIRS = 256;
constexpr int PROFILE_EVERY = 20;

struct Rccl {
  void* lib = nullptr;
  ncclResult_t (*GetUniqueId)(ncclUniqueId*) = nullptr;
  ncclResult_t (*CommInitRank)(ncclComm_t*, int, ncclUniqueId, int) = nullptr;
  ncclResult_t (*AllGather)(const void*, void*, size_t, ncclDataType_t, ncclComm_t,
                            hipStream_t) = nullptr;
  ncclResult_t (*CommDestroy)(ncclComm_t) = nullptr;
  const char* (*GetErrorString)(ncclResult_t) = nullptr;
};
Rccl g_rccl;

int load_rccl() {
  if (g_rccl.lib) return 0;
  const char* names[] = {"librccl.so.1", "librccl.so", "/opt/rocm/lib/librccl.so.1"};
  void* lib = nullptr;
  for (const char* n : names) {
    lib = dlopen(n, RTLD_NOW | RTLD_GLOBAL);
    if (lib) break;
  }
  if (!lib) return fail(CLIPPER_HIP_E_COMM, "cannot load librccl: %s", dlerror());
  auto sym = [&](const char* s) { return dlsym(lib, s); };
  g_rccl.GetUniqueId = reinterpret_cast<decltype(g_rccl.GetUniqueId)>(sym("ncclGetUniqueId"));
  g_rccl.CommInitRank = reinterpret_cast<decltype(g_rccl.CommInitRank)>(sym("ncclCommInitRank"));
  g_rccl.AllGather = reinterpret_cast<decltype(g_rccl.AllGather)>(sym("ncclAllGather"));
  g_rccl.CommDestroy = reinterpret_cast<decltype(g_rccl.CommDestroy)>(sym("ncclCommDestroy"));
  g_rccl.GetErrorString =
      reinterpret_cast<decltype(g_rccl.GetErrorString)>(sym("ncclGetErrorString"));
  if (!g_rccl.GetUniqueId || !g_rccl.CommInitRank || !g_rccl.AllGather || !g_rccl.CommDestroy)
    return fail(CLIPPER_HIP_E_COMM, "librccl is missing required symbols");
  g_rccl.lib = lib;
  return 0;
}

struct SliceStore {
  uint32_t* sSizes = nullptr;
  uint32_t* sLq = nullptr;
  uint64_t* sPre = nullptr;
  uint64_t* sBlk = nullptr;
  uint8_t* sdata = nullptr;
  SliceWork* swork = nullptr;
  size_t scap_slices = 0, scap_bytes = 0, scap_work = 0;
  int s_ncg = 0, s_nchunks = 0;
  int s_nwork = 0;
  int s_nslots = 0;
  uint64_t s_bytes = 0;
  uint64_t s_entries = 0;
};

struct RowView {
  SliceStore st;
  int32_t* rowmap[2] = {nullptr, nullptr};
  uint8_t* in_view[2] = {nullptr, nullptr};
  int cur = 0;
  SliceView* desc = nullptr;
  uint32_t* blk = nullptr;
  int32_t* viewpos = nullptr;
  size_t cap_rows = 0, cap_flags = 0, cap_blk = 0, cap_pos = 0;
  int64_t nrows = 0;
  bool valid = false;
  bool plan_pending = false;
  SliceStore full;
  bool full_valid = false;
};

struct Shard : SliceStore {
  int device = 0;
  int slot = 0;
  hipStream_t stream = nullptr;
  void* S = nullptr;
  void* Cs = nullptr;
  double* part = nullptr;
  double* u0 = nullptr;
  double* pt = nullptr;
  double* cab = nullptr;
  double* X[2] = {nullptr, nullptr};
  double* ab = nullptr;
  double* scal = nullptr;
  SolverState* st = nullptr;
  uint8_t* marks = nullptr;
  SolveShared* shared = nullptr;
  double *P1 = nullptr, *P2 = nullptr;
  float *P1f = nullptr, *P2f = nullptr;
  size_t capPf = 0;
  int32_t* Adev = nullptr;
  double *dD1 = nullptr, *dD2 = nullptr;
  size_t capP = 0, capA = 0, capD1 = 0, capD2 = 0;
  hipEvent_t ev_reduced = nullptr, ev_copied = nullptr;
  size_t bytes_S = 0;
  size_t part_tiles = 0;
  uint16_t* gOff = nullptr;
  uint64_t* gPre = nullptr;
  void* gvals = nullptr;
  uint8_t* grows = nullptr;
  CscBuildCtl* cctl = nullptr;
  size_t gcap_units = 0, gcap_groups = 0;
  RowView rv;
};

struct Resident {
  bool ready = false;
  bool failed = false;
  int last_error = 0;
  int V = 0, E = 0, nunits = 0, maxslots = 0;
  uint32_t lds_slices = 0, lds_total = 0;
  uint8_t* host_plan = nullptr;
  uint8_t* host_plan_dev = nullptr;
  size_t host_plan_cap = 0;
  size_t off_np = 0, off_wc = 0, off_pc = 0;
  unsigned long long* xb = nullptr;
  size_t xb_cap = 0;
  unsigned long long* ctl = nullptr;
  unsigned long long epoch = 0;
  int V_forced = 0;
  bool xcd_off = false;
  int home = -1;
};

struct ViewResident {
  bool ready = false;
  int nunits = 0;
  uint32_t lds_slices = 0;
  uint8_t* host_plan = nullptr;
  uint8_t* host_plan_dev = nullptr;
  size_t host_plan_cap = 0;
  size_t off_np = 0, off_wc = 0, off_pc = 0;
  unsigned long long* xb = nullptr;
  size_t xb_bytes = 0;
  uint32_t* ctl = nullptr;
  unsigned long long epoch = 0;
  int target_units = 0;
  uint32_t* giveup_host = nullptr;
  hipEvent_t ev[2 * 16] = {};
  int ev_n = 0;
  uint64_t plan_entries = 0;
  uint32_t* giveup_host_dev = nullptr;
  int launches_this_solve = 0;
  int cooldown = 0, cooldown_next = 1;
  int max_units_device = -1;
  bool on_replica = false;
  uint8_t* backup = nullptr;
};
constexpr int RVR_GIVEUP_SLOTS = 16;

constexpr int SUB_MAX_ENTRIES = 4;
constexpr int64_t SUB_MIN_M = 12000;
struct SubProblem {
  struct clipper_hip_ctx* ctx = nullptr;
  struct clipper_hip_ctx* ctx_dense = nullptr;
  struct clipper_hip_ctx* use = nullptr;
  int32_t* cnt = nullptr;
  uint8_t* flags = nullptr;
  int32_t* colmap = nullptr;
  int32_t* pos = nullptr;
  uint32_t* blk = nullptr;
  int32_t* nout_acc = nullptr;
  size_t cap = 0, cap_blk = 0;
  SubRecord* rec = nullptr;
  SubRecord* rec_dev = nullptr;
  bool ready = false;
  bool active = false;
  int entries = 0;
  int launches_since_entry = 0;
  int64_t nS = 0;
  double ncol = 0.0;
  int64_t passes_at_entry = 0, sub_passes = 0, leaves = 0;
  double build_ms = 0.0;
};

}

struct clipper_hip_ctx {
  int storage = CLIPPER_HIP_STORE_F32;
  int world = 1;
  bool multiproc = false;
  std::vector<Shard> sh;
  ncclComm_t comm = nullptr;
  clipper_hip_allgather_fn xchg_fn = nullptr;
  void* xchg_user = nullptr;
  double* xchg_send = nullptr;
  double* xchg_recv = nullptr;
  size_t xchg_cap = 0;

  int64_t m = 0;
  int64_t W = 0;
  int64_t alloc_m = 0, alloc_W = 0;
  bool has_matrix = false;
  bool explicitC = false;
  bool compressed = false;
  bool csc_valid = false;
  bool csc_emitted = false;
  CscOut csc_out{};
  int csc_nblocks = 0, csc_nstrips = 0;
  uint32_t* csc_hLq = nullptr;
  CscBuildCtl* csc_hctl = nullptr;
  uint64_t* csc_htotal = nullptr;
  SliceWork* csc_hwork = nullptr;
  size_t csc_hcap_slices = 0, csc_hcap_work = 0;
  int staged_d = 0;
  double staged_maxabs = 0;
  bool plain_affinity = false;
  bool strip_affinity = false;
  int64_t staged_pstride = 0;
  bool u0_staged = false;
  int ntiles = 1, rows_per_tile = 0, nstrips = 0;
  int cus = 256;

  std::vector<int32_t> A;
  std::vector<int32_t> nodes;
  std::vector<double> u_host;

  SolveShared* host_state = nullptr;
  hipEvent_t ev_poll[2] = {nullptr, nullptr};
  hipEvent_t ev_aff[2] = {nullptr, nullptr};
  HostMirror* mirror = nullptr;
  HostMirror* mirror_dev = nullptr;
  uint8_t* kind = nullptr;
  uint8_t* kind_dev = nullptr;
  double* u_pinned = nullptr;
  double* u_pinned_dev = nullptr;
  size_t u_pinned_cap = 0;
  int V = 6;
  int V_forced = 0;
  int64_t mp = 0;
  int par = 0;
  Resident res;
  ViewResident vres;
  bool decide_only = false;
  std::function<int()> enqueue_one;
  bool early_decide_done = false;
  int resident_mode = 0;
  int last_solver = 0;

  int fill_kind = 0;
  EuclidParams fill_e{};
  PointNormalParams fill_n{};
  float fill_E2 = 0.f;
  double total_slice_bytes = 0.0;
  ViewPolicy rvp{};
  bool rv_fresh = false;
  int rv_mode = 0;
  SliceView* rv_desc_host = nullptr;
  int rv_desc_slot = 0;
  SliceView* rv_desc_host_dev = nullptr;
  int32_t* rv_count = nullptr;
  int32_t* rv_count_dev = nullptr;
  clipper_hip_view_stats_t rv_stats{};
  SubProblem sub;
  struct clipper_hip_ctx* parent = nullptr;
  bool adaptive_window = true;
  int sub_mode = 0;

  long long* stamps_dev = nullptr;
  int stamps_rows = 4096;
  bool profiling = false;
  int profiling_level = 0;
  std::vector<hipEvent_t> ev_pairs;
  std::vector<int64_t> ev_launch_index;
  std::vector<hipEvent_t> ev_xchg;
  std::vector<char> ev_xchg_used;
  int ev_used = 0;
  int64_t launch_counter = 0;
  clipper_hip_timings_t tm{};

  size_t esize() const { return storage == CLIPPER_HIP_STORE_F64 ? 8 : 4; }
};
```

clipper_amd/csrc/host_subproblem.hpp:

```cpp
#pragma once

namespace {

bool sub_enabled(const Ctx* h) {
  static const bool env_off = [] {
    const char* e = std::getenv("CLIPPER_HIP_SUBPROBLEM");
    return e && std::atoi(e) == 0;
  }();
  static const int64_t min_m = std::getenv("CLIPPER_HIP_SUBPROBLEM_MIN_M") ? std::atoll(std::getenv("CLIPPER_HIP_SUBPROBLEM_MIN_M")) : SUB_MIN_M;
  return !env_off && h->sub_mode != 1 && h->parent == nullptr && h->sh.size() == 1 && h->world == 1 && !h->multiproc &&
         h->csc_valid && !h->explicitC && h->m >= min_m && rect_fill_possible(h);
}

void sub_begin_solve(Ctx* h) {
  SubProblem& sp = h->sub;
  sp.ready = sp.active = false;
  sp.entries = 0;
  sp.sub_passes = sp.leaves = 0;
  sp.build_ms = 0.0;
}

void sub_free(Ctx* h) {
  SubProblem& sp = h->sub;
  for (Ctx** pc : {&sp.ctx, &sp.ctx_dense}) {
    if (*pc) {
      (*pc)->sh[0].stream = nullptr;
      clipper_hip_destroy(*pc);
      *pc = nullptr;
    }
  }
  sp.use = nullptr;
  if (!h->sh.empty()) hipSetDevice(h->sh[0].device);
  auto fr = [](auto*& p) {
    if (p) hipFree(p);
    p = nullptr;
  };
  fr(sp.cnt);
  fr(sp.flags);
  fr(sp.colmap);
  fr(sp.pos);
  fr(sp.blk);
  fr(sp.nout_acc);
  if (sp.rec) hipHostFree(sp.rec);
  sp.rec = sp.rec_dev = nullptr;
  sp.cap = sp.cap_blk = 0;
  sp.ready = sp.active = false;
}

int sub_stage(Ctx* h, Ctx* c, int64_t nS) {
  Shard& s = h->sh[0];
  Shard& cs = c->sh[0];
  c->V_forced = h->V;
  c->resident_mode = 1;
  c->rv_mode = 1;
  c->nodes.clear();
  c->fill_kind = 0;
  rowview_drop(c);
  int rc = ensure_problem(c, nS);
  if (rc) return rc;
  const int d = h->staged_d;
  const int64_t qs = round_up(nS, 64);
  const size_t bp = static_cast<size_t>(d) * qs * sizeof(double);
  size_t capP2 = cs.capP;
  if ((rc = ensure_cap(cs.P1, cs.capP, bp))) return rc;
  if ((rc = ensure_cap(cs.P2, capP2, bp))) return rc;
  size_t capPf2 = cs.capPf;
  if ((rc = ensure_cap(cs.P1f, cs.capPf, bp / 2))) return rc;
  if ((rc = ensure_cap(cs.P2f, capPf2, bp / 2))) return rc;
  if ((rc = ensure_cap(cs.Adev, cs.capA, static_cast<size_t>(2 * nS) * sizeof(int32_t)))) return rc;
  dim3 grid(static_cast<unsigned>(ceil_div(qs, 256))), block(256);
  hipLaunchKernelGGL(k_sub_gather_points, grid, block, 0, s.stream, s.P1, s.P1f, d, h->staged_pstride, s.Adev, h->m,
                     h->sub.colmap, nS, qs, cs.P1, cs.P1f, cs.Adev, 0);
  hipLaunchKernelGGL(k_sub_gather_points, grid, block, 0, s.stream, s.P2, s.P2f, d, h->staged_pstride, s.Adev, h->m,
                     h->sub.colmap, nS, qs, cs.P2, cs.P2f, cs.Adev, 1);
  c->staged_d = d;
  c->staged_pstride = qs;
  c->staged_maxabs = h->staged_maxabs;
  c->plain_affinity = h->plain_affinity;
  c->strip_affinity = h->strip_affinity;
  return 0;
}

template <int V>
int sub_prepare_v(Ctx* h) {
  SubProblem& sp = h->sub;
  sp.ready = false;
  Shard& s = h->sh[0];
  RowView& v = s.rv;
  if (!sub_enabled(h) || !v.valid || h->vres.ready || sp.entries >= SUB_MAX_ENTRIES) return 0;
  const auto t0 = std::chrono::high_resolution_clock::now();
  HIPCHK(hipSetDevice(s.device));
  const int64_t m = h->m, mp = h->mp;
  const int nblk = static_cast<int>(ceil_div(m, RV_BLK));
  int rc;
  if (static_cast<size_t>(mp) > sp.cap) {
    for (void** p : {reinterpret_cast<void**>(&sp.cnt), reinterpret_cast<void**>(&sp.flags), reinterpret_cast<void**>(&sp.colmap),
                     reinterpret_cast<void**>(&sp.pos)}) {
      if (*p) hipFree(*p);
      *p = nullptr;
    }
    sp.cap = 0;
    HIPCHK(hipMalloc(&sp.cnt, static_cast<size_t>(mp) * sizeof(int32_t)));
    HIPCHK(hipMalloc(&sp.flags, static_cast<size_t>(mp)));
    HIPCHK(hipMalloc(&sp.colmap, static_cast<size_t>(mp) * sizeof(int32_t)));
    HIPCHK(hipMalloc(&sp.pos, static_cast<size_t>(mp) * sizeof(int32_t)));
    sp.cap = static_cast<size_t>(mp);
  }
  if ((rc = rv_grow(sp.blk, sp.cap_blk, static_cast<size_t>(nblk) + 2))) return rc;
  if (!sp.nout_acc) HIPCHK(hipMalloc(&sp.nout_acc, 8 * sizeof(int32_t)));
  if (!sp.rec) {
    HIPCHK(hipHostMalloc(reinterpret_cast<void**>(&sp.rec), 64, hipHostMallocMapped | hipHostMallocCoherent));
    HIPCHK(hipHostGetDevicePointer(reinterpret_cast<void**>(&sp.rec_dev), sp.rec, 0));
  }
  sp.rec->nS = -1;
  sp.rec->ncol = -1;
  sp.rec->n0 = -1;
  std::atomic_thread_fence(std::memory_order_seq_cst);
  const SliceView RV = row_view(h, s);
  hipLaunchKernelGGL(k_sub_begin, dim3(1), dim3(64), 0, s.stream, sp.nout_acc);
  hipLaunchKernelGGL(k_sub_colcount, dim3(static_cast<unsigned>(ceil_div(RV.ncg, 4))), dim3(256), 0, s.stream, RV, sp.cnt, mp);
  hipLaunchKernelGGL((k_sub_flags<V>), dim3(static_cast<unsigned>(nblk)), dim3(256), 0, s.stream, s.st + h->par, sp.cnt,
                     v.in_view[v.cur], m, mp, sp.flags, sp.blk, sp.nout_acc);
  hipLaunchKernelGGL(k_rv_scan, dim3(1), dim3(1024), 0, s.stream, sp.blk, nblk, &sp.rec_dev->nS);
  hipLaunchKernelGGL(k_rv_scatter, dim3(static_cast<unsigned>(nblk)), dim3(256), 0, s.stream, sp.flags, m, sp.blk, sp.colmap,
                     static_cast<int64_t>(sp.cap), sp.pos, mp);
  hipLaunchKernelGGL(k_sub_publish, dim3(1), dim3(64), 0, s.stream, sp.nout_acc, sp.rec_dev);
  HIPCHK(hipStreamSynchronize(s.stream));
  HIPCHK(hipGetLastError());
  std::atomic_thread_fence(std::memory_order_acquire);
  const int64_t nS = sp.rec->nS;
  static const bool host_timing = std::getenv("CLIPPER_HIP_HOST_TIMING") != nullptr;
  if (host_timing)
    std::fprintf(stderr, "[sub] view of %lld rows: S = %lld associations, N0 = %d, the largest count outside %d\n",
                 static_cast<long long>(v.nrows), static_cast<long long>(nS), sp.rec->n0, sp.rec->ncol);
  if (nS < 64 || sp.rec->ncol < 0 || nS > 2 * v.nrows + 1024 || 3 * nS > m) return 0;
  auto build_child = [&](Ctx*& c, int storage) -> int {
    if (!c) {
      c = make_ctx(&s.device, 1, storage, 1, 0, false);
      if (!c) return CLIPPER_HIP_E_HIP;
      hipStreamDestroy(c->sh[0].stream);
      c->sh[0].stream = s.stream;
      c->parent = h;
    }
    if (int r2 = sub_stage(h, c, nS)) return r2;
    if (h->fill_kind == 1)
      return clipper_hip_affinity_euclidean_staged(c, h->fill_e.sigma, h->fill_e.epsilon, h->fill_e.mindist, h->fill_e.affinityeps);
    return clipper_hip_affinity_pointnormal_staged(c, h->fill_n.sigp, h->fill_n.epsp, h->fill_n.sign, h->fill_n.epsn,
                                                   h->fill_n.affinityeps);
  };
  const int storage = h->compressed ? (h->storage == CLIPPER_HIP_STORE_F64 ? CLIPPER_HIP_STORE_F64_CSC : CLIPPER_HIP_STORE_F32_CSC)
                                    : h->storage;
  static const bool dense_off = std::getenv("CLIPPER_HIP_SUB_DENSE") && std::atoi(std::getenv("CLIPPER_HIP_SUB_DENSE")) == 0;
  const double in_entries = static_cast<double>((static_cast<unsigned long long>(sp.rec->entries_hi) << 32) | sp.rec->entries_lo);
  const double density = in_entries / (static_cast<double>(nS) * static_cast<double>(std::max<int64_t>(1, v.nrows)));
  const bool dense = !dense_off && h->sub_mode != 2 && h->storage == CLIPPER_HIP_STORE_F32 && density >= 0.5 && nS >= 1024;
  Ctx* c = nullptr;
  if (dense) {
    rc = build_child(sp.ctx_dense, CLIPPER_HIP_STORE_F32);
    if (rc == 0 && sp.ctx_dense->has_matrix && !sp.ctx_dense->csc_valid) c = sp.ctx_dense;
    else if (rc != 0 && rc != CLIPPER_HIP_E_NOMEM) return rc;
    else (void)hipGetLastError();
  }
  if (c == nullptr) {
    if ((rc = build_child(sp.ctx, storage))) return rc;
    if (!sp.ctx->csc_valid) return 0;
    c = sp.ctx;
  }
  sp.use = c;
  HIPCHK(hipSetDevice(s.device));
  sp.nS = nS;
  sp.ncol = static_cast<double>(std::max(1, sp.rec->ncol)) + static_cast<double>(std::max<int64_t>(0, nS - v.nrows));
  sp.ready = true;
  sp.build_ms += std::chrono::duration<double, std::milli>(std::chrono::high_resolution_clock::now() - t0).count();
  if (host_timing)
    std::fprintf(stderr, "[sub] ready: %lld associations, density %.2f -> %s (%.1f MB), prepared in %.2f ms\n",
                 static_cast<long long>(nS), density, c->csc_valid ? "slices" : "a dense fp32 store",
                 (c->csc_valid ? static_cast<double>(c->sh[0].s_bytes) : algorithmic_gemv_bytes(c)) * 1e-6, sp.build_ms);
  return 0;
}

int sub_prepare(Ctx* h) {
  int rc = 0;
  dispatch_window(h, [&](auto v) { rc = sub_prepare_v<decltype(v)::value>(h); });
  return rc;
}

int enqueue_iteration(Ctx* h, const SolverParams& prm);

int sub_enter(Ctx* h, const SolverParams& prm) {
  SubProblem& sp = h->sub;
  if (!sp.ready || sp.active || !sp.use) return fail(CLIPPER_HIP_E_INTERNAL, "sub-problem: a hand-over nobody prepared");
  Shard& s = h->sh[0];
  Ctx* c = sp.use;
  Shard& cs = c->sh[0];
  HIPCHK(hipSetDevice(s.device));
  hipLaunchKernelGGL(k_sub_resume, dim3(1), dim3(64), 0, s.stream, s.st + h->par, s.shared);
  h->decide_only = true;
  int rc = enqueue_iteration(h, prm);
  h->decide_only = false;
  if (rc) return rc;
  std::memset(h->u_pinned, 0, static_cast<size_t>(h->m) * sizeof(double));
  std::atomic_thread_fence(std::memory_order_seq_cst);
  hipLaunchKernelGGL(k_sub_enter, dim3(static_cast<unsigned>(ceil_div(c->mp, 256))), dim3(256), 0, s.stream, s.st + h->par, s.pt,
                     s.cab, h->mp, h->V, sp.colmap, sp.nS, cs.st, cs.shared, cs.pt, cs.cab, c->mp,
                     c->csc_valid ? static_cast<double*>(nullptr) : cs.X[0], prm.beta);
  c->par = 0;
  c->decide_only = false;
  c->rv_fresh = false;
  sp.active = true;
  sp.entries += 1;
  sp.launches_since_entry = 0;
  sp.passes_at_entry = h->mirror->n_passes;
  h->rv_stats.sub_entries += 1;
  return 0;
}

int sub_leave(Ctx* h) {
  SubProblem& sp = h->sub;
  if (!sp.active || !sp.use) return fail(CLIPPER_HIP_E_INTERNAL, "sub-problem: nothing to leave");
  Shard& s = h->sh[0];
  Ctx* c = sp.use;
  Shard& cs = c->sh[0];
  HIPCHK(hipSetDevice(s.device));
  hipLaunchKernelGGL(k_sub_leave, dim3(static_cast<unsigned>(ceil_div(h->mp, 256))), dim3(256), 0, s.stream, cs.st + c->par, cs.pt,
                     cs.cab, c->mp, h->V, sp.pos, s.rv.in_view[s.rv.cur], h->m, s.pt, s.cab, h->mp, sp.nout_acc);
  hipLaunchKernelGGL(k_sub_leave_state, dim3(1), dim3(256), 0, s.stream, cs.st + c->par, s.st + h->par, s.shared, sp.nout_acc);
  sp.active = false;
  sp.leaves += 1;
  if (sp.entries >= SUB_MAX_ENTRIES) sp.ready = false;
  return 0;
}

}
```

Before: 1.328.

## Defer compressed affinity build completion and settle lazily on next API call

The compressed (CSC-emitting) affinity build is now enqueued and returned immediately, with completion checking, overflow retry and validity flags deferred to a settle step that every public entry point calls first. Host-side waits switch from stream synchronize to spin-polling an event. The solver's run-ahead enqueue is capped to one iteration while a resident launch is still in flight. This aims to overlap host work with the fill kernel and to cut synchronisation latency. In exchange it adds deferred-state complexity, lambdas captured by value for later replay, and a busy-wait that uses a CPU core.

```diff
diff --git a/clipper_amd/csrc/clipper_hip.hip b/clipper_amd/csrc/clipper_hip.hip
--- a/clipper_amd/csrc/clipper_hip.hip
+++ b/clipper_amd/csrc/clipper_hip.hip
@@ -104,6 +104,7 @@
 } CLIPPER_HIP_GUARD_INT
 
 int clipper_hip_comm_init(clipper_hip_t* h, const void* id128) try {
+  if (int rc = settle(h)) return rc;
   if (!h || !id128) return fail(CLIPPER_HIP_E_INVALID, "invalid argument");
   if (!h->multiproc) return 0;
   int rc = load_rccl();
@@ -119,6 +120,7 @@
 } CLIPPER_HIP_GUARD_INT
 
 int clipper_hip_comm_init_callback(clipper_hip_t* h, clipper_hip_allgather_fn fn, void* user) try {
+  if (int rc = settle(h)) return rc;
   if (!h || !fn) return fail(CLIPPER_HIP_E_INVALID, "invalid argument");
   if (!h->multiproc) return 0;
   h->xchg_fn = fn;
@@ -128,6 +130,8 @@
 
 void clipper_hip_destroy(clipper_hip_t* h) try {
   if (!h) return;
+  h->build_pending = false;
+  h->pending_fill = nullptr;
   for (auto& s : h->sh) {
     hipSetDevice(s.device);
     if (s.stream) hipStreamSynchronize(s.stream);
@@ -138,6 +142,7 @@
     free_shard_buffers(s);
     if (s.ev_reduced) hipEventDestroy(s.ev_reduced);
     if (s.ev_copied) hipEventDestroy(s.ev_copied);
+    if (s.ev_wait) hipEventDestroy(s.ev_wait);
     if (s.stream) hipStreamDestroy(s.stream);
   }
   if (!h->sh.empty()) hipSetDevice(h->sh[0].device);
@@ -145,6 +150,7 @@
   for (hipEvent_t e : h->ev_xchg) hipEventDestroy(e);
   if (h->ev_poll[0]) hipEventDestroy(h->ev_poll[0]);
   if (h->ev_poll[1]) hipEventDestroy(h->ev_poll[1]);
+  if (h->ev_res_end) hipEventDestroy(h->ev_res_end);
   if (h->host_state) hipHostFree(h->host_state);
   if (h->mirror) hipHostFree(h->mirror);
   if (h->kind) hipHostFree(h->kind);
@@ -173,6 +179,7 @@
 
 int clipper_hip_affinity_euclidean_staged(clipper_hip_t* h, double sigma, double epsilon,
                                           double mindist, double affinityeps) try {
+  if (int rc = settle(h)) return rc;
   if (!h) return fail(CLIPPER_HIP_E_INVALID, "invalid argument");
   if (h->staged_d < 1) return fail(CLIPPER_HIP_E_STATE, "clipper_hip_stage_inputs not called");
   const EuclidParams prm{sigma, epsilon, mindist, affinityeps};
@@ -182,7 +189,7 @@
   h->fill_e = prm;
   h->fill_n = PointNormalParams{};
   h->fill_E2 = guarded_threshold_sq(guarded_threshold(epsilon, h->staged_maxabs, d));
-  return run_affinity(h, use_sym_fill(h) && (d == 2 || d == 3), [&](Shard& s) {
+  return run_affinity(h, use_sym_fill(h) && (d == 2 || d == 3), [=](Shard& s) {
     dim3 grid(static_cast<unsigned>(ceil_div(W, 1024)),
               static_cast<unsigned>(ceil_div(mm, AFF_ROWS_PER_BLK))),
         block(256);
@@ -240,6 +247,7 @@
 
 int clipper_hip_affinity_pointnormal_staged(clipper_hip_t* h, double sigp, double epsp,
                                             double sign, double epsn, double affinityeps) try {
+  if (int rc = settle(h)) return rc;
   if (!h) return fail(CLIPPER_HIP_E_INVALID, "invalid argument");
   if (h->staged_d != 6)
     return fail(CLIPPER_HIP_E_STATE, "PointNormalDistance needs staged inputs with d == 6");
@@ -249,7 +257,7 @@
   h->fill_e = EuclidParams{};
   h->fill_n = prm;
   h->fill_E2 = guarded_threshold_sq(guarded_threshold(epsp, h->staged_maxabs, 3));
-  return run_affinity(h, use_sym_fill(h), [&](Shard& s) {
+  return run_affinity(h, use_sym_fill(h), [=](Shard& s) {
     dim3 grid(static_cast<unsigned>(ceil_div(W, 1024)),
               static_cast<unsigned>(ceil_div(mm, AFF_ROWS_PER_BLK))),
         block(256);
@@ -294,11 +302,13 @@
                                    const double* D2, int64_t n2, const int32_t* A, int64_t m,
                                    double sigma, double epsilon, double mindist,
                                    double affinityeps) try {
+  if (int rc = settle(h)) return rc;
   const auto t0 = std::chrono::high_resolution_clock::now();
   int rc = stage_inputs(h, D1, d, n1, D2, n2, A, m);
   if (rc) return rc;
   rc = clipper_hip_affinity_euclidean_staged(h, sigma, epsilon, mindist, affinityeps);
   if (rc) return rc;
+  if ((rc = settle(h))) return rc;
   h->tm.affinity_total_ms =
       std::chrono::duration<double, std::milli>(std::chrono::high_resolution_clock::now() - t0)
           .count();
@@ -309,12 +319,14 @@
                                      const double* D2, int64_t n2, const int32_t* A, int64_t m,
                                      double sigp, double epsp, double sign, double epsn,
                                      double affinityeps) try {
+  if (int rc = settle(h)) return rc;
   if (d != 6) return fail(CLIPPER_HIP_E_INVALID, "PointNormalDistance needs d == 6");
   const auto t0 = std::chrono::high_resolution_clock::now();
   int rc = stage_inputs(h, D1, d, n1, D2, n2, A, m);
   if (rc) return rc;
   rc = clipper_hip_affinity_pointnormal_staged(h, sigp, epsp, sign, epsn, affinityeps);
   if (rc) return rc;
+  if ((rc = settle(h))) return rc;
   h->tm.affinity_total_ms =
       std::chrono::duration<double, std::milli>(std::chrono::high_resolution_clock::now() - t0)
           .count();
@@ -335,6 +347,7 @@
 
 
 int clipper_hip_set_matrix(clipper_hip_t* h, const double* M, const double* C, int64_t m) try {
+  if (int rc = settle(h)) return rc;
   if (!h || !M || !C || m < 1) return fail(CLIPPER_HIP_E_INVALID, "invalid argument");
   if (h->A.size() != static_cast<size_t>(2 * m)) h->A.clear();
   h->nodes.clear();
@@ -434,6 +447,7 @@
 int clipper_hip_set_sparse(clipper_hip_t* h, int64_t m, const int64_t* Mcolptr,
                            const int32_t* Mrow, const double* Mval, const int64_t* Ccolptr,
                            const int32_t* Crow, const double* Cval) try {
+  if (int rc = settle(h)) return rc;
   if (!h || !Mcolptr || !Ccolptr || m < 1) return fail(CLIPPER_HIP_E_INVALID, "invalid argument");
   auto check_csc = [&](const char* what, const int64_t* cp, const int32_t* ri, const double* va) -> int {
     if (cp[0] != 0) return fail(CLIPPER_HIP_E_INVALID, "%s: colptr[0] must be 0", what);
@@ -674,6 +688,7 @@
 } CLIPPER_HIP_GUARD_INT
 
 int clipper_hip_get_matrix(clipper_hip_t* h, double* M_out, double* C_out) try {
+  if (int rc = settle(h)) return rc;
   if (!h) return fail(CLIPPER_HIP_E_INVALID, "invalid argument");
   if (!h->has_matrix) return fail(CLIPPER_HIP_E_STATE, "no matrix has been built or set");
   if (h->multiproc)
@@ -715,6 +730,7 @@
 
 
 int clipper_hip_stage_u0(clipper_hip_t* h, const double* u0) try {
+  if (int rc = settle(h)) return rc;
   if (!h || !u0) return fail(CLIPPER_HIP_E_INVALID, "u0 is required");
   if (!h->has_matrix) return fail(CLIPPER_HIP_E_STATE, "no matrix has been built or set");
   const size_t vbytes = static_cast<size_t>(h->m) * sizeof(double);
@@ -730,6 +746,7 @@
 
 int clipper_hip_solve(clipper_hip_t* h, const double* u0, const clipper_params_t* P,
                       double* u_out, clipper_solve_info_t* info) try {
+  if (int rc = settle(h)) return rc;
   if (!h || !u0 || !P) return fail(CLIPPER_HIP_E_INVALID, "u0 and params are required");
   const auto t0 = std::chrono::high_resolution_clock::now();
   int rc = clipper_hip_stage_u0(h, u0);
@@ -745,6 +762,7 @@
 
 int clipper_hip_solve_staged(clipper_hip_t* h, const clipper_params_t* P, double* u_out,
                              clipper_solve_info_t* info) try {
+  if (int rc = settle(h)) return rc;
   if (!h || !P) return fail(CLIPPER_HIP_E_INVALID, "params are required");
   if (!h->has_matrix) return fail(CLIPPER_HIP_E_STATE, "no matrix has been built or set");
   if (!h->u0_staged) return fail(CLIPPER_HIP_E_STATE, "clipper_hip_stage_u0 not called");
@@ -835,6 +853,8 @@
     volatile HostMirror* hm = h->mirror;
     int64_t queued = 0;
     uint64_t spins = 0;
+    bool behind_resident = false;
+    int64_t queued_behind = 0;
     h->rv_fresh = false;
     constexpr int run_ahead = RUN_AHEAD;
     h->enqueue_one = [h, &prm]() { return enqueue_iteration(h, prm); };
@@ -890,6 +910,12 @@
           }
           bool launched = false;
           if ((rc = rvr_enqueue(h, prm, launched))) return rc;
+          if (launched) {
+            if (!h->ev_res_end) HIPCHK(hipEventCreateWithFlags(&h->ev_res_end, hipEventDisableTiming));
+            HIPCHK(hipEventRecord(h->ev_res_end, s0.stream));
+            behind_resident = true;
+            queued_behind = 0;
+          }
           mark_t("resident queued");
         }
         if ((rc = rowview_finish_plan(h))) return rc;
@@ -904,9 +930,11 @@
         continue;
       }
       if (hm->iters > queued) queued = hm->iters;
-      if (queued - hm->iters < run_ahead) {
+      if (behind_resident && hipEventQuery(h->ev_res_end) != hipErrorNotReady) behind_resident = false;
+      if (behind_resident ? queued_behind < 1 : queued - hm->iters < run_ahead) {
         if ((rc = enqueue_next())) return rc;
         ++queued;
+        queued_behind += behind_resident ? 1 : 0;
         spins = 0;
       } else if ((++spins & 0xfffff) == 0) {
         hipError_t q = hipStreamQuery(s0.stream);
@@ -1101,6 +1129,7 @@
 } CLIPPER_HIP_GUARD_INT
 
 int clipper_hip_get_nodes(const clipper_hip_t* h, int32_t* out, int32_t capacity) try {
+  if (int rc = settle(h)) return rc;
   if (!h || !out) return fail(CLIPPER_HIP_E_INVALID, "invalid argument");
   const int32_t k = static_cast<int32_t>(h->nodes.size());
   if (capacity < k) return fail(CLIPPER_HIP_E_INVALID, "capacity %d < %d nodes", capacity, k);
@@ -1110,6 +1139,7 @@
 
 int clipper_hip_get_selected_associations(const clipper_hip_t* h, int32_t* A_out,
                                           int32_t capacity) try {
+  if (int rc = settle(h)) return rc;
   if (!h || !A_out) return fail(CLIPPER_HIP_E_INVALID, "invalid argument");
   const int32_t k = static_cast<int32_t>(h->nodes.size());
   if (capacity < k) return fail(CLIPPER_HIP_E_INVALID, "capacity %d < %d nodes", capacity, k);
@@ -1126,6 +1156,7 @@
 
 int clipper_hip_densest_subgraph(clipper_hip_t* h, const int32_t* S, int32_t k, int32_t* nodes_out,
                                  int32_t capacity) try {
+  if (int rc = settle(h)) return rc;
   if (!h || !nodes_out) return fail(CLIPPER_HIP_E_INVALID, "invalid argument");
   if (!h->has_matrix) return fail(CLIPPER_HIP_E_STATE, "no matrix has been built or set");
   if (h->multiproc)
@@ -1257,6 +1288,7 @@
 } CLIPPER_HIP_GUARD_INT
 
 int clipper_hip_set_window(clipper_hip_t* h, int window) try {
+  if (int rc = settle(h)) return rc;
   if (!h) return fail(CLIPPER_HIP_E_INVALID, "invalid argument");
   if (window != 0 && window != 1 && window != 4 && window != 6 && window != 8)
     return fail(CLIPPER_HIP_E_INVALID, "window must be 0 (automatic), 1, 4, 6 or 8");
@@ -1265,10 +1297,12 @@
 } CLIPPER_HIP_GUARD_INT
 
 int clipper_hip_window(const clipper_hip_t* h) try {
+  if (int rc = settle(h)) return rc;
   return h ? h->V : 0;
 } CLIPPER_HIP_GUARD_INT
 
 int clipper_hip_set_resident(clipper_hip_t* h, int mode) try {
+  if (int rc = settle(h)) return rc;
   if (!h) return fail(CLIPPER_HIP_E_INVALID, "invalid argument");
   if (mode != 0 && mode != 1 && mode != 2)
     return fail(CLIPPER_HIP_E_INVALID, "mode must be 0 (automatic), 1 (never) or 2 (the sub-problem always as slices)");
@@ -1277,10 +1311,12 @@
 } CLIPPER_HIP_GUARD_INT
 
 int clipper_hip_last_solver(const clipper_hip_t* h) try {
+  if (int rc = settle(h)) return rc;
   return h ? h->last_solver : -1;
 } CLIPPER_HIP_GUARD_INT
 
 int clipper_hip_set_row_view(clipper_hip_t* h, int mode) try {
+  if (int rc = settle(h)) return rc;
   if (!h) return fail(CLIPPER_HIP_E_INVALID, "invalid argument");
   if (mode != 0 && mode != 1 && mode != 2)
     return fail(CLIPPER_HIP_E_INVALID, "mode must be 0 (automatic), 1 (never) or 2 (views, but streamed: never the resident solver on one)");
@@ -1291,6 +1327,7 @@
 } CLIPPER_HIP_GUARD_INT
 
 int clipper_hip_set_subproblem(clipper_hip_t* h, int mode) try {
+  if (int rc = settle(h)) return rc;
   if (!h) return fail(CLIPPER_HIP_E_INVALID, "invalid argument");
   if (mode != 0 && mode != 1 && mode != 2)
     return fail(CLIPPER_HIP_E_INVALID, "mode must be 0 (automatic), 1 (never) or 2 (the sub-problem always as slices)");
@@ -1300,18 +1337,21 @@
 } CLIPPER_HIP_GUARD_INT
 
 int clipper_hip_get_view_stats(const clipper_hip_t* h, clipper_hip_view_stats_t* out) try {
+  if (int rc = settle(h)) return rc;
   if (!h || !out) return fail(CLIPPER_HIP_E_INVALID, "invalid argument");
   *out = h->rv_stats;
   return 0;
 } CLIPPER_HIP_GUARD_INT
 
 int clipper_hip_storage_in_use(const clipper_hip_t* h) try {
+  if (int rc = settle(h)) return rc;
   if (!h) return -1;
   if (!h->csc_valid) return h->storage;
   return h->storage == CLIPPER_HIP_STORE_F64 ? CLIPPER_HIP_STORE_F64_CSC : CLIPPER_HIP_STORE_F32_CSC;
 } CLIPPER_HIP_GUARD_INT
 
 int clipper_hip_matvec(clipper_hip_t* h, const double* x, double* yM, double* yC) try {
+  if (int rc = settle(h)) return rc;
   if (!h || !x) return fail(CLIPPER_HIP_E_INVALID, "invalid argument");
   if (!h->has_matrix) return fail(CLIPPER_HIP_E_STATE, "no matrix has been built or set");
   const int64_t m = h->m, W = h->W;
@@ -1342,6 +1382,7 @@
 
 int clipper_hip_view_matvec(clipper_hip_t* h, const int32_t* rows, int64_t nrows, const double* x,
                             double* yM, double* yC) try {
+  if (int rc = settle(h)) return rc;
   if (!h || !rows || !x || nrows < 1) return fail(CLIPPER_HIP_E_INVALID, "invalid argument");
   if (!h->has_matrix || !h->csc_valid || !csc_single(h) || !rect_fill_possible(h))
     return fail(CLIPPER_HIP_E_STATE, "a row view needs slices of a matrix scored from staged points on one device");
@@ -1407,6 +1448,7 @@
 
 
 int clipper_hip_set_profiling(clipper_hip_t* h, int on) try {
+  if (int rc = settle(h)) return rc;
   if (!h) return fail(CLIPPER_HIP_E_INVALID, "invalid argument");
   h->profiling = (on != 0);
   h->profiling_level = on;
@@ -1423,12 +1465,14 @@
 } CLIPPER_HIP_GUARD_INT
 
 int clipper_hip_get_timings(const clipper_hip_t* h, clipper_hip_timings_t* out) try {
+  if (int rc = settle(h)) return rc;
   if (!h || !out) return fail(CLIPPER_HIP_E_INVALID, "invalid argument");
   *out = h->tm;
   return 0;
 } CLIPPER_HIP_GUARD_INT
 
 int clipper_hip_bench_matvec(clipper_hip_t* h, int reps, double* avg_us) try {
+  if (int rc = settle(h)) return rc;
   if (!h || reps < 1 || !avg_us) return fail(CLIPPER_HIP_E_INVALID, "invalid argument");
   if (!h->has_matrix) return fail(CLIPPER_HIP_E_STATE, "no matrix has been built or set");
   if (!h->csc_valid)
@@ -1453,6 +1497,7 @@
 } CLIPPER_HIP_GUARD_INT
 
 int clipper_hip_debug_stamps(clipper_hip_t* h, int64_t* out, int capacity) try {
+  if (int rc = settle(h)) return rc;
   if (!h || !out || capacity < 0) return fail(CLIPPER_HIP_E_INVALID, "invalid argument");
   if (!h->stamps_dev) return fail(CLIPPER_HIP_E_STATE, "CLIPPER_HIP_STAMPS was not set when the context was created");
   const int n = std::min(capacity, h->stamps_rows * 4);
@@ -1479,6 +1524,7 @@
 } CLIPPER_HIP_GUARD_INT
 
 int clipper_hip_device_info(const clipper_hip_t* h, char* name64, int* cus, int64_t* hbm_bytes) try {
+  if (int rc = settle(h)) return rc;
   if (!h) return fail(CLIPPER_HIP_E_INVALID, "invalid argument");
   hipDeviceProp_t prop;
   HIPCHK(hipGetDeviceProperties(&prop, h->sh[0].device));
diff --git a/clipper_amd/csrc/host_matrix.hpp b/clipper_amd/csrc/host_matrix.hpp
--- a/clipper_amd/csrc/host_matrix.hpp
+++ b/clipper_amd/csrc/host_matrix.hpp
@@ -493,8 +493,62 @@
   return sync_all(h);
 }
 
+int emit_queue(Ctx* h) {
+  Shard& s0 = h->sh[0];
+  CscOut O{};
+  if (int rc = emit_prepare(h, s0, O)) return rc;
+  h->csc_out = O;
+  HIPCHK(hipSetDevice(s0.device));
+  HIPCHK(hipEventRecord(h->ev_aff[0], s0.stream));
+  h->pending_fill(s0);
+  if (int rc = emit_enqueue(h, s0)) return rc;
+  HIPCHK(hipEventRecord(h->ev_aff[1], s0.stream));
+  return 0;
+}
+
+int build_settle(Ctx* h) {
+  if (!h->build_pending) return 0;
+  h->build_pending = false;
+  Shard& s0 = h->sh[0];
+  int rc = 0;
+  for (int attempt = 0;; ++attempt) {
+    const auto th1 = std::chrono::high_resolution_clock::now();
+    if ((rc = spin_sync(s0))) break;
+    bool again = false;
+    if ((rc = emit_check(h, s0, again))) break;
+    if (std::getenv("CLIPPER_HIP_HOST_TIMING")) {
+      const auto th2 = std::chrono::high_resolution_clock::now();
+      float kms = 0.f;
+      (void)hipEventElapsedTime(&kms, h->ev_aff[0], h->ev_aff[1]);
+      std::fprintf(stderr, "[affinity] settled: fill %.1f us (events), wait + check + plan %.1f us\n", kms * 1e3,
+                   std::chrono::duration<double, std::micro>(th2 - th1).count());
+    }
+    if (!again) {
+      h->csc_valid = true;
+      break;
+    }
+    if (attempt >= 2) {
+      rc = fail(CLIPPER_HIP_E_HIP, "compressed storage: the build keeps overflowing");
+      break;
+    }
+    if ((rc = emit_queue(h))) break;
+  }
+  h->pending_fill = nullptr;
+  if (rc) return rc;
+  float ms = 0.f;
+  HIPCHK(hipSetDevice(s0.device));
+  HIPCHK(hipEventElapsedTime(&ms, h->ev_aff[0], h->ev_aff[1]));
+  h->tm.affinity_kernel_ms = ms;
+  h->tm.affinity_bytes = static_cast<double>(s0.s_bytes);
+  h->has_matrix = true;
+  return 0;
+}
+
+int settle(const Ctx* h) { return h ? build_settle(const_cast<Ctx*>(h)) : 0; }
+
 template <typename Launch>
 int run_affinity(Ctx* h, bool emits, Launch launch) {
+  if (int rc = build_settle(h)) return rc;
   h->has_matrix = false;
   h->csc_valid = false;
   h->total_slice_bytes = 0.0;
@@ -530,59 +584,33 @@
     HIPCHK(hipEventCreate(&h->ev_aff[0]));
     HIPCHK(hipEventCreate(&h->ev_aff[1]));
   }
+  if (emit) {
+    h->pending_fill = launch;
+    h->build_pending = true;
+    if ((rc = emit_queue(h))) {
+      h->build_pending = false;
+      h->pending_fill = nullptr;
+      return rc;
+    }
+    return h->defer_build ? 0 : build_settle(h);
+  }
   hipEvent_t e0 = h->ev_aff[0], e1 = h->ev_aff[1];
-  double build_ms = 0.0;
-  for (int attempt = 0;; ++attempt) {
-    CscOut O{};
-    if (emit) {
-      rc = emit_prepare(h, s0, O);
-      if (rc) return rc;
-    } else {
-      h->csc_valid = false;
-      h->csc_emitted = false;
-    }
-    h->csc_out = O;
-    HIPCHK(hipSetDevice(s0.device));
-    HIPCHK(hipEventRecord(e0, s0.stream));
-    for (auto& s : h->sh) {
-      HIPCHK(hipSetDevice(s.device));
-      launch(s);
-    }
-    if (emit) {
-      rc = emit_enqueue(h, s0);
-      if (rc) return rc;
-    }
-    HIPCHK(hipSetDevice(s0.device));
-    HIPCHK(hipEventRecord(e1, s0.stream));
-    const auto th0 = std::chrono::high_resolution_clock::now();
-    rc = sync_all(h);
-    if (rc) return rc;
-    const auto th1 = std::chrono::high_resolution_clock::now();
-    if (!emit) {
-      const auto t0 = std::chrono::high_resolution_clock::now();
-      rc = csc_rebuild(h);
-      if (rc) return rc;
-      build_ms = std::chrono::duration<double, std::milli>(
-                     std::chrono::high_resolution_clock::now() - t0).count();
-      break;
-    }
-    bool again = false;
-    rc = emit_check(h, s0, again);
-    if (rc) return rc;
-    if (std::getenv("CLIPPER_HIP_HOST_TIMING")) {
-      const auto th2 = std::chrono::high_resolution_clock::now();
-      float kms = 0.f;
-      (void)hipEventElapsedTime(&kms, e0, e1);
-      std::fprintf(stderr, "[affinity] enqueue->synced %.1f us (events %.1f us), check+plan %.1f us\n",
-                   std::chrono::duration<double, std::micro>(th1 - th0).count(), kms * 1e3,
-                   std::chrono::duration<double, std::micro>(th2 - th1).count());
-    }
-    if (!again) {
-      h->csc_valid = true;
-      break;
-    }
-    if (attempt >= 2) return fail(CLIPPER_HIP_E_HIP, "compressed storage: the build keeps overflowing");
-  }
+  h->csc_valid = false;
+  h->csc_emitted = false;
+  h->csc_out = CscOut{};
+  HIPCHK(hipSetDevice(s0.device));
+  HIPCHK(hipEventRecord(e0, s0.stream));
+  for (auto& s : h->sh) {
+    HIPCHK(hipSetDevice(s.device));
+    launch(s);
+  }
+  HIPCHK(hipSetDevice(s0.device));
+  HIPCHK(hipEventRecord(e1, s0.stream));
+  if ((rc = sync_all(h))) return rc;
+  const auto t0 = std::chrono::high_resolution_clock::now();
+  if ((rc = csc_rebuild(h))) return rc;
+  const double build_ms = std::chrono::duration<double, std::milli>(
+                              std::chrono::high_resolution_clock::now() - t0).count();
   float ms = 0.f;
   HIPCHK(hipSetDevice(s0.device));
   HIPCHK(hipEventElapsedTime(&ms, e0, e1));
diff --git a/clipper_amd/csrc/host_rowview.hpp b/clipper_amd/csrc/host_rowview.hpp
--- a/clipper_amd/csrc/host_rowview.hpp
+++ b/clipper_amd/csrc/host_rowview.hpp
@@ -336,8 +336,7 @@
       v.cur = cur0;
       v.nrows = nrows0;
     }
-    HIPCHK(hipStreamSynchronize(s.stream));
-    HIPCHK(hipGetLastError());
+    if ((rc = spin_sync(s))) return rc;
     lap("filled");
     if (!counted) {
       counted = true;
diff --git a/clipper_amd/csrc/host_solver.hpp b/clipper_amd/csrc/host_solver.hpp
--- a/clipper_amd/csrc/host_solver.hpp
+++ b/clipper_amd/csrc/host_solver.hpp
@@ -455,6 +455,17 @@
   return 0;
 }
 
+int spin_sync(Shard& s) {
+  HIPCHK(hipSetDevice(s.device));
+  HIPCHK(hipEventRecord(s.ev_wait, s.stream));
+  hipError_t q;
+  while ((q = hipEventQuery(s.ev_wait)) == hipErrorNotReady) {
+  }
+  if (q != hipSuccess) return fail(CLIPPER_HIP_E_HIP, "stream failed: %s", hipGetErrorString(q));
+  HIPCHK(hipGetLastError());
+  return 0;
+}
+
 std::vector<int32_t> indices_of_k_largest(const std::vector<double>& x, int k) {
   using T = std::pair<double, int>;
   if (k < 1) return {};
@@ -516,7 +527,8 @@
     if (hipSetDevice(s.device) != hipSuccess ||
         hipStreamCreateWithFlags(&s.stream, hipStreamNonBlocking) != hipSuccess ||
         hipEventCreateWithFlags(&s.ev_reduced, hipEventDisableTiming) != hipSuccess ||
-        hipEventCreateWithFlags(&s.ev_copied, hipEventDisableTiming) != hipSuccess) {
+        hipEventCreateWithFlags(&s.ev_copied, hipEventDisableTiming) != hipSuccess ||
+        hipEventCreateWithFlags(&s.ev_wait, hipEventDisableTiming) != hipSuccess) {
       fail(CLIPPER_HIP_E_HIP, "cannot create stream/events on device %d", s.device);
       clipper_hip_destroy(h);
       return nullptr;
@@ -577,6 +589,8 @@
     if (std::atoi(e) == 0) h->adaptive_window = false;
   if (const char* e = std::getenv("CLIPPER_HIP_RESIDENT"))
     if (std::atoi(e) == 0) h->resident_mode = 1;
+  if (const char* e = std::getenv("CLIPPER_HIP_SYNC_BUILD"))
+    if (std::atoi(e) != 0) h->defer_build = false;
   return h;
 }
 
@@ -619,10 +633,13 @@
   return 0;
 }
 
+int build_settle(Ctx* h);
+
 int stage_inputs(Ctx* h, const double* D1, int d, int64_t n1, const double* D2, int64_t n2,
                  const int32_t* A, int64_t m_in) {
   if (!h || !D1 || !D2 || d < 1 || n1 < 1 || n2 < 1)
     return fail(CLIPPER_HIP_E_INVALID, "invalid argument");
+  if (int rc = build_settle(h)) return rc;
   int64_t m = m_in;
   if (A == nullptr || m_in == 0) {
     m = n1 * n2;
diff --git a/clipper_amd/csrc/host_state.hpp b/clipper_amd/csrc/host_state.hpp
--- a/clipper_amd/csrc/host_state.hpp
+++ b/clipper_amd/csrc/host_state.hpp
@@ -152,6 +152,7 @@
   double *dD1 = nullptr, *dD2 = nullptr;
   size_t capP = 0, capA = 0, capD1 = 0, capD2 = 0;
   hipEvent_t ev_reduced = nullptr, ev_copied = nullptr;
+  hipEvent_t ev_wait = nullptr;
   size_t bytes_S = 0;
   size_t part_tiles = 0;
   uint16_t* gOff = nullptr;
@@ -256,6 +257,9 @@
   bool csc_valid = false;
   bool csc_emitted = false;
   CscOut csc_out{};
+  bool build_pending = false;
+  bool defer_build = true;
+  std::function<void(Shard&)> pending_fill;
   int csc_nblocks = 0, csc_nstrips = 0;
   uint32_t* csc_hLq = nullptr;
   CscBuildCtl* csc_hctl = nullptr;
@@ -278,6 +282,7 @@
   SolveShared* host_state = nullptr;
   hipEvent_t ev_poll[2] = {nullptr, nullptr};
   hipEvent_t ev_aff[2] = {nullptr, nullptr};
+  hipEvent_t ev_res_end = nullptr;
   HostMirror* mirror = nullptr;
   HostMirror* mirror_dev = nullptr;
   uint8_t* kind = nullptr;
diff --git a/clipper_amd/csrc/host_subproblem.hpp b/clipper_amd/csrc/host_subproblem.hpp
--- a/clipper_amd/csrc/host_subproblem.hpp
+++ b/clipper_amd/csrc/host_subproblem.hpp
@@ -141,6 +141,7 @@
       hipStreamDestroy(c->sh[0].stream);
       c->sh[0].stream = s.stream;
       c->parent = h;
+      c->defer_build = false;
     }
     if (int r2 = sub_stage(h, c, nS)) return r2;
     if (h->fill_kind == 1)
```

Result: faster. 1.301 (median of 6 runs) (-2.0%).
